# VIDILabs/instantvnr

Hardware: AMD Instinct MI355X
Metric: fps at 1024^2 on 1024^3 volume (higher is better)
Workload: dtype f16

## Files before the change

instantvnr_amd/csrc/infer_kernel.h:

```cpp
#pragma once
#include <algorithm>
#include <cstdlib>

#include "infer_tile.h"
#include "pack_rays.h"

namespace vnr {

struct FusedMlp {
  const uint16_t* packed;
  uint32_t lds_halves, width, n_hidden_matmuls, activation, output_activation;
  bool general;
  bool weights_global;
  float quantize_threshold;
};

struct InferArgs {
  const LevelInfo* levels;
  uint32_t n_levels, interpolation;
  const half_t* table;
  uint32_t table_bytes;
  const uint8_t* brick_image;
  const half_t* packed_mlp;
  const float* coords;
  float* out;
  half_t* features_out;
  half_t* acts_out;
  const uint32_t* n_ptr;
  const uint32_t* dest;
  uint32_t queue_mode;
  uint32_t out_stride;
  uint32_t n;
  uint32_t n_hidden_matmuls;
  uint32_t activation;
  uint32_t output_activation;
  uint32_t lds_halves;
  uint32_t sharers;
  uint32_t weights_global;
  float quantize_threshold;
  PackArgs pack;
};

template <int F, int K_IN, int W, int MODE, bool GENERAL>
__global__ void __launch_bounds__(64 * MlpShape<W>::WAVES) fused_infer_kernel(const InferArgs args)
{
  constexpr int NCHUNK = K_IN / 8;
  constexpr uint32_t WAVES = MlpShape<W>::WAVES;
  extern __shared__ __attribute__((aligned(16))) half_t lds[];

  const uint32_t lane = threadIdx.x & 63u;
  const uint32_t wave = threadIdx.x >> 6;

  if (MODE == 0 && WAVES == 4 && args.pack.n_blocks) {
    uint32_t* s_part = (uint32_t*)lds;
    for (uint32_t item = blockIdx.x; item < args.pack.n_blocks; item += gridDim.x) {
      pack_rays_block<4>(args.pack, item, s_part);
      __syncthreads();
    }
  }
  const uint32_t n = args.n_ptr ? min(*args.n_ptr, args.n) : args.n;
  const uint32_t n_tiles = (n + 63u) >> 6;
  const uint32_t xcd = blockIdx.x & 7u;
  const uint32_t per_xcd = (n_tiles + 7u) >> 3;
  const uint32_t waves_per_xcd = (gridDim.x >> 3) * WAVES;
  const uint32_t tile_end = min(n_tiles, (xcd + 1u) * per_xcd);
  if (xcd * per_xcd + (blockIdx.x >> 3) * WAVES >= tile_end) return;

  constexpr bool CAN_GLOBAL = GENERAL;
  const bool wglobal = CAN_GLOBAL && args.weights_global != 0u;
  if (MODE != 1 && !wglobal) {
    const uint4_t* src = (const uint4_t*)args.packed_mlp;
    uint4_t* dst = (uint4_t*)lds;
    for (uint32_t i = threadIdx.x; i < args.lds_halves / 8; i += blockDim.x) dst[i] = src[i];
    __syncthreads();
  }
  const uint32_t nh = args.n_hidden_matmuls;
  const uint32_t act = args.activation;
  const uint32_t h = lane >> 5;
  const uint32_t r = lane & 31u;
  const table_rsrc_t rsrc = make_table_rsrc(args.table, args.table_bytes);

  for (uint32_t tile = xcd * per_xcd + (blockIdx.x >> 3) * WAVES + wave; tile < tile_end; tile += waves_per_xcd) {
    const uint32_t i = tile * 64u + lane;
    const uint32_t ic = min(i, n - 1u);
    float3_packed p;
    uint32_t out_index = i;
    if (args.queue_mode) {
      const uint4_t rec = ((const uint4_t*)args.coords)[ic];
      p = {__uint_as_float(rec.x), __uint_as_float(rec.y), __uint_as_float(rec.z)};
      out_index = rec.w * args.out_stride;
    } else {
      p = ((const float3_packed*)args.coords)[ic];
      if (args.dest) out_index = args.dest[ic];
    }

    half8_t feat[NCHUNK];
    encode_tile<F, K_IN, GENERAL>(args.levels, args.n_levels, args.interpolation, rsrc, args.brick_image, p.x, p.y, p.z, feat,
                                  GENERAL ? args.quantize_threshold : 0.0f);

    if (MODE != 0 && args.features_out && i < n) {
      half8_t* dst = (half8_t*)(args.features_out + (size_t)i * K_IN);
#pragma unroll
      for (int c = 0; c < NCHUNK; ++c) dst[c] = feat[c];
    }
    if (MODE == 1) continue;

    float y;
    if (CAN_GLOBAL && wglobal)
      y = mlp_tile<W, K_IN, MODE == 2, GENERAL>(args.packed_mlp, feat, nh, act, h, r, args.acts_out, n, tile * 64u);
    else
      y = mlp_tile<W, K_IN, MODE == 2, GENERAL>((const half_t*)lds, feat, nh, act, h, r, args.acts_out, n, tile * 64u);
    if (i < n) args.out[out_index] = finish_output<GENERAL>(y, args.output_activation);
  }
}

template <int F, int K_IN, int W, int MODE, bool GENERAL>
static void launch_one(const InferArgs& a, size_t n_max, hipStream_t s)
{
  constexpr uint32_t WAVES = MlpShape<W>::WAVES;
  const Runtime& rt = Runtime::get();
  const uint32_t n_tiles = div_round_up(n_max, 64);
  uint32_t blocks = div_round_up(n_tiles, WAVES);
  static const uint32_t forced = [] {
    const char* e = std::getenv("VNR_AMD_INFER_BLOCKS_PER_CU");
    const int v = e ? std::atoi(e) : 0;
    return (uint32_t)(v >= 1 && v <= 64 ? v : 0);
  }();
  const size_t shmem = (MODE == 1 || a.weights_global) ? 16 : (size_t)a.lds_halves * sizeof(uint16_t);
  const uint32_t fit = (uint32_t)std::max<size_t>(1, std::min<size_t>(4, (160 * 1024) / std::max<size_t>(shmem, 1)));
  uint32_t max_blocks = (uint32_t)rt.n_cus * (forced ? forced : std::min(fit, a.sharers >= 2 ? 3u : 4u));
  if (!forced && a.n_ptr && a.queue_mode) max_blocks = std::min((uint32_t)rt.n_cus * 32u, std::max((uint32_t)rt.n_cus * 4u, n_tiles / 33u));
  if (blocks > max_blocks) blocks = max_blocks;
  blocks = next_multiple(blocks, 8);
  auto kernel = fused_infer_kernel<F, K_IN, W, MODE, GENERAL>;
  static bool attr_set = false;
  if (!attr_set) {
    VNR_HIP_CHECK(hipFuncSetAttribute((const void*)kernel, hipFuncAttributeMaxDynamicSharedMemorySize, 160 * 1024));
    attr_set = true;
  }
  kernel<<<blocks, 64 * WAVES, shmem, s>>>(a);
  VNR_HIP_CHECK(hipGetLastError());
}

template <int W, int MODE, bool GENERAL>
static void dispatch(uint32_t F, uint32_t K_IN, const InferArgs& a, size_t n_max, hipStream_t s)
{
#define VNR_CASE(f, k) if (F == f && K_IN == k) return launch_one<f, k, W, MODE, GENERAL>(a, n_max, s)
  VNR_CASE(1, 16); VNR_CASE(1, 32);
  VNR_CASE(2, 16); VNR_CASE(2, 32); VNR_CASE(2, 48); VNR_CASE(2, 64);
  VNR_CASE(4, 16); VNR_CASE(4, 32); VNR_CASE(4, 48); VNR_CASE(4, 64); VNR_CASE(4, 80); VNR_CASE(4, 96); VNR_CASE(4, 112); VNR_CASE(4, 128);
  VNR_CASE(8, 16); VNR_CASE(8, 32); VNR_CASE(8, 48); VNR_CASE(8, 64); VNR_CASE(8, 80); VNR_CASE(8, 96); VNR_CASE(8, 112); VNR_CASE(8, 128);
#undef VNR_CASE
  throw std::runtime_error("unsupported encoding shape: n_features_per_level=" + std::to_string(F) +
                           " padded width=" + std::to_string(K_IN));
}

#define VNR_DEFINE_FUSED_WIDTH(W, GENERAL, SUFFIX)                                                                        \
  void launch_fused_w##W##SUFFIX(int mode, uint32_t F, uint32_t K_IN, const InferArgs& a, size_t n_max, hipStream_t s)    \
  {                                                                                                                       \
    if (mode == 0) dispatch<W, 0, GENERAL>(F, K_IN, a, n_max, s);                                                         \
    else dispatch<W, 2, GENERAL>(F, K_IN, a, n_max, s);                                                                   \
  }

}
```

instantvnr_amd/csrc/march_device.h:

```cpp
#pragma once

#include <cfloat>

#include "renderer.h"
#include "sampling_device.h"

namespace vnr {

#define VNR_FLOAT_LARGE 1e20f
#define VNR_NEARLY_ONE 0.9999f

struct RenderParams {
  vec4f* frame;
  vec4f* accumulation;
  int width, height, frame_index;
  uint32_t pixel_lo, pixel_hi;
  uint32_t il_parts, il_part, n_local;
  uint32_t out_parts;
  uint32_t tiles_per_row, tile_row0;
  uint32_t tile_w_log2;
  float bin_depth_rcp;
  uint32_t tfn_in_lds;
  uint32_t debug_flags;
  vec3f cam_pos, cam_dir, cam_hor, cam_ver;
  affine3f wto;
  vec3i vol_dims;
  const float* volume;
  vec3f bbox_lo, bbox_hi;
  float step, step_rcp;
  vec3i mc_dims;
  vec3f mc_rcp;
  const float* mc_max_opacity;
  DeviceTfn tfn;
  int n_iters;
  affine3f otw;
  vec3f grad_step;
  vec3f light_dir;
  uint32_t slot_cap;
  uint32_t shading_mode;
  vec3f* px_org;
  vec3f* px_color;
  float* px_alpha;
  vec4f* px_shading;
  float* px_jitter;
  vec3f shadow_dir;
  float density_scale;
  uint32_t ssh_third_draw;
  uint32_t grad_flip;
  uint32_t pt_reset_interval;
};

#if defined(VNR_DIAG)
__host__ __device__ __forceinline__ uint32_t dbg(const RenderParams& p) { return p.debug_flags; }
#else
__host__ __device__ __forceinline__ constexpr uint32_t dbg(const RenderParams&) { return 0u; }
#endif

enum { M_NONE = 0, M_GRADIENT = 1, M_SSH = 2, M_SHADOW = 3 };

__device__ __forceinline__ uint32_t arena_value_index(uint32_t slot) { return 2u * slot; }
__device__ __forceinline__ uint32_t arena_grad_index(uint32_t slot_cap, uint32_t slot) { return 2u * slot_cap + 4u * slot; }

constexpr int kDepthBins = 64;


__device__ __forceinline__ float min3f(float a, float b, float c) { return fminf(fminf(a, b), c); }
__device__ __forceinline__ float max3f(float a, float b, float c) { return fmaxf(fmaxf(a, b), c); }

__device__ __forceinline__ bool intersect_box(float& t0, float& t1, vec3f org, vec3f dir, vec3f lower, vec3f upper)
{
  const bool sx = fabsf(dir.x) <= FLT_MIN, sy = fabsf(dir.y) <= FLT_MIN, sz = fabsf(dir.z) <= FLT_MIN;
  const vec3f rcp = {1.0f / dir.x, 1.0f / dir.y, 1.0f / dir.z};
  const vec3f lo = {sx ? VNR_FLOAT_LARGE : (lower.x - org.x) * rcp.x, sy ? VNR_FLOAT_LARGE : (lower.y - org.y) * rcp.y,
                    sz ? VNR_FLOAT_LARGE : (lower.z - org.z) * rcp.z};
  const vec3f hi = {sx ? -VNR_FLOAT_LARGE : (upper.x - org.x) * rcp.x, sy ? -VNR_FLOAT_LARGE : (upper.y - org.y) * rcp.y,
                    sz ? -VNR_FLOAT_LARGE : (upper.z - org.z) * rcp.z};
  t0 = fmaxf(t0, max3f(fminf(lo.x, hi.x), fminf(lo.y, hi.y), fminf(lo.z, hi.z)));
  t1 = fminf(t1, min3f(fmaxf(lo.x, hi.x), fmaxf(lo.y, hi.y), fmaxf(lo.z, hi.z)));
  return t1 > t0;
}

__device__ __forceinline__ void compute_ray(const RenderParams& p, uint32_t pixel, vec3f& org, vec3f& dir)
{
  const uint32_t ix = pixel % (uint32_t)p.width, iy = pixel / (uint32_t)p.width;
  const float sx = ((float)ix + 0.5f) / (float)p.width, sy = ((float)iy + 0.5f) / (float)p.height;
  org = xfm_point(p.wto, p.cam_pos);
  const vec3f d = (p.cam_dir + (sx - 0.5f) * p.cam_hor) + (sy - 0.5f) * p.cam_ver;
  dir = xfm_vector(p.wto, normalize(d));
}

__device__ __forceinline__ bool map_pixel(const RenderParams& p, uint32_t i, uint32_t& pixel)
{
  const uint32_t tile = i >> 6, l = i & 63u;
  const uint32_t tr_local = tile / p.tiles_per_row, t = tile - tr_local * p.tiles_per_row;
  const uint32_t twl = p.tile_w_log2, sub_log2 = twl - 3u;
  const uint32_t tc = t >> sub_log2, ts = t & ((1u << sub_log2) - 1u);
  const uint32_t x = (tc << twl) + (l & ((1u << twl) - 1u));
  const uint32_t y = (p.tile_row0 + tr_local * p.il_parts + p.il_part) * 8u + (ts << (6u - twl)) + (l >> twl);
  pixel = y * (uint32_t)p.width + x;
  return x < (uint32_t)p.width && y < (uint32_t)p.height && pixel >= p.pixel_lo && pixel < p.pixel_hi;
}

__device__ __forceinline__ float tea_lcg_first(uint32_t v0, uint32_t v1)
{
  uint32_t s0 = 0;
#pragma unroll
  for (int n = 0; n < 16; ++n) {
    s0 += 0x9e3779b9u;
    v0 += ((v1 << 4) + 0xa341316cu) ^ (v1 + s0) ^ ((v1 >> 5) + 0xc8013ea4u);
    v1 += ((v0 << 4) + 0xad90777du) ^ (v0 + s0) ^ ((v0 >> 5) + 0x7e95761eu);
  }
  const uint32_t state = 1664525u * v0 + 1013904223u;
  return (float)(state & 0x00FFFFFFu) / (float)0x01000000;
}

__device__ __forceinline__ uint32_t tea_lcg_two(uint32_t v0, uint32_t v1, float& a, float& b)
{
  uint32_t s0 = 0;
#pragma unroll
  for (int n = 0; n < 16; ++n) {
    s0 += 0x9e3779b9u;
    v0 += ((v1 << 4) + 0xa341316cu) ^ (v1 + s0) ^ ((v1 >> 5) + 0xc8013ea4u);
    v1 += ((v0 << 4) + 0xad90777du) ^ (v0 + s0) ^ ((v0 >> 5) + 0x7e95761eu);
  }
  uint32_t state = 1664525u * v0 + 1013904223u;
  a = (float)(state & 0x00FFFFFFu) / (float)0x01000000;
  state = 1664525u * state + 1013904223u;
  b = (float)(state & 0x00FFFFFFu) / (float)0x01000000;
  return state;
}

__device__ __forceinline__ float adaptive_sampling_rate(float base_step, float max_opacity)
{
  const float scale = 15.0f * base_step;
  const float r = fabsf(clampf(max_opacity, 0.1f, 1.0f) - 1.0f);
  return fmaxf(base_step + scale * (r * r), base_step);
}
__device__ __forceinline__ float opacity_correction(float step_rcp, float distance, float opacity)
{
  return 1.0f - __builtin_powf(1.0f - opacity, step_rcp * distance);
}
__device__ __forceinline__ void write_pixel(const RenderParams& p, vec4f rgba, uint32_t pixel)
{
  if (p.out_parts > 1u) {
    const uint32_t y = pixel / (uint32_t)p.width, x = pixel - y * (uint32_t)p.width;
    pixel = (((y >> 3) / p.out_parts) * 8u + (y & 7u)) * (uint32_t)p.width + x;
  }
  if (p.frame_index != 1) {
    const vec4f a = p.accumulation[pixel];
    rgba = {a.x + rgba.x, a.y + rgba.y, a.z + rgba.z, a.w + rgba.w};
  }
  p.accumulation[pixel] = rgba;
  const float f = (float)p.frame_index;
  p.frame[pixel] = {rgba.x / f, rgba.y / f, rgba.z / f, rgba.w / f};
}

__device__ __forceinline__ vec3f shade_simple_light(vec3f ray_dir, vec3f normal, vec3f albedo)
{
  if (dot(normal, normal) > 1.0e-6f) {
    const vec3f n = normalize(normal);
    const float c = 0.2f + 0.8f * fabsf(-dot(ray_dir, n));
    return c * albedo;
  }
  return {0, 0, 0};
}

__device__ __forceinline__ vec3f shade_scivis_light(vec3f ray_dir, vec3f normal, vec3f albedo, vec3f light_dir)
{
  const float m_ambient = 0.6f, m_diffuse = 0.9f, m_specular = 0.4f, m_shininess = 40.0f;
  vec3f color = {0, 0, 0};
  if (dot(normal, normal) > 1.0e-6f) {
    const vec3f L = normalize(light_dir);
    const vec3f N = normalize(normal);
    const vec3f V = {-ray_dir.x, -ray_dir.y, -ray_dir.z};
    color = color + m_ambient * albedo;
    const float cosNL = fmaxf(dot(N, L), 0.0f);
    if (cosNL > 0.0f) {
      color = color + (m_diffuse * cosNL) * albedo;
      const vec3f H = normalize(L + V);
      const float cosNH = fmaxf(dot(N, H), 0.0f);
      const float sp = m_specular * powf(cosNH, m_shininess);
      color = color + vec3f{sp, sp, sp};
    }
  }
  const vec3f shading2 = shade_simple_light(ray_dir, normal, albedo);
  return 0.5f * shading2 + 0.5f * color;
}

__device__ __forceinline__ vec3f gradient_shade(const RenderParams& p, vec3f ray_dir_obj, float f, float fgx, float fgy, float fgz,
                                                vec3f step, vec3f albedo)
{
  const vec3f No = {-((fgx - f) / step.x), -((fgy - f) / step.y), -((fgz - f) / step.z)};
  const vec3f Nw = {dot(p.wto.vx, No), dot(p.wto.vy, No), dot(p.wto.vz, No)};
  const vec3f dir_w = xfm_vector(p.otw, ray_dir_obj);
  const vec3f shaded = shade_scivis_light(dir_w, Nw, albedo, p.light_dir);
  const float k = 0.95f;
  return (1.0f - k) * albedo + k * shaded;
}

struct DDAState {
  vec3f t_next;
  vec3i cell;
  float next_cell_begin;
};

__device__ __forceinline__ void dda_init(DDAState& it, vec3f org, vec3f dir, float t_min, vec3i grid)
{
  const vec3f oiv = org + t_min * dir;
  const vec3f fc = {fmaxf(0.0f, fminf((float)grid.x - 1.0f, floorf(oiv.x))), fmaxf(0.0f, fminf((float)grid.y - 1.0f, floorf(oiv.y))),
                    fmaxf(0.0f, fminf((float)grid.z - 1.0f, floorf(oiv.z)))};
  const vec3f fe = {dir.x > 0.0f ? fc.x + 1.0f : fc.x, dir.y > 0.0f ? fc.y + 1.0f : fc.y, dir.z > 0.0f ? fc.z + 1.0f : fc.z};
  const vec3f ts = {fabsf(1.0f / dir.x), fabsf(1.0f / dir.y), fabsf(1.0f / dir.z)};
  it.t_next = {dir.x == 0.0f ? VNR_FLOAT_LARGE : fabsf(fe.x - oiv.x) * ts.x, dir.y == 0.0f ? VNR_FLOAT_LARGE : fabsf(fe.y - oiv.y) * ts.y,
               dir.z == 0.0f ? VNR_FLOAT_LARGE : fabsf(fe.z - oiv.z) * ts.z};
  it.cell = {(int)fc.x, (int)fc.y, (int)fc.z};
  it.next_cell_begin = 0.0f;
}

template <typename F>
__device__ __forceinline__ bool dda_next(DDAState& it, vec3f dir, float t_min, float t_max, vec3i grid, F&& fn)
{
  const vec3i stop = {dir.x > 0.0f ? grid.x : -1, dir.y > 0.0f ? grid.y : -1, dir.z > 0.0f ? grid.z : -1};
  if (it.cell.x == stop.x) return false;
  if (it.cell.y == stop.y) return false;
  if (it.cell.z == stop.z) return false;
  const vec3f ts = {fabsf(1.0f / dir.x), fabsf(1.0f / dir.y), fabsf(1.0f / dir.z)};
  const vec3i delta = {dir.x > 0.0f ? 1 : -1, dir.y > 0.0f ? 1 : -1, dir.z > 0.0f ? 1 : -1};
  const float t_closest = min3f(it.t_next.x, it.t_next.y, it.t_next.z);
  const float cell_t0 = fmaxf(t_min + it.next_cell_begin, t_min);
  const float cell_t1 = fminf(t_min + t_closest, t_max);
  if (cell_t0 >= cell_t1) return false;
  const bool go = fn(it.cell, cell_t0, cell_t1);
  if (go || fmaxf(t_min + it.next_cell_begin, t_min) >= cell_t1) {
    if (it.t_next.x == t_closest) { it.t_next.x += ts.x; it.cell.x += delta.x; if (it.cell.x == stop.x) return false; }
    if (it.t_next.y == t_closest) { it.t_next.y += ts.y; it.cell.y += delta.y; if (it.cell.y == stop.y) return false; }
    if (it.t_next.z == t_closest) { it.t_next.z += ts.z; it.cell.z += delta.z; if (it.cell.z == stop.z) return false; }
    it.next_cell_begin = t_closest;
  }
  return go;
}

__device__ __forceinline__ bool dda_resumable(const DDAState& it, vec3f dir, float t_min, float t_max, vec3i grid)
{
  const vec3i stop = {dir.x > 0.0f ? grid.x : -1, dir.y > 0.0f ? grid.y : -1, dir.z > 0.0f ? grid.z : -1};
  if (it.cell.x == stop.x) return false;
  if (it.cell.y == stop.y) return false;
  if (it.cell.z == stop.z) return false;
  const float t_closest = min3f(it.t_next.x, it.t_next.y, it.t_next.z);
  const float cell_t0 = fmaxf(t_min + it.next_cell_begin, t_min);
  const float cell_t1 = fminf(t_min + t_closest, t_max);
  return cell_t0 < cell_t1;
}

__device__ __forceinline__ float opacity_upper_bound(const RenderParams& p, vec3i cell)
{
#if defined(VNR_WALK_NOLOAD)
  return 0.05f + 1e-9f * (float)cell.x;
#endif
  const uint32_t idx = cell.x + cell.y * (uint32_t)p.mc_dims.x + cell.z * (uint32_t)p.mc_dims.x * (uint32_t)p.mc_dims.y;
  return p.mc_max_opacity[idx];
}

template <typename B>
__device__ __forceinline__ void iter_exec(const RenderParams& p, DDAState& it, vec3f dir, float t_min, float t_max, float step, B&& body)
{
  const vec3i grid = p.mc_dims;
  const vec3i stop = {dir.x > 0.0f ? grid.x : -1, dir.y > 0.0f ? grid.y : -1, dir.z > 0.0f ? grid.z : -1};
  if (it.cell.x == stop.x || it.cell.y == stop.y || it.cell.z == stop.z) return;
  const vec3f ts = {fabsf(1.0f / dir.x), fabsf(1.0f / dir.y), fabsf(1.0f / dir.z)};
  const vec3i delta = {dir.x > 0.0f ? 1 : -1, dir.y > 0.0f ? 1 : -1, dir.z > 0.0f ? 1 : -1};
  float r = opacity_upper_bound(p, it.cell);
  __builtin_amdgcn_s_waitcnt(0x0f70);
  bool more = true;
  while (more) {
    const float t_closest = min3f(it.t_next.x, it.t_next.y, it.t_next.z);
    const float cell_t0 = fmaxf(t_min + it.next_cell_begin, t_min);
    const float cell_t1 = fminf(t_min + t_closest, t_max);
    if (cell_t0 >= cell_t1) break;
    const bool bx = it.t_next.x == t_closest, by = it.t_next.y == t_closest, bz = it.t_next.z == t_closest;
    const vec3i nc = {it.cell.x + (bx ? delta.x : 0), it.cell.y + (by ? delta.y : 0), it.cell.z + (bz ? delta.z : 0)};
    const bool inside = nc.x != stop.x && nc.y != stop.y && nc.z != stop.z;
    const float r_next = opacity_upper_bound(p, inside ? nc : it.cell);
    bool go = true;
    if (!(fabsf(r) <= FLT_EPSILON)) {
      const float ss = adaptive_sampling_rate(step, r);
      float tx = cell_t0, ty = fminf(cell_t1, cell_t0 + ss);
      bool run = ty > tx;
      while (run) {
        it.next_cell_begin = ty - t_min;
        go = body(tx, ty);
        tx = ty;
        ty = fminf(tx + ss, cell_t1);
        run = go && ty > tx;
      }
    }
    const bool adv = go || fmaxf(t_min + it.next_cell_begin, t_min) >= cell_t1;
    it.t_next.x = (adv && bx) ? it.t_next.x + ts.x : it.t_next.x;
    it.t_next.y = (adv && by) ? it.t_next.y + ts.y : it.t_next.y;
    it.t_next.z = (adv && bz) ? it.t_next.z + ts.z : it.t_next.z;
    it.cell.x = adv ? nc.x : it.cell.x;
    it.cell.y = adv ? nc.y : it.cell.y;
    it.cell.z = adv ? nc.z : it.cell.z;
    it.next_cell_begin = adv ? t_closest : it.next_cell_begin;
    more = go && inside;
    r = r_next;
  }
}

__device__ __forceinline__ uint32_t depth_bin(const RenderParams& p, float t, float front)
{
  return (dbg(p) & 4u) ? 0u : min((uint32_t)kDepthBins - 1u, (uint32_t)fmaxf((t - front) * p.bin_depth_rcp, 0.0f));
}

}
```

instantvnr_amd/csrc/network.h:

```cpp
#pragma once

#include <functional>
#include <utility>
#include <vector>

#include "common.h"
#include "json.h"

namespace vnr {

constexpr int kMaxLevels = 32;
constexpr size_t kLdsBytes = 160 * 1024;
constexpr int kLossScale = 128;

struct LevelInfo {
  float scale;
  uint32_t resolution;
  uint32_t res2;
  uint32_t size;
  uint32_t offset;
  uint32_t hashed;
  uint32_t brick;
  uint32_t pad1;
};

template <int F> struct BrickShape;
template <> struct BrickShape<1> { static constexpr uint32_t lx = 2, ly = 2, lz = 2; };
template <> struct BrickShape<2> { static constexpr uint32_t lx = 2, ly = 2, lz = 1; };
template <> struct BrickShape<4> { static constexpr uint32_t lx = 2, ly = 1, lz = 1; };
template <> struct BrickShape<8> { static constexpr uint32_t lx = 1, ly = 1, lz = 1; };

struct GridDevice {
  LevelInfo levels[kMaxLevels];
  uint32_t n_levels;
  uint32_t n_features;
  uint32_t interpolation;
};

struct ModelConfig {
  uint32_t n_levels = 8, n_features = 8, log2_hashmap_size = 19, base_resolution = 16;
  float per_level_scale = 2.0f;
  uint32_t interpolation = 0;
  float quantize_threshold = 0.0f;
  float max_level = 1000.0f;
  uint32_t grid_type = 0;
  uint32_t n_neurons = 64, n_hidden_layers = 4;
  uint32_t activation = 1;
  uint32_t output_activation = 0;
  float learning_rate = 5e-3f, beta1 = 0.9f, beta2 = 0.999f, epsilon = 1e-15f, l2_reg = 1e-6f;
  uint32_t decay_start = 2000, decay_interval = 1000;
  float decay_base = 0.99f;
  bool has_decay = true;
  uint32_t loss = 0;
};

struct alignas(16) OptState {
  float master;
  float m, v;
  uint32_t step;
};
static_assert(sizeof(OptState) == 16, "OptState must be one 16-byte record");

struct TileNet;
struct PackArgs;
struct FusedMlp;

struct GradExchange {
  virtual ~GradExchange() = default;
  virtual void range_ready(size_t lo, size_t hi, hipStream_t s) = 0;
  virtual size_t bucket_params() const { return (size_t)16u << 20; }
};

struct GridBackwardPlan {
  uint32_t n_levels, lds_levels, tile_entries, lds_blocks;
  uint64_t atomic_requests, flush_requests_at_most;
};

class Network {
public:
  Network() = default;
  void configure(const Json& model, uint64_t init_seed);
  bool valid() const { return n_params_ > 0; }

  const ModelConfig& config() const { return cfg_; }
  const Json& model_json() const { return model_; }
  const GridDevice& grid() const { return grid_; }
  uint32_t padded_width() const { return in_width_; }
  uint32_t width() const { return cfg_.n_neurons; }
  uint32_t lds_halves() const { return lds_halves_; }
  bool weights_in_lds() const { return (size_t)lds_halves_ * 2 <= kLdsBytes; }
  bool common_kind() const
  {
    return cfg_.activation <= 1u && cfg_.output_activation == 0u && cfg_.interpolation != 2u && cfg_.grid_type != 2u && cfg_.quantize_threshold == 0.0f &&
           weights_in_lds();
  }
  uint32_t n_active_levels() const;
  uint32_t n_hidden_matmuls() const { return cfg_.n_hidden_layers - 1; }
  size_t n_params() const { return n_params_; }
  size_t n_mlp_params() const { return n_mlp_; }
  size_t n_grid_params() const { return n_params_ - n_mlp_; }
  size_t model_size_bytes() const { return n_params_ * sizeof(uint16_t); }
  uint64_t steps() const { return steps_; }

  void set_params_f16(const uint16_t* host, size_t count, hipStream_t s);
  void get_params_f16(uint16_t* host, size_t count, hipStream_t s) const;
  Json serialize_params(hipStream_t s) const;
  void deserialize_params(const Json& j, hipStream_t s);

  void inference(const float* d_coords, float* d_out, size_t n, const uint32_t* d_n, size_t n_max, hipStream_t s,
                 const uint32_t* d_dest = nullptr) const;
  bool tile_net(TileNet* out, hipStream_t s) const;
  bool inference_queue(const float* d_records, float* d_out, uint32_t out_stride, const uint32_t* d_n, size_t n_max, hipStream_t s,
                       uint32_t sharers = 1, const PackArgs* pack = nullptr) const;
  void encode(const float* d_coords, uint16_t* d_features, size_t n, hipStream_t s) const;

  void forward_backward(const float* d_coords, const float* d_targets, size_t batch, hipStream_t s, GradExchange* exchange = nullptr);
  uint16_t* grads_f16() { return grads_.ptr; }
  size_t grads_count() const { return grads_.count ? n_params_ : 0; }
  size_t grads_alloc() const { return n_params_ + (n_params_ & 1); }
  float* grads_as_f32(hipStream_t s);
  void optimizer_step(float grad_scale, hipStream_t s);
  void optimizer_step_range(size_t lo, size_t hi, float grad_scale, hipStream_t s);
  void optimizer_finish_step(hipStream_t s);
  float learning_rate() const { return lr_; }
  uint16_t* params_device() { return params_f16_.ptr; }
  OptState* opt_state_device() { return opt_state_.ptr; }
  void set_replica_state(uint64_t steps, float lr, hipStream_t s) { steps_ = steps; lr_ = lr; refresh_inference_weights(s); }
  void ensure_training_state(hipStream_t s);
  void reset_master_from_params(hipStream_t s);
  double training_loss(hipStream_t s);
  uint64_t params_generation() const { return params_generation_; }
  void set_opt_sharded(bool e) { opt_sharded_ = e; }
  bool opt_sharded() const { return opt_sharded_; }
  void set_deterministic(bool e) { deterministic_ = e; }
  bool deterministic() const { return deterministic_; }
  static bool deterministic_default();
  std::vector<std::pair<uint32_t, uint32_t>> exchange_level_buckets(size_t bucket) const;
  void for_each_exchange_range(size_t bucket, const std::function<void(size_t, size_t)>& fn) const;
  size_t level_range_lo(uint32_t level) const { return n_mlp_ + (size_t)grid_.levels[level].offset * cfg_.n_features; }
  size_t level_range_hi(uint32_t level_end) const { return n_mlp_ + ((size_t)grid_.levels[level_end - 1].offset + grid_.levels[level_end - 1].size) * cfg_.n_features; }
  const void* training_buffer(int which, size_t* bytes) const;
  void rescatter_grid_gradients(const float* d_coords, size_t n, hipStream_t s);
  void gradient_distance(const uint16_t* d_ref, double out[4], hipStream_t s);
  void scatter_grid_gradients(const float* d_coords, size_t batch, hipStream_t s, GradExchange* exchange, hipStream_t s_lds = nullptr);
  void set_grads_from_f32(const float* host, size_t count, hipStream_t s);

  size_t bytes_allocated() const;
  void release_temporary();
  static void release_temporary_of_all();

  void set_brick_resolution_cap(uint32_t cap) { brick_res_cap_ = cap; }
  void set_brick_mode(int mode);
  void set_brick_budget(size_t bytes);
  GridBackwardPlan grid_backward_plan(size_t batch) const;
  uint32_t brick_levels_mask() const { return brick_levels_mask_; }
  bool brick_image_in_use() const { return brick_valid_; }
  size_t brick_image_bytes() const { return brick_image_.bytes(); }
  float brick_build_ms() const { return brick_build_ms_; }
  uint64_t brick_builds() const { return brick_builds_; }
  uint64_t brick_small_builds() const { return brick_small_builds_; }
  int brick_tier() const { return brick_valid_ ? brick_tier_ : 0; }
  uint32_t brick_after_now() const;

private:
  void build_layout();
  void initialize_params(uint64_t seed, hipStream_t s);
  void refresh_inference_weights(hipStream_t s);
  FusedMlp fused_mlp() const;
  const LevelInfo* inference_levels(hipStream_t s, const uint8_t** image, size_t n_max) const;
  void build_brick_image(hipStream_t s, bool small) const;
  static double brick_small_budget();

  ModelConfig cfg_;
  Json model_;
  GridDevice grid_{};
  uint32_t in_width_ = 0;
  size_t n_params_ = 0, n_mlp_ = 0;
  uint64_t steps_ = 0;
  uint64_t params_generation_ = 0;
  bool opt_sharded_ = false;
  bool deterministic_ = deterministic_default();
  float lr_ = 0.0f;

  DeviceBuffer<uint16_t> params_f16_{MemTag::Network};
  DeviceBuffer<uint16_t> mlp_packed_{MemTag::Network};
  DeviceBuffer<uint16_t> mlp_packed_T_{MemTag::Network};
  DeviceBuffer<LevelInfo> levels_dev_{MemTag::Network};
  DeviceBuffer<OptState> opt_state_{MemTag::Network};
  DeviceBuffer<uint16_t> grads_{MemTag::Network};
  DeviceBuffer<float> grads_f32_{MemTag::Network};
  DeviceBuffer<uint16_t> ws_features_{MemTag::Network};
  DeviceBuffer<uint16_t> ws_acts_{MemTag::Network};
  DeviceBuffer<uint16_t> ws_dfeat_{MemTag::Network};
  DeviceBuffer<float> ws_loss_{MemTag::Network};
  size_t ws_batch_ = 0;
  hipStream_t side_stream_ = nullptr;
  hipEvent_t ev_fork_ = nullptr, ev_join_ = nullptr;
  uint32_t lds_halves_ = 0, lds_halves_T_ = 0;
  mutable DeviceBuffer<uint8_t> brick_image_{MemTag::Network};
  mutable DeviceBuffer<LevelInfo> levels_brick_dev_{MemTag::Network};
  mutable bool brick_valid_ = false, brick_refused_ = false;
  mutable uint32_t brick_stable_calls_ = 0;
  static constexpr uint32_t kBrickPaysAfter = 64;
  mutable uint32_t brick_served_calls_ = 0, brick_after_scale_ = 1;
  mutable uint64_t brick_builds_ = 0;
  static constexpr size_t kBrickSmallMinLaunch = (size_t)1 << 20;
  mutable int brick_tier_ = 0;
  mutable bool brick_small_refused_ = false;
  mutable uint64_t brick_small_builds_ = 0;
  mutable float brick_build_ms_ = 0.0f;
  uint32_t brick_res_cap_ = 0;
  size_t brick_budget_ = 0;
  mutable uint32_t brick_levels_mask_ = 0;
  int brick_mode_ = -1;

public:
  static constexpr int kTrainPhases = 5, kTrainProfileSteps = 64;
  void set_train_profiling(bool e);
  int train_profile(double* ms_per_step );
private:
  void profile_mark(int phase_boundary, hipStream_t s);
  bool train_profiling_ = false;
  std::vector<hipEvent_t> prof_events_;
  uint64_t prof_steps_ = 0;

public:
  ~Network();
  Network(const Network&) = delete;
  Network& operator=(const Network&) = delete;
};

uint32_t grid_make_layout(const ModelConfig& cfg, GridDevice* out);

}
```

instantvnr_amd/csrc/network_host.hip:

```cpp
#include "network.h"

#include <algorithm>
#include <cstdlib>
#include <set>

#include "infer_kernel.h"

namespace vnr {

void launch_pack_mlp(const uint16_t* params, uint16_t* packed, uint16_t* packedT, uint32_t in_width, uint32_t W, uint32_t n_hidden_matmuls, hipStream_t s);
void launch_fused(int mode, const GridDevice& grid, uint32_t in_width, const FusedMlp& mlp, const LevelInfo* d_levels, const uint16_t* table, size_t table_bytes,
                  const float* coords, float* out, uint16_t* features_out, uint16_t* acts_out, size_t n, const uint32_t* d_n, size_t n_max, hipStream_t s,
                  const uint32_t* d_dest = nullptr, uint32_t queue_out_stride = 0, const uint8_t* brick_image = nullptr,
                  uint32_t sharers = 1, const struct PackArgs* pack = nullptr);
void launch_init_params(OptState* state, uint16_t* params, size_t n_mlp, size_t n_total, uint32_t in_width,
                        uint32_t n_hidden_matmuls, uint32_t width, uint64_t seed, hipStream_t s);
void launch_master_from_f16(const uint16_t* params, OptState* state, size_t n, bool reset_optimizer, hipStream_t s);

uint16_t f32_to_f16(float f)
{
  uint32_t x;
  std::memcpy(&x, &f, 4);
  const uint32_t sign = (x >> 16) & 0x8000u;
  const uint32_t ax = x & 0x7fffffffu;
  if (ax >= 0x7f800000u) return (uint16_t)(sign | 0x7c00u | ((ax > 0x7f800000u) ? (0x200u | ((ax >> 13) & 0x3ffu)) : 0u));
  if (ax >= 0x477ff000u) return (uint16_t)(sign | 0x7c00u);
  if (ax < 0x33000001u) return (uint16_t)sign;
  const int32_t e = (int32_t)(ax >> 23) - 127;
  const uint32_t m = (ax & 0x7fffffu) | 0x800000u;
  const uint32_t shift = e < -14 ? (uint32_t)(-1 - e) : 13u;
  const uint32_t he = e < -14 ? 0u : (uint32_t)(e + 15);
  uint32_t q = m >> shift;
  const uint32_t rem = m & ((1u << shift) - 1u), half = 1u << (shift - 1);
  if (rem > half || (rem == half && (q & 1u))) q++;
  return (uint16_t)(sign | (he == 0 ? q : ((he - 1) << 10) + q));
}

float f16_to_f32(uint16_t h)
{
  const uint32_t sign = ((uint32_t)h & 0x8000u) << 16, e = (h >> 10) & 0x1fu, m = h & 0x3ffu;
  uint32_t x;
  if (e == 0) {
    if (m == 0) x = sign;
    else { float v = (float)m * 5.9604644775390625e-8f; std::memcpy(&x, &v, 4); x |= sign; }
  } else if (e == 31) x = sign | 0x7f800000u | (m << 13);
  else x = sign | ((e + 112u) << 23) | (m << 13);
  float f;
  std::memcpy(&f, &x, 4);
  return f;
}

uint32_t grid_make_layout(const ModelConfig& cfg, GridDevice* out)
{
  if (cfg.n_levels > (uint32_t)kMaxLevels) throw std::runtime_error("too many hash-grid levels");
  const float log2_pls = std::log2(cfg.per_level_scale);
  uint32_t offset = 0;
  for (uint32_t l = 0; l < cfg.n_levels; ++l) {
    const float scale = exp2f((float)l * log2_pls) * (float)cfg.base_resolution - 1.0f;
    const uint32_t res = (uint32_t)ceilf(scale) + 1u;
    const uint32_t max_params = 0xffffffffu / 2u;
    const double cube = (double)res * (double)res * (double)res;
    uint32_t n = cube > (double)max_params ? max_params : (uint32_t)cube;
    n = next_multiple(n, 8u);
    if (cfg.grid_type == 2u) {
      const double tile = (double)cfg.base_resolution * cfg.base_resolution * cfg.base_resolution;
      if ((double)n > tile) n = (uint32_t)tile;
    } else if (cfg.grid_type == 0u) {
      const uint32_t cap = 1u << cfg.log2_hashmap_size;
      if (n > cap) n = cap;
    }
    if (n == 0) throw std::runtime_error("grid level without entries");
    uint32_t stride = 1, dims = 0;
    for (; dims < 3 && stride <= n; ++dims) stride *= res;
    LevelInfo& lv = out->levels[l];
    lv.scale = scale;
    lv.resolution = res;
    lv.res2 = res * res;
    lv.size = n;
    lv.offset = offset;
    if (cfg.grid_type == 0u) lv.hashed = n < stride ? 1u : 0u;
    else lv.hashed = (dims == 3 && (uint64_t)res * res * res <= (uint64_t)n) ? 0u : 1u + dims;
    lv.brick = lv.pad1 = 0;
    if (lv.hashed == 1u && (n & (n - 1)) != 0) throw std::runtime_error("internal: hashed level with non power-of-two size");
    if ((uint64_t)offset + n > 0xffffffffull) throw std::runtime_error("grid encoding too large (more than 2^32 entries)");
    offset += n;
  }
  out->n_levels = cfg.n_levels;
  out->n_features = cfg.n_features;
  out->interpolation = cfg.interpolation;
  return offset;
}

static std::set<Network*>& live_networks()
{
  static std::set<Network*> s;
  return s;
}

static uint32_t json_u32(const Json& j, const char* key, uint32_t def) { return j.contains(key) ? (uint32_t)j.at(key).as_int() : def; }
static float json_f32(const Json& j, const char* key, float def) { return j.contains(key) ? j.at(key).as_float() : def; }
static std::string json_str(const Json& j, const char* key, const char* def) { return j.contains(key) ? j.at(key).as_string() : std::string(def); }

void Network::configure(const Json& config, uint64_t init_seed)
{
  const Json loss = config.value("loss", Json::object());
  const Json enc = config.value("encoding", Json::object());
  const Json net = config.value("network", Json::object());
  ModelConfig c = cfg_;
  if (config.contains("optimizer")) {
    const Json& opt = config.at("optimizer");
    const std::string ot = json_str(opt, "otype", "Adam");
    const Json* adam = &opt;
    if (ot == "ExponentialDecay") {
      c.has_decay = true;
      c.decay_start = json_u32(opt, "decay_start", 10000);
      c.decay_interval = json_u32(opt, "decay_interval", 10000);
      c.decay_base = json_f32(opt, "decay_base", 0.33f);
      if (!opt.contains("nested")) throw std::runtime_error("ExponentialDecay optimizer needs a 'nested' optimizer");
      adam = &opt.at("nested");
    } else {
      c.has_decay = false;
    }
    if (json_str(*adam, "otype", "Adam") != "Adam") throw std::runtime_error("unsupported optimizer otype (Adam / ExponentialDecay{Adam} only)");
    c.learning_rate = json_f32(*adam, "learning_rate", 1e-3f);
    c.beta1 = json_f32(*adam, "beta1", 0.9f);
    c.beta2 = json_f32(*adam, "beta2", 0.999f);
    c.epsilon = json_f32(*adam, "epsilon", 1e-8f);
    c.l2_reg = json_f32(*adam, "l2_reg", 1e-8f);
  }
  const std::string lt = json_str(loss, "otype", "L2");
  if (lt == "L1") c.loss = 0;
  else if (lt == "L2") c.loss = 1;
  else throw std::runtime_error("unsupported loss otype: " + lt);

  const std::string et = json_str(enc, "otype", "");
  if (et != "HashGrid" && et != "Grid" && et != "DenseGrid" && et != "TiledGrid")
    throw std::runtime_error("unsupported encoding otype: '" + et + "' (HashGrid / Grid / DenseGrid / TiledGrid)");
  const std::string gt = json_str(enc, "type", et == "DenseGrid" ? "Dense" : et == "TiledGrid" ? "Tiled" : "Hash");
  if (gt == "Hash") c.grid_type = 0;
  else if (gt == "Dense") c.grid_type = 1;
  else if (gt == "Tiled") c.grid_type = 2;
  else throw std::runtime_error("unsupported grid type: " + gt + " (Hash / Dense / Tiled)");
  c.n_levels = json_u32(enc, "n_levels", 16);
  c.n_features = json_u32(enc, "n_features_per_level", 2);
  c.log2_hashmap_size = json_u32(enc, "log2_hashmap_size", 19);
  c.base_resolution = json_u32(enc, "base_resolution", 16);
  c.per_level_scale = json_f32(enc, "per_level_scale", 2.0f);
  const std::string it = json_str(enc, "interpolation", "Linear");
  if (it == "Linear") c.interpolation = 0;
  else if (it == "Smoothstep") c.interpolation = 1;
  else if (it == "Nearest") c.interpolation = 2;
  else throw std::runtime_error("unsupported interpolation: " + it);
  c.quantize_threshold = json_f32(enc, "quantize_threshold", 0.0f);
  c.max_level = json_f32(enc, "max_level", 1000.0f);
  if (c.n_features != 1 && c.n_features != 2 && c.n_features != 4 && c.n_features != 8)
    throw std::runtime_error("n_features_per_level must be 1, 2, 4 or 8");
  if (c.log2_hashmap_size > 28) throw std::runtime_error("log2_hashmap_size too large");

  const std::string nt = json_str(net, "otype", "FullyFusedMLP");
  if (nt != "FullyFusedMLP") throw std::runtime_error("unsupported network otype: " + nt + " (FullyFusedMLP only)");
  c.n_neurons = json_u32(net, "n_neurons", 128);
  c.n_hidden_layers = json_u32(net, "n_hidden_layers", 5);
  if (c.n_neurons != 16 && c.n_neurons != 32 && c.n_neurons != 64 && c.n_neurons != 128)
    throw std::runtime_error("FullyFusedMLP n_neurons must be 16, 32, 64 or 128");
  if (c.n_hidden_layers < 1) throw std::runtime_error("n_hidden_layers must be >= 1");
  auto activation_of = [](const std::string& a, const char* what) -> uint32_t {
    if (a == "None") return kActNone;
    if (a == "ReLU") return kActReLU;
    if (a == "Exponential") return kActExponential;
    if (a == "Sigmoid") return kActSigmoid;
    if (a == "Squareplus") return kActSquareplus;
    if (a == "Softplus") return kActSoftplus;
    throw std::runtime_error(std::string("unsupported ") + what + ": " + a + " (None / ReLU / Exponential / Sigmoid / Squareplus / Softplus)");
  };
  c.activation = activation_of(json_str(net, "activation", "ReLU"), "activation");
  c.output_activation = activation_of(json_str(net, "output_activation", "None"), "output_activation");

  cfg_ = c;
  model_ = Json::object();
  model_["loss"] = loss;
  model_["encoding"] = enc;
  model_["network"] = net;
  build_layout();
  steps_ = 0;
  lr_ = cfg_.learning_rate;
  initialize_params(init_seed, Runtime::get().stream);
  live_networks().insert(this);
}

void Network::build_layout()
{
  const uint32_t total_entries = grid_make_layout(cfg_, &grid_);
  in_width_ = next_multiple(cfg_.n_levels * cfg_.n_features, 16u);
  const uint32_t widest = cfg_.n_features == 1 ? 32u : cfg_.n_features == 2 ? 64u : 128u;
  if (in_width_ > widest)
    throw std::runtime_error("unsupported encoding shape: n_features_per_level=" + std::to_string(cfg_.n_features) + " with n_levels=" +
                             std::to_string(cfg_.n_levels) + " (encoded width " + std::to_string(in_width_) + " > " + std::to_string(widest) + ")");
  const size_t W = cfg_.n_neurons;
  n_mlp_ = W * in_width_ + (size_t)n_hidden_matmuls() * W * W + (size_t)16 * W;
  n_params_ = n_mlp_ + (size_t)total_entries * cfg_.n_features;
  if ((n_params_ - n_mlp_) * sizeof(uint16_t) >= (1ull << 32)) throw std::runtime_error("hash table >= 4 GiB is not supported");
  lds_halves_ = packed_mlp_halves(in_width_, cfg_.n_neurons, n_hidden_matmuls());
  lds_halves_T_ = packedT_halves(in_width_, cfg_.n_neurons, n_hidden_matmuls());
  params_f16_.resize(n_params_);
  mlp_packed_.resize(lds_halves_);
  mlp_packed_T_.resize(lds_halves_T_);
  levels_dev_.resize(kMaxLevels);
  levels_dev_.upload(grid_.levels, kMaxLevels, Runtime::get().stream);
  VNR_HIP_CHECK(hipStreamSynchronize(Runtime::get().stream));
  opt_state_.release(); grads_.release(); grads_f32_.release();
  ws_batch_ = 0;
}

void Network::initialize_params(uint64_t seed, hipStream_t s)
{
  opt_state_.resize(n_params_);
  launch_init_params(opt_state_.ptr, params_f16_.ptr, n_mlp_, n_params_, in_width_, n_hidden_matmuls(), cfg_.n_neurons, seed, s);
  ++params_generation_;
  opt_sharded_ = false;
  refresh_inference_weights(s);
}

uint32_t Network::n_active_levels() const
{
  uint32_t n = 0;
  while (n < cfg_.n_levels && !((float)n >= cfg_.max_level + 1e-3f)) ++n;
  return n;
}

void Network::refresh_inference_weights(hipStream_t s)
{
  launch_pack_mlp(params_f16_.ptr, mlp_packed_.ptr, mlp_packed_T_.ptr, in_width_, cfg_.n_neurons, n_hidden_matmuls(), s);
  if (brick_valid_ && brick_tier_ == 2) {
    if (brick_served_calls_ < kBrickPaysAfter) brick_after_scale_ = std::min<uint32_t>(brick_after_scale_ * 2u, 1u << 16);
    else brick_after_scale_ = 1;
  }
  brick_valid_ = false;
  brick_tier_ = 0;
  brick_stable_calls_ = 0;
  brick_served_calls_ = 0;
}

static uint32_t brick_after_base()
{
  static const uint32_t after = [] { const char* e = std::getenv("VNR_AMD_BRICK_AFTER"); return e ? (uint32_t)std::max(0, std::atoi(e)) : 24u; }();
  return after;
}

uint32_t Network::brick_after_now() const { return brick_after_base() * brick_after_scale_; }

double Network::brick_small_budget()
{
  static const double gb = [] { const char* e = std::getenv("VNR_AMD_BRICK_SMALL_GB"); return e ? std::max(0.0, std::atof(e)) : 0.75; }();
  return gb * 1073741824.0;
}

Network::~Network()
{
  live_networks().erase(this);
  for (hipEvent_t e : prof_events_) (void)hipEventDestroy(e);
  if (side_stream_) { (void)hipStreamSynchronize(side_stream_); (void)hipStreamDestroy(side_stream_); (void)hipEventDestroy(ev_fork_); (void)hipEventDestroy(ev_join_); }
}

void Network::set_brick_mode(int mode)
{
  brick_mode_ = mode < 0 ? -1 : (mode > 0 ? 1 : 0);
  brick_refused_ = false;
  brick_small_refused_ = false;
  if (brick_mode_ == 0 && brick_valid_) {
    if (Runtime::get().ready()) (void)hipDeviceSynchronize();
    brick_image_.release();
    levels_brick_dev_.release();
    brick_valid_ = false;
    brick_tier_ = 0;
  }
  brick_stable_calls_ = 0;
}

void Network::set_brick_budget(size_t bytes)
{
  brick_budget_ = bytes;
  brick_refused_ = false;
  brick_small_refused_ = false;
  if (brick_valid_) {
    if (Runtime::get().ready()) (void)hipDeviceSynchronize();
    brick_image_.release();
    levels_brick_dev_.release();
    brick_valid_ = false;
    brick_tier_ = 0;
  }
  brick_levels_mask_ = 0;
  brick_stable_calls_ = 0;
}

void Network::set_train_profiling(bool e)
{
  train_profiling_ = e;
  prof_steps_ = 0;
  if (e && prof_events_.empty()) {
    prof_events_.resize((size_t)kTrainProfileSteps * (kTrainPhases + 1));
    for (hipEvent_t& ev : prof_events_) VNR_HIP_CHECK(hipEventCreate(&ev));
  }
}

void Network::profile_mark(int boundary, hipStream_t s)
{
  if (!train_profiling_) return;
  VNR_HIP_CHECK(hipEventRecord(prof_events_[(size_t)(prof_steps_ % kTrainProfileSteps) * (kTrainPhases + 1) + boundary], s));
  if (boundary == kTrainPhases) ++prof_steps_;
}

int Network::train_profile(double* ms_per_step)
{
  for (int p = 0; p < kTrainPhases; ++p) ms_per_step[p] = 0.0;
  const int n = (int)std::min<uint64_t>(prof_steps_, kTrainProfileSteps);
  if (!train_profiling_ || n == 0) return 0;
  VNR_HIP_CHECK(hipEventSynchronize(prof_events_[(size_t)((prof_steps_ - 1) % kTrainProfileSteps) * (kTrainPhases + 1) + kTrainPhases]));
  for (int k = 0; k < n; ++k)
    for (int p = 0; p < kTrainPhases; ++p) {
      float ms = 0.0f;
      VNR_HIP_CHECK(hipEventElapsedTime(&ms, prof_events_[(size_t)k * (kTrainPhases + 1) + p], prof_events_[(size_t)k * (kTrainPhases + 1) + p + 1]));
      ms_per_step[p] += ms / n;
    }
  return n;
}

void Network::release_temporary()
{
  if (Runtime::get().ready()) (void)hipDeviceSynchronize();
  brick_image_.release();
  levels_brick_dev_.release();
  brick_valid_ = false;
  brick_tier_ = 0;
  brick_stable_calls_ = 0;
  ws_features_.release(); ws_acts_.release(); ws_dfeat_.release();
  ws_batch_ = 0;
}

void Network::release_temporary_of_all()
{
  for (Network* n : live_networks()) n->release_temporary();
}

template <int F>
__global__ void brick_build_kernel(const LevelInfo lv, const half_t* __restrict__ table, uint8_t* __restrict__ image, uint64_t n_entries)
{
  typedef typename FeatVec<F>::type vec_t;
  constexpr uint32_t LX = BrickShape<F>::lx, LY = BrickShape<F>::ly, LZ = BrickShape<F>::lz;
  constexpr uint32_t E = 1u << (LX + LY + LZ);
  const uint32_t nbx = (lv.resolution >> LX) + 1u, nby = (lv.resolution >> LY) + 1u;
  vec_t* out = (vec_t*)(image + (size_t)(lv.brick - 1u) * 128u);
  const vec_t* src = (const vec_t*)(table + (size_t)lv.offset * F);
  if constexpr (F == 2) {
    const uint32_t gnbx = lv.pad1, gnby = (lv.resolution >> 1) + 1u;
    for (uint64_t e = (uint64_t)blockIdx.x * blockDim.x + threadIdx.x; e < n_entries; e += (uint64_t)gridDim.x * blockDim.x) {
      const uint32_t w = (uint32_t)(e & 31u);
      const uint64_t b = e >> 5;
      const uint32_t bx = (uint32_t)(b % gnbx), by = (uint32_t)((b / gnbx) % gnby), bz = (uint32_t)(b / ((uint64_t)gnbx * gnby));
      const uint32_t x = bx * 7u + (w & 7u), y = (by << 1) | ((w >> 3) & 1u), z = (bz << 1) | (w >> 4);
      vec_t v;
      if (x <= lv.resolution && y <= lv.resolution && z <= lv.resolution) v = src[level_index(lv, x, y, z)];
      else v = vec_t{};
      out[e] = v;
    }
    return;
  }
  for (uint64_t e = (uint64_t)blockIdx.x * blockDim.x + threadIdx.x; e < n_entries; e += (uint64_t)gridDim.x * blockDim.x) {
    const uint32_t w = (uint32_t)(e & (E - 1u));
    const uint64_t b = e >> (LX + LY + LZ);
    const uint32_t bx = (uint32_t)(b % nbx), by = (uint32_t)((b / nbx) % nby), bz = (uint32_t)(b / ((uint64_t)nbx * nby));
    const uint32_t x = (bx << LX) | (w & ((1u << LX) - 1u)), y = (by << LY) | ((w >> LX) & ((1u << LY) - 1u)), z = (bz << LZ) | (w >> (LX + LY));
    vec_t v;
    if (x <= lv.resolution && y <= lv.resolution && z <= lv.resolution) v = src[level_index(lv, x, y, z)];
    else v = vec_t{};
    out[e] = v;
  }
}

template <int F>
__global__ void __launch_bounds__(256) brick_build_rows_kernel(const LevelInfo lv, const half_t* __restrict__ table, uint8_t* __restrict__ image,
                                                               uint32_t nbx, uint32_t nby, uint32_t nbz)
{
  typedef typename FeatVec<F>::type vec_t;
  constexpr uint32_t LX = F == 2 ? 3u : BrickShape<F>::lx, LY = F == 2 ? 1u : BrickShape<F>::ly, LZ = F == 2 ? 1u : BrickShape<F>::lz;
  constexpr uint32_t E = 1u << (LX + LY + LZ), ROWS = 1u << (LY + LZ);
  static_assert(E * F * 2 == 128, "a brick is one 128-byte line");
  extern __shared__ __attribute__((aligned(16))) uint8_t s_raw[];
  vec_t* s_rows = (vec_t*)s_raw;
  const uint32_t res = lv.resolution, nx = (res + 4u) & ~3u;
  const vec_t* src = (const vec_t*)(table + (size_t)lv.offset * F);
  vec_t* out = (vec_t*)(image + (size_t)(lv.brick - 1u) * 128u);
  for (uint32_t row = blockIdx.x; row < nby * nbz; row += gridDim.x) {
    const uint32_t by = row % nby, bz = row / nby;
    for (uint32_t r = 0; r < ROWS; ++r) {
      const uint32_t y = (by << LY) | (r & ((1u << LY) - 1u)), z = (bz << LZ) | (r >> LY);
      const bool inside = y <= res && z <= res;
      if (F == 2 && lv.hashed == 1u && lv.size >= 4u && inside) {
        const uint32_t h = (y * 2654435761u) ^ (z * 805459861u), mask = lv.size - 1u, hl = h & 3u;
        for (uint32_t x4 = threadIdx.x * 4u; x4 < nx; x4 += 1024u) {
          const uint4_t v = *(const uint4_t*)(src + (((x4 ^ h) & mask) & ~3u));
          uint4_t o;
          if (hl == 0u) o = v; else if (hl == 1u) o = uint4_t{v.y, v.x, v.w, v.z}; else if (hl == 2u) o = uint4_t{v.z, v.w, v.x, v.y}; else o = uint4_t{v.w, v.z, v.y, v.x};
          *(uint4_t*)(s_rows + r * nx + x4) = o;
        }
      } else {
        for (uint32_t x = threadIdx.x; x < res + 1u; x += 256u) s_rows[r * nx + x] = inside ? src[level_index(lv, x, y, z)] : vec_t{};
      }
    }
    __syncthreads();
    vec_t* dst = out + (size_t)row * nbx * E;
    if constexpr (F == 2) {
      for (uint32_t t4 = threadIdx.x; t4 < nbx * 8u; t4 += 256u) {
        const uint32_t b = t4 >> 3, r = (t4 >> 1) & 3u, x0 = b * 7u + (t4 & 1u) * 4u;
        const uint32_t* rowp = (const uint32_t*)(s_rows + r * nx);
        uint4_t o;
        o.x = x0 <= res ? rowp[x0] : 0u;
        o.y = x0 + 1u <= res ? rowp[x0 + 1u] : 0u;
        o.z = x0 + 2u <= res ? rowp[x0 + 2u] : 0u;
        o.w = x0 + 3u <= res ? rowp[x0 + 3u] : 0u;
        *(uint4_t*)(dst + (size_t)t4 * 4u) = o;
      }
    } else {
      for (uint32_t t = threadIdx.x; t < nbx * E; t += 256u) {
        const uint32_t b = t / E, w = t % E;
        const uint32_t wx = w & ((1u << LX) - 1u), r = w >> LX;
        const uint32_t x = (b << LX) | wx;
        dst[t] = x <= res ? s_rows[r * nx + x] : vec_t{};
      }
    }
    __syncthreads();
  }
}

template <int F>
static void launch_brick_build(const LevelInfo& lv, const uint16_t* table, uint8_t* image, uint64_t n_entries, hipStream_t s)
{
  constexpr uint32_t LX = F == 2 ? 3u : BrickShape<F>::lx, LY = F == 2 ? 1u : BrickShape<F>::ly, LZ = F == 2 ? 1u : BrickShape<F>::lz;
  const uint64_t res = lv.resolution;
  const uint32_t nbx = F == 2 ? lv.pad1 : (uint32_t)(res >> LX) + 1u, nby = (uint32_t)(res >> LY) + 1u, nbz = (uint32_t)(res >> LZ) + 1u;
  const size_t shmem = (size_t)(1u << (LY + LZ)) * ((res + 4) & ~(uint64_t)3) * F * 2;
  if (shmem <= 64 * 1024 && (uint64_t)nbx * nby * nbz * (128u / (F * 2)) == n_entries) {
    const uint32_t blocks = (uint32_t)std::min<uint64_t>((uint64_t)nby * nbz, 1u << 20);
    brick_build_rows_kernel<F><<<blocks, 256, shmem, s>>>(lv, (const half_t*)table, image, nbx, nby, nbz);
  } else {
    const uint32_t blocks = (uint32_t)std::min<uint64_t>((n_entries + 255) / 256, 1u << 20);
    brick_build_kernel<F><<<blocks, 256, 0, s>>>(lv, (const half_t*)table, image, n_entries);
  }
  VNR_HIP_CHECK(hipGetLastError());
}

void Network::build_brick_image(hipStream_t s, bool small) const
{
  static const double max_gb = [] { const char* e = std::getenv("VNR_AMD_BRICK_MAX_GB"); return e ? std::atof(e) : -1.0; }();
  size_t free_b = 0, total_b = 0;
  VNR_HIP_CHECK(hipMemGetInfo(&free_b, &total_b));
  double policy = brick_budget_ ? (double)brick_budget_ : max_gb >= 0.0 ? max_gb * 1073741824.0 : (double)total_b / 16.0;
  if (small) policy = std::min(policy, brick_small_budget());
  const uint64_t budget_lines = (uint64_t)std::min(policy, (double)(free_b + brick_image_.bytes()) / 4.0) / 128u;
  const uint32_t mask_before = brick_valid_ ? brick_levels_mask_ : 0u;
  brick_levels_mask_ = 0;
  hipEvent_t t0, t1;
  VNR_HIP_CHECK(hipEventCreate(&t0)); VNR_HIP_CHECK(hipEventCreate(&t1));
  const uint32_t F = cfg_.n_features;
  const uint32_t lx = F == 8 ? 1 : 2, ly = F >= 4 ? 1 : 2, lz = F == 1 ? 2 : 1;
  const uint64_t entries_per_line = 64u / F;
  std::vector<LevelInfo> lv(grid_.levels, grid_.levels + kMaxLevels);
  std::vector<uint64_t> lines(kMaxLevels, 0);
  uint64_t used = 0;
  const bool finest_first = F <= 2;
  for (int k = 0; k < (int)grid_.n_levels; ++k) {
    const int l = finest_first ? (int)grid_.n_levels - 1 - k : k;
    if (lv[l].hashed != 1u) continue;
    if (brick_res_cap_ && lv[l].resolution > brick_res_cap_ + 1u) continue;
    const uint64_t res = lv[l].resolution;
    uint64_t n = ((res >> lx) + 1) * ((res >> ly) + 1) * ((res >> lz) + 1);
    if (F == 2) {
      if (res >= 13000) continue;
      n = (res / 7 + 1) * ((res >> 1) + 1) * ((res >> 1) + 1);
      lv[l].pad1 = (uint32_t)(res / 7 + 1);
    }
    if (n * entries_per_line >= (1ull << 32) || used + n + 1 > budget_lines || used + n + 1 >= 0xffffffffull) continue;
    lv[l].brick = (uint32_t)used + 1u;
    lines[l] = n;
    used += n;
    brick_levels_mask_ |= 1u << l;
  }
  if (used == 0) {
    if (!small) brick_refused_ = true;
    else brick_small_refused_ = true;
    brick_valid_ = false;
    (void)hipEventDestroy(t0); (void)hipEventDestroy(t1);
    return;
  }
  if (!small && brick_valid_ && mask_before == brick_levels_mask_ && brick_image_.bytes() == (used + 1) * 128u) {
    brick_tier_ = 2;
    (void)hipEventDestroy(t0); (void)hipEventDestroy(t1);
    return;
  }
  if (brick_image_.bytes() != (used + 1) * 128u) {
    if (brick_image_.bytes()) VNR_HIP_CHECK(hipDeviceSynchronize());
    brick_valid_ = false;
  }
  brick_image_.resize((used + 1) * 128u);
  VNR_HIP_CHECK(hipEventRecord(t0, s));
  for (uint32_t l = 0; l < grid_.n_levels; ++l) {
    if (!lv[l].brick) continue;
    const uint64_t n_entries = lines[l] * entries_per_line;
    const uint16_t* table = params_f16_.ptr + n_mlp_;
    switch (F) {
    case 1: launch_brick_build<1>(lv[l], table, brick_image_.ptr, n_entries, s); break;
    case 2: launch_brick_build<2>(lv[l], table, brick_image_.ptr, n_entries, s); break;
    case 4: launch_brick_build<4>(lv[l], table, brick_image_.ptr, n_entries, s); break;
    default: launch_brick_build<8>(lv[l], table, brick_image_.ptr, n_entries, s); break;
    }
  }
  VNR_HIP_CHECK(hipMemsetAsync(brick_image_.ptr + used * 128u, 0, 128, s));
  levels_brick_dev_.resize(kMaxLevels);
  VNR_HIP_CHECK(hipMemcpyAsync(levels_brick_dev_.ptr, lv.data(), kMaxLevels * sizeof(LevelInfo), hipMemcpyHostToDevice, s));
  VNR_HIP_CHECK(hipEventRecord(t1, s));
  VNR_HIP_CHECK(hipEventSynchronize(t1));
  VNR_HIP_CHECK(hipEventElapsedTime(&brick_build_ms_, t0, t1));
  (void)hipEventDestroy(t0); (void)hipEventDestroy(t1);
  brick_valid_ = true;
  brick_tier_ = small ? 1 : 2;
}

const LevelInfo* Network::inference_levels(hipStream_t s, const uint8_t** image, size_t n_max) const
{
  static const int env_mode = [] { const char* e = std::getenv("VNR_AMD_BRICK"); return e ? std::atoi(e) : -1; }();
  const int mode = brick_mode_ >= 0 ? brick_mode_ : env_mode;
  *image = nullptr;
  if (mode == 0 || brick_refused_) return levels_dev_.ptr;
  if (brick_tier_ != 2 || !brick_valid_) {
    if (brick_stable_calls_ < 0xffffffffu) ++brick_stable_calls_;
    const bool want_full = mode == 1 || brick_stable_calls_ > brick_after_now();
    if (want_full) {
      build_brick_image(s, false);
      if (brick_valid_ && brick_tier_ == 2) { ++brick_builds_; brick_served_calls_ = 0; }
    } else if (!brick_valid_ && !brick_small_refused_ && n_max >= kBrickSmallMinLaunch && brick_small_budget() > 0.0 && cfg_.n_features <= 2u) {
      build_brick_image(s, true);
      if (brick_valid_) ++brick_small_builds_;
    }
    if (!brick_valid_) return levels_dev_.ptr;
  }
  if (brick_served_calls_ < 0xffffffffu) ++brick_served_calls_;
  *image = brick_image_.ptr;
  return levels_brick_dev_.ptr;
}

void Network::set_params_f16(const uint16_t* host, size_t count, hipStream_t s)
{
  if (count != n_params_) throw std::runtime_error("parameter count mismatch: got " + std::to_string(count) + ", model has " + std::to_string(n_params_));
  VNR_HIP_CHECK(hipMemcpyAsync(params_f16_.ptr, host, count * sizeof(uint16_t), hipMemcpyHostToDevice, s));
  if (opt_state_.count == n_params_) launch_master_from_f16(params_f16_.ptr, opt_state_.ptr, n_params_, false, s);
  ++params_generation_;
  refresh_inference_weights(s);
  VNR_HIP_CHECK(hipStreamSynchronize(s));
}

void Network::get_params_f16(uint16_t* host, size_t count, hipStream_t s) const
{
  if (count != n_params_) throw std::runtime_error("parameter count mismatch");
  VNR_HIP_CHECK(hipMemcpyAsync(host, params_f16_.ptr, count * sizeof(uint16_t), hipMemcpyDeviceToHost, s));
  VNR_HIP_CHECK(hipStreamSynchronize(s));
}

Json Network::serialize_params(hipStream_t s) const
{
  std::vector<uint16_t> host(n_params_);
  get_params_f16(host.data(), n_params_, s);
  Json j = Json::object();
  j["n_params"] = (uint64_t)n_params_;
  j["params_type"] = "__half";
  j["params_binary"] = Json::binary(host.data(), host.size() * sizeof(uint16_t));
  return j;
}

void Network::deserialize_params(const Json& j, hipStream_t s)
{
  const size_t n = (size_t)j.at("n_params").as_int();
  if (n != n_params_) throw std::runtime_error("Can't set params because buffer has the wrong size: " + std::to_string(n) + " vs " + std::to_string(n_params_));
  const std::string type = j.at("params_type").as_string();
  const std::string& bin = j.at("params_binary").as_binary();
  std::vector<uint16_t> host(n);
  if (type == "__half") {
    if (bin.size() != n * 2) throw std::runtime_error("params_binary has the wrong size");
    std::memcpy(host.data(), bin.data(), n * 2);
  } else if (type == "float") {
    if (bin.size() != n * 4) throw std::runtime_error("params_binary has the wrong size");
    const float* f = (const float*)bin.data();
    for (size_t i = 0; i < n; ++i) host[i] = f32_to_f16(f[i]);
  } else {
    throw std::runtime_error("Unknown params_type: " + type);
  }
  set_params_f16(host.data(), n, s);
  if (j.contains("optimizer") || j.contains("step")) {  }
}

void Network::inference(const float* d_coords, float* d_out, size_t n, const uint32_t* d_n, size_t n_max, hipStream_t s,
                        const uint32_t* d_dest) const
{
  const uint8_t* image;
  const LevelInfo* levels = inference_levels(s, &image, d_n ? n_max : n);
  GridDevice grid = grid_;
  grid.n_levels = n_active_levels();
  launch_fused(0, grid, in_width_, fused_mlp(), levels, params_f16_.ptr + n_mlp_, n_grid_params() * 2, d_coords, d_out, nullptr, nullptr, n, d_n, n_max, s, d_dest, 0, image);
}

bool Network::inference_queue(const float* d_records, float* d_out, uint32_t out_stride, const uint32_t* d_n, size_t n_max, hipStream_t s,
                              uint32_t sharers, const PackArgs* pack) const
{
  const uint8_t* image;
  const LevelInfo* levels = inference_levels(s, &image, n_max);
  GridDevice grid = grid_;
  grid.n_levels = n_active_levels();
  if (cfg_.n_neurons == 128u) pack = nullptr;
  launch_fused(0, grid, in_width_, fused_mlp(), levels, params_f16_.ptr + n_mlp_, n_grid_params() * 2, d_records, d_out, nullptr, nullptr, 0, d_n, n_max, s, nullptr,
               out_stride, image, sharers, pack);
  return pack != nullptr;
}

FusedMlp Network::fused_mlp() const
{
  const bool wglobal = !weights_in_lds();
  return FusedMlp{mlp_packed_.ptr, lds_halves_, cfg_.n_neurons, n_hidden_matmuls(), cfg_.activation, cfg_.output_activation, !common_kind() || wglobal, wglobal,
                  cfg_.quantize_threshold};
}

bool Network::tile_net(TileNet* out, hipStream_t s) const
{
  if (!weights_in_lds()) return false;
  if (n_grid_params() * 2 >= (1ull << 32)) throw std::runtime_error("hash table >= 4 GiB is not supported");
  const uint8_t* image;
  const LevelInfo* levels = inference_levels(s, &image, kBrickSmallMinLaunch);
  out->levels = levels;
  out->n_levels = n_active_levels();
  out->interpolation = grid_.interpolation;
  out->table = (const half_t*)(params_f16_.ptr + n_mlp_);
  out->table_bytes = (uint32_t)(n_grid_params() * 2);
  out->brick_image = image;
  out->packed_mlp = (const half_t*)mlp_packed_.ptr;
  out->lds_halves = lds_halves_;
  out->n_hidden_matmuls = n_hidden_matmuls();
  out->activation = cfg_.activation;
  out->output_activation = cfg_.output_activation;
  out->n_features = grid_.n_features;
  out->in_width = in_width_;
  out->width = cfg_.n_neurons;
  out->general = common_kind() ? 0u : 1u;
  out->quantize_threshold = cfg_.quantize_threshold;
  return true;
}

void Network::encode(const float* d_coords, uint16_t* d_features, size_t n, hipStream_t s) const
{
  const uint8_t* image;
  const LevelInfo* levels = inference_levels(s, &image, n);
  GridDevice grid = grid_;
  grid.n_levels = n_active_levels();
  launch_fused(1, grid, in_width_, fused_mlp(), levels, params_f16_.ptr + n_mlp_, n_grid_params() * 2, d_coords, nullptr, d_features, nullptr, n, nullptr, n, s, nullptr, 0, image);
}

size_t Network::bytes_allocated() const
{
  return brick_image_.bytes() + params_f16_.bytes() + mlp_packed_.bytes() + mlp_packed_T_.bytes() + opt_state_.bytes() + grads_.bytes() + grads_f32_.bytes() + ws_features_.bytes() + ws_acts_.bytes() + ws_dfeat_.bytes() + ws_loss_.bytes();
}

}
```

instantvnr_amd/csrc/network_infer.hip:

```cpp
#include "infer_kernel.h"

namespace vnr {

__global__ void pack_mlp_kernel(const half_t* __restrict__ params, half_t* __restrict__ packed, half_t* __restrict__ packedT, uint32_t in_width,
                                uint32_t W, uint32_t nh)
{
  const uint32_t RW = mlp_rows_padded(W), KS = W / 16u, step = 16u * RW, hidden = KS * step;
  const uint32_t total = packed_mlp_halves(in_width, W, nh), totalT = packedT ? packedT_halves(in_width, W, nh) : 0u;
  const uint32_t l1 = (in_width / 16u) * step;
  const uint32_t first_sz = W * in_width;
  for (uint32_t e = blockIdx.x * blockDim.x + threadIdx.x; e < total + totalT; e += gridDim.x * blockDim.x) {
    half_t v = (half_t)0.0f;
    if (e < total) {
      if (e < l1) {
        const uint32_t j = e & 7u, q = e >> 3, row = q % RW, hs = q / RW, h = hs & 1u, s = hs >> 1;
        if (row < W) v = params[row * in_width + 16u * s + 8u * h + j];
      } else if (e < l1 + nh * hidden) {
        const uint32_t r = e - l1, layer = r / hidden, qq = r % hidden;
        const uint32_t j = qq & 7u, q = qq >> 3, row = q % RW, hs = q / RW, h = hs & 1u, s = hs >> 1;
        const uint32_t k = 16u * s + 8u * (j >> 2) + 4u * h + (j & 3u);
        if (row < W) v = params[first_sz + layer * W * W + row * W + k];
      } else {
        const uint32_t q = e - l1 - nh * hidden;
        const uint32_t j = q & 7u, h = (q >> 3) & 1u, s = q >> 4;
        const uint32_t k = 16u * s + 8u * (j >> 2) + 4u * h + (j & 3u);
        v = params[first_sz + nh * W * W + k];
      }
      packed[e] = v;
    } else {
      const uint32_t t = e - total;
      const uint32_t rp = ((in_width + 31u) / 32u) * 32u;
      if (t < KS * 16u) {
        const uint32_t j = t & 7u, h = (t >> 3) & 1u, s = t >> 4;
        v = params[first_sz + nh * W * W + 16u * s + 8u * (j >> 2) + 4u * h + (j & 3u)];
      } else if (t < KS * 16u + nh * hidden) {
        const uint32_t r = t - KS * 16u, layer = r / hidden, qq = r % hidden;
        const uint32_t j = qq & 7u, q = qq >> 3, row = q % RW, hs = q / RW, h = hs & 1u, s = hs >> 1;
        const uint32_t kk = 16u * s + 8u * (j >> 2) + 4u * h + (j & 3u);
        if (row < W) v = params[first_sz + layer * W * W + kk * W + row];
      } else {
        const uint32_t qq = t - KS * 16u - nh * hidden;
        const uint32_t j = qq & 7u, q = qq >> 3, row = q % rp, hs = q / rp, h = hs & 1u, s = hs >> 1;
        const uint32_t kk = 16u * s + 8u * (j >> 2) + 4u * h + (j & 3u);
        if (row < in_width) v = params[kk * in_width + row];
      }
      packedT[t] = v;
    }
  }
}

void launch_pack_mlp(const uint16_t* params, uint16_t* packed, uint16_t* packedT, uint32_t in_width, uint32_t W, uint32_t n_hidden_matmuls, hipStream_t s)
{
  const uint32_t total = packed_mlp_halves(in_width, W, n_hidden_matmuls) + (packedT ? packedT_halves(in_width, W, n_hidden_matmuls) : 0u);
  pack_mlp_kernel<<<div_round_up(total, 256), 256, 0, s>>>((const half_t*)params, (half_t*)packed, (half_t*)packedT, in_width, W, n_hidden_matmuls);
}

#define VNR_DECL(name) void name(int mode, uint32_t F, uint32_t K_IN, const InferArgs& a, size_t n_max, hipStream_t s)
VNR_DECL(launch_fused_w16); VNR_DECL(launch_fused_w32); VNR_DECL(launch_fused_w64); VNR_DECL(launch_fused_w128);
VNR_DECL(launch_fused_w16g); VNR_DECL(launch_fused_w32g); VNR_DECL(launch_fused_w64g); VNR_DECL(launch_fused_w128g);
#undef VNR_DECL

void launch_fused(int mode, const GridDevice& grid, uint32_t in_width, const FusedMlp& mlp, const LevelInfo* d_levels, const uint16_t* table, size_t table_bytes,
                  const float* coords, float* out, uint16_t* features_out, uint16_t* acts_out, size_t n, const uint32_t* d_n, size_t n_max, hipStream_t s,
                  const uint32_t* d_dest, uint32_t queue_out_stride, const uint8_t* brick_image, uint32_t sharers, const PackArgs* pack)
{
  if (n_max == 0) { if (pack && pack->n_blocks) throw std::runtime_error("internal: ray packing fused into an empty evaluation launch"); return; }
  if (n_max > 0xffffffc0ull) throw std::runtime_error("inference batch too large (max 2^32-64 samples per call)");
  if (table_bytes >= (1ull << 32)) throw std::runtime_error("hash table >= 4 GiB is not supported");
  InferArgs a;
  a.levels = d_levels;
  a.n_levels = grid.n_levels;
  a.interpolation = grid.interpolation;
  a.table = (const half_t*)table;
  a.table_bytes = (uint32_t)table_bytes;
  a.brick_image = brick_image;
  a.sharers = sharers;
  a.packed_mlp = (const half_t*)mlp.packed;
  a.coords = coords;
  a.out = out;
  a.features_out = (half_t*)features_out;
  a.acts_out = (half_t*)acts_out;
  a.n_ptr = d_n;
  a.dest = d_dest;
  a.queue_mode = queue_out_stride ? 1u : 0u;
  a.out_stride = queue_out_stride;
  a.n = d_n ? (uint32_t)n_max : (uint32_t)n;
  a.n_hidden_matmuls = mlp.n_hidden_matmuls;
  a.activation = mlp.activation;
  a.output_activation = mlp.output_activation;
  a.lds_halves = mlp.lds_halves;
  a.weights_global = mlp.weights_global ? 1u : 0u;
  a.quantize_threshold = mlp.quantize_threshold;
  if (mlp.weights_global && !mlp.general) throw std::runtime_error("internal: weights from global memory are a GENERAL instance's");
  if (pack && mode == 0) {
    if (mlp.width == 128u) throw std::runtime_error("internal: the 128-neuron evaluation kernel (8 waves per block) does not take the ray packing prologue");
    a.pack = *pack;
  } else a.pack.n_blocks = 0;
  if (mode == 1) {
    if (mlp.general) return dispatch<64, 1, true>(grid.n_features, in_width, a, n_max, s);
    return dispatch<64, 1, false>(grid.n_features, in_width, a, n_max, s);
  }
  const uint32_t F = grid.n_features;
  switch (mlp.width) {
  case 16: return mlp.general ? launch_fused_w16g(mode, F, in_width, a, n_max, s) : launch_fused_w16(mode, F, in_width, a, n_max, s);
  case 32: return mlp.general ? launch_fused_w32g(mode, F, in_width, a, n_max, s) : launch_fused_w32(mode, F, in_width, a, n_max, s);
  case 64: return mlp.general ? launch_fused_w64g(mode, F, in_width, a, n_max, s) : launch_fused_w64(mode, F, in_width, a, n_max, s);
  case 128: return mlp.general ? launch_fused_w128g(mode, F, in_width, a, n_max, s) : launch_fused_w128(mode, F, in_width, a, n_max, s);
  default: throw std::runtime_error("internal: no MFMA kernel for n_neurons = " + std::to_string(mlp.width));
  }
}

}
```

instantvnr_amd/csrc/network_train.hip:

```cpp
#include "infer_kernel.h"

namespace vnr {

void launch_fused(int mode, const GridDevice& grid, uint32_t in_width, const FusedMlp& mlp, const LevelInfo* d_levels, const uint16_t* table, size_t table_bytes,
                  const float* coords, float* out, uint16_t* features_out, uint16_t* acts_out, size_t n, const uint32_t* d_n, size_t n_max, hipStream_t s,
                  const uint32_t* d_dest = nullptr, uint32_t queue_out_stride = 0, const uint8_t* brick_image = nullptr,
                  uint32_t sharers = 1, const struct PackArgs* pack = nullptr);

struct Pcg32 {
  uint64_t state, inc;
  __host__ __device__ Pcg32(uint64_t initstate, uint64_t initseq = 0xda3e39cb94b95bdbULL)
  {
    state = 0u;
    inc = (initseq << 1u) | 1u;
    next_uint();
    state += initstate;
    next_uint();
  }
  __host__ __device__ uint32_t next_uint()
  {
    const uint64_t old = state;
    state = old * 0x5851f42d4c957f2dULL + inc;
    const uint32_t xs = (uint32_t)(((old >> 18u) ^ old) >> 27u);
    const uint32_t rot = (uint32_t)(old >> 59u);
    return (xs >> rot) | (xs << ((~rot + 1u) & 31));
  }
  __host__ __device__ float next_float()
  {
    const uint32_t u = (next_uint() >> 9) | 0x3f800000u;
    return __builtin_bit_cast(float, u) - 1.0f;
  }
  __host__ __device__ void advance(uint64_t delta)
  {
    uint64_t cur_mult = 0x5851f42d4c957f2dULL, cur_plus = inc, acc_mult = 1u, acc_plus = 0u;
    while (delta > 0) {
      if (delta & 1) { acc_mult *= cur_mult; acc_plus = acc_plus * cur_mult + cur_plus; }
      cur_plus = (cur_mult + 1) * cur_plus;
      cur_mult *= cur_mult;
      delta >>= 1;
    }
    state = acc_mult * state + acc_plus;
  }
};

__global__ void init_params_kernel(OptState* __restrict__ state, half_t* __restrict__ params, size_t n_mlp, size_t n_total,
                                   uint32_t in_width, uint32_t n_hidden_matmuls, uint32_t width, uint64_t seed)
{
  const size_t t = (size_t)blockIdx.x * blockDim.x + threadIdx.x;
  const size_t e0 = t * 4;
  if (e0 >= n_total) return;
  Pcg32 rng(seed);
  rng.advance(e0);
  const size_t first = (size_t)width * in_width, hidden_end = first + (size_t)n_hidden_matmuls * width * width;
  for (size_t e = e0; e < e0 + 4 && e < n_total; ++e) {
    const float u = rng.next_float();
    float scale;
    if (e < first) scale = sqrtf(6.0f / (float)(in_width + width));
    else if (e < hidden_end) scale = sqrtf(6.0f / (float)(width + width));
    else if (e < n_mlp) scale = sqrtf(6.0f / (float)(width + 16));
    else scale = 1e-4f;
    const float v = u * (2.0f * scale) - scale;
    state[e] = OptState{v, 0.0f, 0.0f, 0u};
    params[e] = (half_t)v;
  }
}

void launch_init_params(OptState* state, uint16_t* params, size_t n_mlp, size_t n_total, uint32_t in_width,
                        uint32_t n_hidden_matmuls, uint32_t width, uint64_t seed, hipStream_t s)
{
  const size_t threads = (n_total + 3) / 4;
  init_params_kernel<<<div_round_up(threads, 256), 256, 0, s>>>(state, (half_t*)params, n_mlp, n_total, in_width,
                                                                n_hidden_matmuls, width, seed);
  VNR_HIP_CHECK(hipGetLastError());
}

__global__ void master_from_f16_kernel(const half_t* __restrict__ in, OptState* __restrict__ state, size_t n, bool reset_optimizer)
{
  for (size_t i = (size_t)blockIdx.x * blockDim.x + threadIdx.x; i < n; i += (size_t)gridDim.x * blockDim.x) {
    if (reset_optimizer) state[i] = OptState{(float)in[i], 0.0f, 0.0f, 0u};
    else state[i].master = (float)in[i];
  }
}
void launch_master_from_f16(const uint16_t* params, OptState* state, size_t n, bool reset_optimizer, hipStream_t s)
{
  master_from_f16_kernel<<<min(div_round_up(n, 256), 4096u), 256, 0, s>>>((const half_t*)params, state, n, reset_optimizer);
  VNR_HIP_CHECK(hipGetLastError());
}

__global__ void loss_grad_kernel(const float* __restrict__ y, const float* __restrict__ target, uint32_t n, uint32_t loss_type, uint32_t out_act,
                                 half_t* __restrict__ dy, float* __restrict__ loss_partials)
{
  __shared__ float red[256];
  float acc = 0.0f;
  const float inv_n = 1.0f / (float)n;
  for (uint32_t i = blockIdx.x * blockDim.x + threadIdx.x; i < n; i += gridDim.x * blockDim.x) {
    const float d = y[i] - target[i];
    float g;
    if (loss_type == 0) { acc += fabsf(d) * inv_n; g = copysignf(1.0f, d); }
    else { acc += d * d * inv_n; g = 2.0f * d; }
    dy[i] = act_backward_f16((half_t)((float)kLossScale * g * inv_n), (half_t)y[i], out_act);
  }
  red[threadIdx.x] = acc;
  __syncthreads();
  for (uint32_t s = 128; s > 0; s >>= 1) {
    if (threadIdx.x < s) red[threadIdx.x] += red[threadIdx.x + s];
    __syncthreads();
  }
  if (threadIdx.x == 0) loss_partials[blockIdx.x] = red[0];
}

struct BackwardArgs {
  const half_t* packedT;
  const half_t* dy;
  const half_t* acts;
  half_t* d_out;
  half_t* dfeat;
  uint32_t n, nh, activation, in_width, lds_halves;
  uint32_t weights_global;
};

__device__ __forceinline__ half8_t load_frag_rowmajor(const half_t* row, int s, uint32_t h)
{
  const half4_t lo = *(const half4_t*)(row + 16 * s + 4 * h);
  const half4_t hi = *(const half4_t*)(row + 16 * s + 8 + 4 * h);
  return half8_t{lo[0], lo[1], lo[2], lo[3], hi[0], hi[1], hi[2], hi[3]};
}
__device__ __forceinline__ void store_frag_rowmajor(half_t* row, int s, uint32_t h, const half8_t& v)
{
  *(half4_t*)(row + 16 * s + 4 * h) = half4_t{v[0], v[1], v[2], v[3]};
  *(half4_t*)(row + 16 * s + 8 + 4 * h) = half4_t{v[4], v[5], v[6], v[7]};
}
__device__ __forceinline__ half8_t pack_plain(const f32x16& acc, int sh)
{
  float8_t v;
#pragma unroll
  for (int j = 0; j < 8; ++j) v[j] = acc[8 * sh + j];
  return __builtin_convertvector(v, half8_t);
}
__device__ __noinline__ half8_t act_backward_general8(half8_t d, half8_t a, uint32_t act)
{
#pragma unroll
  for (int j = 0; j < 8; ++j) d[j] = act_backward_f16(d[j], a[j], act);
  return d;
}
template <bool GENERAL>
__device__ __forceinline__ half8_t act_backward8(const half8_t& d, const half8_t& a, uint32_t act)
{
  if (act == kActNone) return d;
  if (GENERAL && act > kActReLU) return act_backward_general8(d, a, act);
  half8_t r;
#pragma unroll
  for (int j = 0; j < 8; ++j) r[j] = a[j] > (half_t)0.0f ? d[j] : (half_t)0.0f;
  return r;
}

template <int W, int MTF, bool GENERAL>
__global__ void __launch_bounds__(256) mlp_backward_kernel(const BackwardArgs args)
{
  typedef MlpShape<W> Sh;
  constexpr int MT = Sh::MT, RW = Sh::RW, KS = Sh::KS;
  constexpr int NTB = W == 128 ? 1 : 2;
  extern __shared__ __attribute__((aligned(16))) half_t lds[];
  constexpr bool CAN_GLOBAL = GENERAL;
  const bool wglobal = CAN_GLOBAL && args.weights_global != 0u;
  if (!wglobal) {
    const uint4_t* src = (const uint4_t*)args.packedT;
    uint4_t* dst = (uint4_t*)lds;
    for (uint32_t i = threadIdx.x; i < args.lds_halves / 8; i += blockDim.x) dst[i] = src[i];
    __syncthreads();
  }
  const uint32_t lane = threadIdx.x & 63u, wave = threadIdx.x >> 6;
  const uint32_t h = lane >> 5, r = lane & 31u;
  const uint32_t n = args.n, nh = args.nh;
  const uint32_t act = args.activation;
  const uint32_t n_tiles = (n + 63u) >> 6;
  constexpr int RP = MTF * 32;

  auto run = [&](const half_t* __restrict__ img) __attribute__((always_inline)) {
  for (uint32_t tile = blockIdx.x * 4u + wave; tile < n_tiles; tile += gridDim.x * 4u) {
#pragma unroll
    for (int nt0 = 0; nt0 < 2; nt0 += NTB) {
      half8_t bf[KS][NTB];
      uint32_t smp[NTB];
      bool ok[NTB];
#pragma unroll
      for (int q = 0; q < NTB; ++q) {
        smp[q] = tile * 64u + 32u * (uint32_t)(nt0 + q) + r;
        ok[q] = smp[q] < n;
        const uint32_t sc = ok[q] ? smp[q] : n - 1u;
        const float g = (float)args.dy[sc];
        const half_t* arow = args.acts + ((size_t)nh * n + sc) * W;
#pragma unroll
        for (int s = 0; s < KS; ++s) {
          const half8_t wv = *(const half8_t*)(img + (s * 2 + h) * 8);
          half8_t d;
#pragma unroll
          for (int j = 0; j < 8; ++j) d[j] = (half_t)((float)wv[j] * g);
          d = act_backward8<GENERAL>(d, load_frag_rowmajor(arow, s, h), act);
          bf[s][q] = d;
          if (ok[q]) store_frag_rowmajor(args.d_out + ((size_t)nh * n + smp[q]) * W, s, h, d);
        }
      }
      for (int layer = (int)nh - 1; layer >= 0; --layer) {
        const half_t* w = img + Sh::LAST + layer * Sh::HIDDEN;
        f32x16 acc[MT][NTB];
#pragma unroll
        for (int m = 0; m < MT; ++m)
#pragma unroll
          for (int q = 0; q < NTB; ++q)
#pragma unroll
            for (int e = 0; e < 16; ++e) acc[m][q][e] = 0.0f;
#pragma unroll
        for (int s = 0; s < KS; ++s)
#pragma unroll
          for (int m = 0; m < MT; ++m) {
            const half8_t a = *(const half8_t*)(w + ((s * 2 + h) * RW + m * 32 + r) * 8);
#pragma unroll
            for (int q = 0; q < NTB; ++q) acc[m][q] = __builtin_amdgcn_mfma_f32_32x32x16_f16(a, bf[s][q], acc[m][q], 0, 0, 0);
          }
#pragma unroll
        for (int q = 0; q < NTB; ++q) {
          const uint32_t sc = ok[q] ? smp[q] : n - 1u;
          const half_t* arow = args.acts + ((size_t)layer * n + sc) * W;
#pragma unroll
          for (int s = 0; s < KS; ++s) {
            half8_t d = pack_plain(acc[s >> 1][q], s & 1);
            d = act_backward8<GENERAL>(d, load_frag_rowmajor(arow, s, h), act);
            bf[s][q] = d;
            if (ok[q]) store_frag_rowmajor(args.d_out + ((size_t)layer * n + smp[q]) * W, s, h, d);
          }
        }
      }
      {
        const half_t* w = img + Sh::LAST + nh * Sh::HIDDEN;
        f32x16 acc[MTF][NTB];
#pragma unroll
        for (int m = 0; m < MTF; ++m)
#pragma unroll
          for (int q = 0; q < NTB; ++q)
#pragma unroll
            for (int e = 0; e < 16; ++e) acc[m][q][e] = 0.0f;
#pragma unroll
        for (int s = 0; s < KS; ++s)
#pragma unroll
          for (int m = 0; m < MTF; ++m) {
            const half8_t a = *(const half8_t*)(w + ((s * 2 + h) * RP + m * 32 + r) * 8);
#pragma unroll
            for (int q = 0; q < NTB; ++q) acc[m][q] = __builtin_amdgcn_mfma_f32_32x32x16_f16(a, bf[s][q], acc[m][q], 0, 0, 0);
          }
#pragma unroll
        for (int q = 0; q < NTB; ++q) {
          if (!ok[q]) continue;
          half_t* row = args.dfeat + (size_t)smp[q] * args.in_width;
#pragma unroll
          for (int m = 0; m < MTF; ++m)
#pragma unroll
            for (int sh = 0; sh < 2; ++sh) {
              const half8_t d = pack_plain(acc[m][q], sh);
              const uint32_t f0 = 32 * m + 16 * sh;
              if (f0 < args.in_width) {
                *(half4_t*)(row + f0 + 4 * h) = half4_t{d[0], d[1], d[2], d[3]};
                *(half4_t*)(row + f0 + 8 + 4 * h) = half4_t{d[4], d[5], d[6], d[7]};
              }
            }
        }
      }
    }
  }
  };
  if (CAN_GLOBAL && wglobal) run(args.packedT); else run((const half_t*)lds);
}

struct WGradArgs {
  const half_t* features;
  const half_t* acts;
  const half_t* d_all;
  const half_t* dy;
  float* slab;
  uint32_t n, nh, in_width, n_mlp;
};

constexpr int kWgStage = 64;
constexpr int kWgStages = 4;

template <int W, int NT>
__global__ void __launch_bounds__(256) weight_grad_mfma_kernel(const WGradArgs args, uint32_t layer_lo)
{
  typedef MlpShape<W> Sh;
  constexpr int MT = Sh::MT;
  constexpr int DS = W + 8;
  constexpr int DC = W / 8;
  constexpr int DQ = (kWgStage * DC + 255) / 256;
  constexpr int XS = 32 * NT + 8;
  constexpr int XC = 4 * NT;
  constexpr int XQ = (kWgStage * XC + 255) / 256;
  __shared__ __attribute__((aligned(16))) half_t sd[kWgStage * DS];
  __shared__ __attribute__((aligned(16))) half_t sx[kWgStage * XS];
  __shared__ float red[3 * 16 * 64];
  const uint32_t layer = layer_lo + blockIdx.y;
  const uint32_t n = args.n, nh = args.nh;
  const uint32_t blk0 = blockIdx.x * (uint32_t)(kWgStage * kWgStages);
  if (blk0 >= n) return;
  const uint32_t blk_end = min(n, blk0 + (uint32_t)(kWgStage * kWgStages));
  float* slab = args.slab + (size_t)blockIdx.x * args.n_mlp;
  const size_t first_sz = (size_t)W * args.in_width;

  if (layer == nh + 1) {
    constexpr uint32_t CH = W / 8, SL = 256 / CH, ROWS = (kWgStage * kWgStages) / SL;
    const uint32_t c = threadIdx.x % CH, sr = threadIdx.x / CH;
    float acc[8] = {0, 0, 0, 0, 0, 0, 0, 0};
// ... 1118 lines not shown
```

instantvnr_amd/csrc/pack_rays.h:

```cpp
#pragma once
#include "common.h"

namespace vnr {

struct RayList {
  uint32_t* pixel_index;
  float* jitter;
  float* alpha;
  vec3f* color;
  vec3i* cell;
  vec3f* t_next;
  float* next_cell_begin;
  uint32_t* sample_base;
  uint32_t* sample_count;
};

struct SshLists {
  vec3f* org[2];
  vec3f* color[2];
  float* alpha[2];
};

enum { C_RAYS0 = 0, C_RAYS1 = 1, C_SAMPLES0 = 2, C_SAMPLES1 = 3, C_HIT = 4, C_STAT_SAMPLES = 6, C_STAT_REFRAYS = 8, C_COUNT = 16 };

struct PackArgs {
  RayList src, dst;
  const uint32_t* ray_counts;
  uint32_t n_first;
  uint32_t* counters;
  int parity, first, ssh, grad;
  SshLists ssh_lists;
  uint32_t* host_alive;
  uint32_t* host_stats;
  uint32_t n_blocks;
};

#if defined(__HIPCC__)
template <int WAVES>
__device__ __forceinline__ void pack_rays_block(const PackArgs& a, uint32_t item, uint32_t* s_part)
{
  constexpr uint32_t T = 64u * WAVES;
  const uint32_t tid = threadIdx.x, lane = tid & 63u, wave = tid >> 6;
  uint32_t* counters = a.counters;
  const int parity = a.parity;
  const uint32_t n_in = a.first ? a.n_first : counters[C_RAYS0 + parity];
  const uint32_t n_groups = ((n_in + 255u) & ~255u) >> 6;
  if (item == 0 && tid == 0) counters[C_SAMPLES0 + (parity ^ 1)] = 0;
  if (n_groups == 0) {
    if (item == 0 && tid == 0) { counters[C_RAYS0 + (parity ^ 1)] = 0; *a.host_alive = 0; }
    if (item == 0 && tid >= C_HIT && tid < C_COUNT) a.host_stats[tid] = counters[tid];
    return;
  }
  const uint32_t g0 = item * (uint32_t)WAVES;
  if (g0 >= n_groups) return;
  const uint32_t* __restrict__ ray_counts = a.ray_counts;
  uint32_t sum = 0;
  for (uint32_t g = tid; g < g0; g += T) sum += ray_counts[g] & 0xffu;
#pragma unroll
  for (int d = 32; d > 0; d >>= 1) sum += __shfl_xor(sum, d);
  if (lane == 0) s_part[wave] = sum;
  __syncthreads();
  uint32_t before = 0;
#pragma unroll
  for (int w = 0; w < WAVES; ++w) before += s_part[w];
  const uint32_t mine = (lane < (uint32_t)WAVES && g0 + lane < n_groups) ? ray_counts[g0 + lane] & 0xffu : 0u;
  uint32_t incl = mine;
#pragma unroll
  for (int d = 1; d < WAVES; d <<= 1) {
    const uint32_t y = __shfl_up(incl, d);
    if ((int)lane >= d) incl += y;
  }
  const uint32_t count = __shfl(mine, (int)wave), base = before + __shfl(incl, (int)wave) - count;
  const uint32_t block_total = __shfl(incl, WAVES - 1);
  const bool last_block = g0 + (uint32_t)WAVES >= n_groups;
  if (last_block && tid == 0) { counters[C_RAYS0 + (parity ^ 1)] = before + block_total; *a.host_alive = before + block_total; }
  if (lane < count) {
    const RayList& src = a.src;
    const RayList& dst = a.dst;
    const uint32_t from = ((g0 + wave) << 6) + lane, to = base + lane;
    dst.pixel_index[to] = src.pixel_index[from];
    dst.jitter[to] = src.jitter[from];
    dst.alpha[to] = src.alpha[from];
    dst.color[to] = src.color[from];
    dst.cell[to] = src.cell[from];
    dst.t_next[to] = src.t_next[from];
    dst.next_cell_begin[to] = src.next_cell_begin[from];
    dst.sample_base[to] = src.sample_base[from];
    dst.sample_count[to] = src.sample_count[from];
    if (a.ssh) {
      const SshLists& sl = a.ssh_lists;
      sl.org[0][to] = sl.org[1][from]; sl.color[0][to] = sl.color[1][from]; sl.alpha[0][to] = sl.alpha[1][from];
    }
  }
  if (last_block) {
    uint32_t asum = 0;
    for (uint32_t g = tid; g < n_groups; g += T) asum += ray_counts[g] >> 8;
#pragma unroll
    for (int d = 32; d > 0; d >>= 1) asum += __shfl_xor(asum, d);
    __syncthreads();
    if (lane == 0) s_part[wave] = asum;
    __syncthreads();
    if (tid == 0) {
      uint32_t alive_total = 0;
      for (int w = 0; w < WAVES; ++w) alive_total += s_part[w];
      const uint32_t records = counters[C_SAMPLES0 + parity];
      unsigned long long* c64 = (unsigned long long*)counters;
      c64[C_STAT_SAMPLES / 2] += (unsigned long long)(a.grad ? records >> 2 : records);
      c64[C_STAT_REFRAYS / 2] += (unsigned long long)alive_total;
      if (a.first) counters[C_HIT] += alive_total;
    }
    __syncthreads();
    if (tid >= C_HIT && tid < C_COUNT) a.host_stats[tid] = ((volatile uint32_t*)counters)[tid];
  }
}
#endif

}
```

instantvnr_amd/csrc/render.hip:

```cpp
#include "renderer.h"

#include <algorithm>
#include <cfloat>
#include <cstdlib>

#include "dist.h"
#include "infer_tile.h"
#include "pack_rays.h"
#include "sampling_device.h"
#include "march_device.h"
#include "pt_device.h"

namespace vnr {

template <bool FIRST, int MODE>
__global__ void __launch_bounds__(256) march_kernel(const RenderParams p, const RayList cur, const RayList nxt,
                                                    const vec2f* __restrict__ vd_in, vec4f* __restrict__ queue,
                                                    vec2f* __restrict__ vd_out, uint32_t* __restrict__ counters,
                                                    uint32_t* __restrict__ ray_counts, int parity, const SshLists ssh_lists,
                                                    uint32_t* __restrict__ tail_flag)
{
  extern __shared__ float s_t[];
  float* s_t0 = s_t;
  float* s_t1 = s_t + (size_t)p.n_iters * 256;
  uint32_t* s_hist = (uint32_t*)(s_t + (size_t)2 * p.n_iters * 256);
  uint32_t* s_claim = s_hist + 256;
  DeviceTfn tfn = p.tfn;
  constexpr bool GRAD = MODE == M_GRADIENT;
  tfn_lds_colors_t lds_colors = nullptr;
  tfn_lds_alphas_t lds_alphas = nullptr;
  bool tfn_merged = false;
  if (!FIRST && p.tfn_in_lds) {
    vec4f* s_colors = (vec4f*)(s_claim + 16);
    float* s_alphas = (float*)(s_colors + p.tfn.n_colors);
    tfn_merged = tfn_tables_to_lds(p.tfn, s_colors, s_alphas, !(dbg(p) & 32u));
    __syncthreads();
    lds_colors = (tfn_lds_colors_t)s_colors;
    lds_alphas = (tfn_lds_alphas_t)s_alphas;
  }
  const uint32_t tid = threadIdx.x, lane = tid & 63u;
  const uint32_t n_in = FIRST ? p.n_local : counters[C_RAYS0 + parity];
  uint32_t* n_samples_out = counters + C_SAMPLES0 + parity;
  const uint32_t n_round = (n_in + 255u) & ~255u;
  const unsigned long long lt_mask = (1ull << lane) - 1ull;
  uint32_t trip = 0;

  for (uint32_t base = blockIdx.x * 256u; base < n_round; base += gridDim.x * 256u) {
    const uint32_t i = base + tid;
    const bool active = i < n_in;
    uint32_t pixel = 0;
    float jitter = 0.0f, alpha = 0.0f;
    vec3f color = {0, 0, 0};
    DDAState it;
    it.t_next = {0, 0, 0}; it.cell = {0, 0, 0}; it.next_cell_begin = 0.0f;
    vec3f org = {0, 0, 0}, dir = {0, 0, 1}, m_dir = {0, 0, 1};
    float tmin = 0.0f, tmax = VNR_FLOAT_LARGE;
    bool alive = false;
    vec3f h_org = {0, 0, 0}, h_color = {0, 0, 0};
    float h_alpha = 0.0f;

    auto finish = [&]() {
      if (MODE == M_SSH) {
        p.px_org[pixel] = h_org; p.px_color[pixel] = h_color; p.px_alpha[pixel] = h_alpha;
        p.px_shading[pixel] = {color.x, color.y, color.z, alpha};
      } else if (MODE == M_SHADOW) {
        const float transmittance = 1.0f - alpha, k = 0.95f;
        vec4f sc = p.px_shading[pixel];
        const vec3f hc = p.px_color[pixel];
        sc.x = (1.0f - k) * sc.x + k * (hc.x * sc.w * transmittance);
        sc.y = (1.0f - k) * sc.y + k * (hc.y * sc.w * transmittance);
        sc.z = (1.0f - k) * sc.z + k * (hc.z * sc.w * transmittance);
        write_pixel(p, sc, pixel);
      } else {
        write_pixel(p, {color.x, color.y, color.z, alpha}, pixel);
      }
    };

    if (active) {
      if (FIRST) {
        if (map_pixel(p, i, pixel)) {
          if (MODE == M_SHADOW) {
            jitter = p.px_jitter[pixel];
            org = p.px_org[pixel];
            dir = p.shadow_dir;
            color = org;
            m_dir = dir * p.mc_rcp;
            alive = intersect_box(tmin, tmax, org, dir, p.bbox_lo, p.bbox_hi) && p.px_alpha[pixel] > 0.0f;
            if (alive) dda_init(it, org * p.mc_rcp, m_dir, tmin, p.mc_dims);
            else write_pixel(p, p.px_shading[pixel], pixel);
          } else {
            if (MODE == M_SSH) {
              float j2;
              const uint32_t state2 = tea_lcg_two((uint32_t)p.frame_index, pixel, jitter, j2);
              p.px_jitter[pixel] = p.ssh_third_draw ? (float)((1664525u * state2 + 1013904223u) & 0x00FFFFFFu) / (float)0x01000000 : j2;
            } else {
              jitter = tea_lcg_first((uint32_t)p.frame_index, pixel);
            }
            compute_ray(p, pixel, org, dir);
            m_dir = dir * p.mc_rcp;
            alive = intersect_box(tmin, tmax, org, dir, p.bbox_lo, p.bbox_hi);
            if (alive) dda_init(it, org * p.mc_rcp, m_dir, tmin, p.mc_dims);
            else if (MODE == M_SSH) finish();
            else write_pixel(p, {0, 0, 0, 0}, pixel);
          }
        }
      } else {
        pixel = cur.pixel_index[i];
        jitter = cur.jitter[i];
        alpha = cur.alpha[i];
        color = cur.color[i];
        it.cell = cur.cell[i];
        it.t_next = cur.t_next[i];
        it.next_cell_begin = cur.next_cell_begin[i];
        const uint32_t sb = cur.sample_base[i], sc = cur.sample_count[i];
        if (MODE == M_SHADOW) { org = color; dir = p.shadow_dir; }
        else compute_ray(p, pixel, org, dir);
        if (MODE == M_SSH) { h_org = ssh_lists.org[0][i]; h_color = ssh_lists.color[0][i]; h_alpha = ssh_lists.alpha[0][i]; }
        m_dir = dir * p.mc_rcp;
        intersect_box(tmin, tmax, org, dir, p.bbox_lo, p.bbox_hi);
        constexpr uint32_t kChunk = 8;
        const uint32_t sc_eff = (dbg(p) & 1u) ? 0u : sc;
        bool saturated = false;
        vec2f ahead[kChunk];
#pragma unroll
        for (uint32_t j = 0; j < kChunk; ++j) ahead[j] = vd_in[sb + 64u * min(j, sc - 1u)];
        for (uint32_t k0 = 0; k0 < sc_eff && !saturated; k0 += kChunk) {
          vec2f chunk[kChunk];
#pragma unroll
          for (uint32_t j = 0; j < kChunk; ++j) chunk[j] = ahead[j];
#pragma unroll
          for (uint32_t j = 0; j < kChunk; ++j) ahead[j] = vd_in[sb + 64u * min(k0 + kChunk + j, sc - 1u)];
          vec3f crgb[kChunk]; float ca[kChunk];
#pragma unroll
          for (uint32_t j = 0; j < kChunk; ++j) {
            if (dbg(p) & 2u) { crgb[j] = {0.5f, 0.5f, 0.5f}; ca[j] = chunk[j].x * 0.01f; }
            else if (p.tfn_in_lds) tfn_sample_lds(tfn, lds_colors, lds_alphas, chunk[j].x, crgb[j], ca[j], tfn_merged);
            else tfn_sample(tfn, chunk[j].x, crgb[j], ca[j]);
            ca[j] = opacity_correction(p.step_rcp, chunk[j].y, ca[j]);
          }
#pragma unroll
          for (uint32_t j = 0; j < kChunk; ++j) {
            const uint32_t k = k0 + j;
            if (k >= sc_eff) break;
            vec3f rgb = crgb[j]; float a = ca[j];
            const vec2f vd = chunk[j];
            if (GRAD) {
              const vec4f fg = *(const vec4f*)((const float*)vd_in + arena_grad_index(p.slot_cap, sb + 64u * k));
              vec3f stp = p.grad_step;
              if (p.grad_flip) {
                const vec3f c = org + fg.w * dir;
                if (c.x + stp.x > 1.0f - FLT_EPSILON) stp.x *= -1.0f;
                if (c.y + stp.y > 1.0f - FLT_EPSILON) stp.y *= -1.0f;
                if (c.z + stp.z > 1.0f - FLT_EPSILON) stp.z *= -1.0f;
              }
              rgb = gradient_shade(p, dir, vd.x, fg.x, fg.y, fg.z, stp, rgb);
            }
            if (MODE == M_SSH && h_alpha < (1.0f - alpha) * a) {
              const float t = ((const float*)vd_in)[arena_grad_index(p.slot_cap, sb + 64u * k)];
              h_org = org + t * dir;
              h_color = rgb;
              h_alpha = (1.0f - alpha) * a;
            }
            const float tr = 1.0f - alpha;
            alpha += tr * a;
            if (MODE != M_SHADOW) { color.x += tr * rgb.x * a; color.y += tr * rgb.y * a; color.z += tr * rgb.z * a; }
            if (!(alpha < VNR_NEARLY_ONE)) { saturated = true; break; }
          }
        }
        alive = (alpha < VNR_NEARLY_ONE) && dda_resumable(it, m_dir, tmin, tmax, p.mc_dims);
        if (!alive) finish();
      }
    }

    uint32_t k = 0;
    if (alive && !(dbg(p) & 8u)) {
      const int n_iters = p.n_iters;
      iter_exec(p, it, m_dir, tmin, tmax, p.step, [&](float t0, float t1) -> bool {
        s_t0[k * 256u + tid] = t0;
        s_t1[k * 256u + tid] = t1;
        return (int)(++k) < n_iters;
      });
      if (k == 0) finish();
    }
    const bool survive = alive && k > 0;

    const unsigned long long mask = __ballot(survive);
    const unsigned long long alive_mask = __ballot(alive);
    uint32_t incl = k;
#pragma unroll
    for (int d = 1; d < 64; d <<= 1) {
      const uint32_t y = __shfl_up(incl, d);
      if ((int)lane >= d) incl += y;
    }
    const uint32_t wave_samples = __shfl(incl, 63);
    const uint32_t wave_rays = (uint32_t)__popcll(mask);
    if (tail_flag && lane == 0 && wave_rays) *tail_flag = 1u;
    const uint32_t group = i >> 6;
    uint32_t* claim = s_claim + 8u * (trip & 1u);
    if (lane == 0) {
      ray_counts[group] = wave_rays | ((uint32_t)__popcll(alive_mask) << 8);
      claim[tid >> 6] = wave_samples;
    }
    __syncthreads();
    if (tid == 0) {
      const uint32_t total = claim[0] + claim[1] + claim[2] + claim[3];
      uint32_t b = 0;
      if (total) b = GRAD ? atomicAdd(n_samples_out, 4u * total) >> 2 : atomicAdd(n_samples_out, total);
      claim[4] = b;
    }
    __syncthreads();
    uint32_t smp_base = claim[4];
    for (uint32_t w = 0; w < (tid >> 6); ++w) smp_base += claim[w];
    ++trip;
    if (wave_rays == 0 || (dbg(p) & 16u)) continue;

    float front = survive ? s_t0[tid] : VNR_FLOAT_LARGE;
#pragma unroll
    for (int d = 32; d > 0; d >>= 1) front = fminf(front, __shfl_xor(front, d));
    uint32_t* hist = s_hist + (tid & ~63u);
    hist[lane] = 0;
    __builtin_amdgcn_wave_barrier();
    if (survive) {
      for (uint32_t j = 0; j < k; ++j) {
        const float t0 = s_t0[j * 256u + tid], t1 = s_t1[j * 256u + tid];
        const float t = (1.0f - jitter) * t0 + jitter * t1;
        atomicAdd(&hist[depth_bin(p, t, front)], 1u);
      }
    }
    __builtin_amdgcn_wave_barrier();
    const uint32_t h = hist[lane];
    uint32_t hs = h;
#pragma unroll
    for (int d = 1; d < 64; d <<= 1) {
      const uint32_t y = __shfl_up(hs, d);
      if ((int)lane >= d) hs += y;
    }
    hist[lane] = smp_base + hs - h;
    __builtin_amdgcn_wave_barrier();

    if (survive) {
      const uint32_t slot = (group << 6) + (uint32_t)__popcll(mask & lt_mask);
      const uint32_t sb = group * (uint32_t)p.n_iters * 64u + lane;
      nxt.pixel_index[slot] = pixel;
      nxt.jitter[slot] = jitter;
      nxt.alpha[slot] = alpha;
      nxt.color[slot] = color;
      nxt.cell[slot] = it.cell;
      nxt.t_next[slot] = it.t_next;
      nxt.next_cell_begin[slot] = it.next_cell_begin;
      nxt.sample_base[slot] = sb;
      nxt.sample_count[slot] = k;
      if (MODE == M_SSH) { ssh_lists.org[1][slot] = h_org; ssh_lists.color[1][slot] = h_color; ssh_lists.alpha[1][slot] = h_alpha; }
      for (uint32_t j = 0; j < k; ++j) {
        const float t0 = s_t0[j * 256u + tid], t1 = s_t1[j * 256u + tid];
        const float t = (1.0f - jitter) * t0 + jitter * t1;
        const vec3f c = org + t * dir;
        const uint32_t g = atomicAdd(&hist[depth_bin(p, t, front)], 1u);
        if (GRAD) {
          const uint32_t gi = arena_grad_index(p.slot_cap, sb + 64u * j);
          vec4f* q = queue + 4u * (size_t)g;
          vec3f stp = p.grad_step;
          if (p.grad_flip) {
            if (c.x + stp.x > 1.0f - FLT_EPSILON) stp.x *= -1.0f;
            if (c.y + stp.y > 1.0f - FLT_EPSILON) stp.y *= -1.0f;
            if (c.z + stp.z > 1.0f - FLT_EPSILON) stp.z *= -1.0f;
            ((float*)vd_out)[gi + 3u] = t;
          }
          q[0] = {c.x, c.y, c.z, __uint_as_float(arena_value_index(sb + 64u * j))};
          q[1] = {c.x + stp.x, c.y, c.z, __uint_as_float(gi + 0u)};
          q[2] = {c.x, c.y + stp.y, c.z, __uint_as_float(gi + 1u)};
          q[3] = {c.x, c.y, c.z + stp.z, __uint_as_float(gi + 2u)};
        } else {
          if (g < p.slot_cap) queue[g] = {c.x, c.y, c.z, __uint_as_float(arena_value_index(sb + 64u * j))};
        }
        vd_out[sb + 64u * j].y = t1 - t0;
        if (MODE == M_SSH) ((float*)vd_out)[arena_grad_index(p.slot_cap, sb + 64u * j)] = t;
      }
    }
    __builtin_amdgcn_wave_barrier();
  }
}


__global__ void gt_sample_kernel(const uint32_t* __restrict__ n_ptr, const float* __restrict__ vol, vec3i dims,
                                 const vec4f* __restrict__ queue, float* __restrict__ arena)
{
  const uint32_t n = *n_ptr;
  for (uint32_t i = blockIdx.x * blockDim.x + threadIdx.x; i < n; i += gridDim.x * blockDim.x) {
    const vec4f r = queue[i];
    arena[__float_as_uint(r.w)] = sample_volume_nodal(vol, dims, r.x, r.y, r.z);
  }
}

template <int WAVES>
__global__ void __launch_bounds__(64 * WAVES) compact_rays_kernel(const PackArgs a)
{
  __shared__ uint32_t s_part[WAVES];
  pack_rays_block<WAVES>(a, blockIdx.x, s_part);
}

__global__ void monolithic_kernel(const RenderParams p)
{
  const uint32_t i = blockIdx.x * blockDim.x + threadIdx.x;
  if (i >= p.n_local) return;
  uint32_t pixel;
  if (!map_pixel(p, i, pixel)) return;
  vec3f org, dir;
  compute_ray(p, pixel, org, dir);
  float alpha = 0.0f;
  vec3f color = {0, 0, 0};
  vec3f h_org = {0, 0, 0}, h_color = {0, 0, 0};
  float h_alpha = 0.0f;

  auto march = [&](vec3f o, vec3f d, float t0, float t1, float jitter, float step, bool shadow) {
    const vec3f m_dir = d * p.mc_rcp;
    DDAState it;
    dda_init(it, o * p.mc_rcp, m_dir, t0, p.mc_dims);
    auto cell_fn = [&](vec3i cell, float c0, float c1) -> bool {
      const float r = opacity_upper_bound(p, cell);
      if (fabsf(r) <= FLT_EPSILON) return true;
      float ss = adaptive_sampling_rate(step, r);
      {
        const int N = (int)((c1 - c0) / ss + 1.0f);
        ss = (c1 - c0) / (float)N;
      }
      float tx = c0, ty = fminf(c1, c0 + ss);
      while (ty > tx) {
        const float t = (1.0f - jitter) * tx + jitter * ty;
        const vec3f c = o + t * d;
        const float v = sample_volume_nodal(p.volume, p.vol_dims, c.x, c.y, c.z);
        vec3f rgb; float a;
        tfn_sample(p.tfn, v, rgb, a);
        a = opacity_correction(p.step_rcp, ty - tx, a);
        if (shadow) {
          alpha += (1.0f - alpha) * a;
          if (!(alpha < VNR_NEARLY_ONE)) return false;
          tx = ty;
          ty = fminf(tx + ss, c1);
          continue;
        }
        if (p.shading_mode == 1u) {
          vec3f stp = p.grad_step;
          if (c.x + stp.x > 1.0f - FLT_EPSILON) stp.x *= -1.0f;
          if (c.y + stp.y > 1.0f - FLT_EPSILON) stp.y *= -1.0f;
          if (c.z + stp.z > 1.0f - FLT_EPSILON) stp.z *= -1.0f;
          const float fgx = sample_volume_nodal(p.volume, p.vol_dims, c.x + stp.x, c.y, c.z);
          const float fgy = sample_volume_nodal(p.volume, p.vol_dims, c.x, c.y + stp.y, c.z);
          const float fgz = sample_volume_nodal(p.volume, p.vol_dims, c.x, c.y, c.z + stp.z);
          rgb = gradient_shade(p, d, v, fgx, fgy, fgz, stp, rgb);
        }
        if (p.shading_mode == 2u && h_alpha < (1.0f - alpha) * a) {
          h_org = c; h_color = rgb; h_alpha = (1.0f - alpha) * a;
        }
        const float tr = 1.0f - alpha;
        color.x += tr * rgb.x * a; color.y += tr * rgb.y * a; color.z += tr * rgb.z * a;
        alpha += tr * a;
        if (!(alpha < VNR_NEARLY_ONE)) return false;
        tx = ty;
        ty = fminf(tx + ss, c1);
      }
      return true;
    };
    if (t0 < t1) {
      const vec3i stop = {m_dir.x > 0.0f ? p.mc_dims.x : -1, m_dir.y > 0.0f ? p.mc_dims.y : -1, m_dir.z > 0.0f ? p.mc_dims.z : -1};
      const vec3f ts = {fabsf(1.0f / m_dir.x), fabsf(1.0f / m_dir.y), fabsf(1.0f / m_dir.z)};
      const vec3i delta = {m_dir.x > 0.0f ? 1 : -1, m_dir.y > 0.0f ? 1 : -1, m_dir.z > 0.0f ? 1 : -1};
      for (;;) {
        const float t_closest = min3f(it.t_next.x, it.t_next.y, it.t_next.z);
        const float c0 = fmaxf(t0 + it.next_cell_begin, t0), c1 = fminf(t0 + t_closest, t1);
        if (c0 >= c1) break;
        if (!cell_fn(it.cell, c0, c1)) break;
        if (it.t_next.x == t_closest) { it.t_next.x += ts.x; it.cell.x += delta.x; if (it.cell.x == stop.x) break; }
        if (it.t_next.y == t_closest) { it.t_next.y += ts.y; it.cell.y += delta.y; if (it.cell.y == stop.y) break; }
        if (it.t_next.z == t_closest) { it.t_next.z += ts.z; it.cell.z += delta.z; if (it.cell.z == stop.z) break; }
        it.next_cell_begin = t_closest;
      }
    }
  };

  float t0 = 0.0f, t1 = VNR_FLOAT_LARGE;
  if (intersect_box(t0, t1, org, dir, p.bbox_lo, p.bbox_hi)) {
    float jitter, unused;
    tea_lcg_two((uint32_t)p.frame_index, pixel, jitter, unused);
    march(org, dir, t0, t1, jitter, p.step, false);
    if (p.shading_mode == 2u && h_alpha > 0.0f) {
      const float pixel_alpha = alpha;
      float s0 = 0.0f, s1 = VNR_FLOAT_LARGE;
      alpha = 0.0f;
      if (intersect_box(s0, s1, h_org, p.shadow_dir, p.bbox_lo, p.bbox_hi)) {
        uint32_t v0 = (uint32_t)p.frame_index, v1 = pixel, s = 0;
#pragma unroll
        for (int n = 0; n < 16; ++n) {
          s += 0x9e3779b9u;
          v0 += ((v1 << 4) + 0xa341316cu) ^ (v1 + s) ^ ((v1 >> 5) + 0xc8013ea4u);
          v1 += ((v0 << 4) + 0xad90777du) ^ (v0 + s) ^ ((v0 >> 5) + 0x7e95761eu);
        }
        uint32_t st = 1664525u * v0 + 1013904223u;
        st = 1664525u * st + 1013904223u;
        st = 1664525u * st + 1013904223u;
        const float j3 = (float)(st & 0x00FFFFFFu) / (float)0x01000000;
        march(h_org, p.shadow_dir, s0, s1, j3, 2.0f * p.step, true);
      }
      const float transmittance = 1.0f - alpha, k = 0.95f;
      alpha = pixel_alpha;
      color.x = (1.0f - k) * color.x + k * (h_color.x * alpha * transmittance);
      color.y = (1.0f - k) * color.y + k * (h_color.y * alpha * transmittance);
      color.z = (1.0f - k) * color.z + k * (h_color.z * alpha * transmittance);
    }
  }
  write_pixel(p, {color.x, color.y, color.z, alpha}, pixel);
}

template <bool FIRST>
__global__ void __launch_bounds__(256) pt_kernel(const RenderParams p, const PtRays dense, const PtRays scratch, const float* __restrict__ values,
                                                 uint32_t* __restrict__ counters, uint32_t* __restrict__ ray_counts, int parity)
{
  const uint32_t tid = threadIdx.x, lane = tid & 63u;
  const uint32_t n_in = FIRST ? p.n_local : counters[C_RAYS0 + parity];
  const uint32_t n_round = (n_in + 255u) & ~255u;
  const unsigned long long lt_mask = (1ull << lane) - 1ull;
  for (uint32_t base = blockIdx.x * 256u; base < n_round; base += gridDim.x * 256u) {
    const uint32_t i = base + tid;
    PtRay r;
    bool alive = false, finished = false;
    if (i < n_in) {
      if (FIRST) {
        uint32_t pixel;
        if (map_pixel(p, i, pixel)) {
          r.pidx = pixel; r.shadow = false;
          compute_ray(p, pixel, r.org, r.dir);
          r.tnear = 0.0f; r.tfar = VNR_FLOAT_LARGE;
          r.scatter_index = 0; r.sample_coord = {0, 0, 0}; r.majorant = 0.0f;
          r.L = {0, 0, 0}; r.throughput = {1, 1, 1};
          {
            uint32_t v0 = (uint32_t)p.frame_index, v1 = pixel, s0 = 0;
#pragma unroll
            for (int n = 0; n < 16; ++n) {
              s0 += 0x9e3779b9u;
              v0 += ((v1 << 4) + 0xa341316cu) ^ (v1 + s0) ^ ((v1 >> 5) + 0xc8013ea4u);
              v1 += ((v0 << 4) + 0xad90777du) ^ (v0 + s0) ^ ((v0 >> 5) + 0x7e95761eu);
            }
            r.rng = v0;
          }
          r.it.t_next = {0, 0, 0}; r.it.cell = {0, 0, 0}; r.it.next_cell_begin = 0.0f;
          if (intersect_box(r.tnear, r.tfar, r.org, r.dir, p.bbox_lo, p.bbox_hi)) {
            atomicAdd(counters + C_HIT, 1u);
            dda_init(r.it, r.org * p.mc_rcp, r.dir * p.mc_rcp, r.tnear, p.mc_dims);
            alive = pt_take_sample(p, r);
          }
          finished = !alive;
        }
      } else {
        r.load(dense, i);
        r.tnear = 0.0f; r.tfar = VNR_FLOAT_LARGE;
        intersect_box(r.tnear, r.tfar, r.org, r.dir, p.bbox_lo, p.bbox_hi);
        alive = pt_shade(p, p.tfn, r, values[i]) && pt_take_sample(p, r);
        finished = !alive;
      }
    }
    if (finished) write_pixel(p, {r.L.x, r.L.y, r.L.z, 1.0f}, r.pidx);
    const unsigned long long mask = __ballot(alive);
    const uint32_t group = i >> 6;
    if (lane == 0) ray_counts[group] = (uint32_t)__popcll(mask);
    if (alive) r.store(scratch, (group << 6) + (uint32_t)__popcll(mask & lt_mask));
  }
}

__global__ void pt_monolithic_kernel(const RenderParams p)
{
  const uint32_t i = blockIdx.x * blockDim.x + threadIdx.x;
  if (i >= p.n_local) return;
  uint32_t pixel;
  if (!map_pixel(p, i, pixel)) return;
  PtRay r;
  r.pidx = pixel; r.shadow = false;
  compute_ray(p, pixel, r.org, r.dir);
  r.tnear = 0.0f; r.tfar = VNR_FLOAT_LARGE;
  r.scatter_index = 0; r.majorant = 0.0f; r.sample_coord = {0, 0, 0};
  r.L = {0, 0, 0}; r.throughput = {1, 1, 1};
  {
    uint32_t v0 = (uint32_t)p.frame_index, v1 = pixel, s0 = 0;
#pragma unroll
    for (int n = 0; n < 16; ++n) {
      s0 += 0x9e3779b9u;
      v0 += ((v1 << 4) + 0xa341316cu) ^ (v1 + s0) ^ ((v1 >> 5) + 0xc8013ea4u);
      v1 += ((v0 << 4) + 0xad90777du) ^ (v0 + s0) ^ ((v0 >> 5) + 0x7e95761eu);
    }
    r.rng = v0;
  }
  while (intersect_box(r.tnear, r.tfar, r.org, r.dir, p.bbox_lo, p.bbox_hi)) {
    float t = r.tnear;
    vec3f albedo = {0, 0, 0};
    bool found = false;
    dda_init(r.it, r.org * p.mc_rcp, r.dir * p.mc_rcp, r.tnear, p.mc_dims);
    while (pt_hashit(p, r, t)) {
      const vec3f c = r.org + t * r.dir;
      const float v = sample_volume_nodal(p.volume, p.vol_dims, c.x, c.y, c.z);
      vec3f rgb; float a;
      tfn_sample(p.tfn, v, rgb, a);
      if (r.next_float() * r.majorant < a * p.density_scale) { albedo = rgb; found = true; break; }
    }
    const bool exited = !found;
    if (r.shadow) {
      if (exited) r.L = r.L + r.throughput;
      r.tnear = 0.0f; r.tfar = VNR_FLOAT_LARGE;
      const float s0 = r.next_float(), s1 = r.next_float();
      r.dir = xfm_vector(p.wto, pt_uniform_sample_sphere(s0, s1));
      r.shadow = false;
    } else {
      if (exited) {
        if (r.scatter_index > 0u) r.L = r.L + 1.5f * r.throughput;
        break;
      }
      if (r.scatter_index > 4u) {
        const float q = fminf(0.95f, max3f(r.throughput.x, r.throughput.y, r.throughput.z));
        if (r.next_float() > q) break;
        r.throughput = {r.throughput.x / q, r.throughput.y / q, r.throughput.z / q};
      }
      ++r.scatter_index;
      r.org = r.org + t * r.dir;
      r.throughput = r.throughput * (0.6f * albedo);
      r.tnear = 0.0f; r.tfar = VNR_FLOAT_LARGE;
      r.dir = p.shadow_dir;
      r.shadow = true;
    }
  }
  write_pixel(p, {r.L.x, r.L.y, r.L.z, 1.0f}, pixel);
}

__global__ void __launch_bounds__(1024) pt_compact_kernel(const PtRays src, const PtRays dst, const uint32_t* __restrict__ ray_counts,
                                                          uint32_t n_first, uint32_t* __restrict__ counters, int parity, int first,
                                                          vec4f* __restrict__ queue)
{
  __shared__ uint32_t s_part[16];
  const uint32_t tid = threadIdx.x, lane = tid & 63u, wave = tid >> 6;
  const uint32_t n_in = first ? n_first : counters[C_RAYS0 + parity];
  const uint32_t n_groups = ((n_in + 255u) & ~255u) >> 6;
  if (n_groups == 0) {
    if (blockIdx.x == 0 && tid == 0) counters[C_RAYS0 + (parity ^ 1)] = 0;
    return;
  }
  const uint32_t g0 = blockIdx.x * 16u;
  if (g0 >= n_groups) return;
  uint32_t sum = 0;
  for (uint32_t g = tid; g < g0; g += 1024u) sum += ray_counts[g];
#pragma unroll
  for (int d = 32; d > 0; d >>= 1) sum += __shfl_xor(sum, d);
  if (lane == 0) s_part[wave] = sum;
  __syncthreads();
  uint32_t before = 0;
#pragma unroll
  for (int w = 0; w < 16; ++w) before += s_part[w];
  const uint32_t mine = (lane < 16u && g0 + lane < n_groups) ? ray_counts[g0 + lane] : 0u;
  uint32_t incl = mine;
#pragma unroll
  for (int d = 1; d < 16; d <<= 1) {
    const uint32_t y = __shfl_up(incl, d);
    if ((int)lane >= d) incl += y;
  }
  const uint32_t count = __shfl(mine, (int)wave), base = before + __shfl(incl, (int)wave) - count;
  const uint32_t block_total = __shfl(incl, 15);
  if (g0 + 16u >= n_groups && tid == 0) {
    const uint32_t total = before + block_total;
    counters[C_RAYS0 + (parity ^ 1)] = total;
    atomicAdd((unsigned long long*)(counters + C_STAT_SAMPLES), (unsigned long long)total);
  }
  if (lane < count) {
    const uint32_t from = ((g0 + wave) << 6) + lane, to = base + lane;
#pragma unroll
    for (int k = 0; k < kPtPlanes; ++k) dst.base[(size_t)k * dst.stride + to] = src.base[(size_t)k * src.stride + from];
    queue[to] = {src.base[(size_t)8 * src.stride + from], src.base[(size_t)9 * src.stride + from], src.base[(size_t)10 * src.stride + from],
                 __uint_as_float(to)};
  }
}

}
#include "in_shader.h"
#include "decoupled.h"
namespace vnr {

struct PartState {
  RenderParams p;
  RayList rl[2];
  SshLists ssh;
  vec4f* queue;
  vec2f* vd[2];
  uint32_t* c;
  uint32_t* rc;
  uint32_t* hc;
  uint32_t* hs;
  hipStream_t s;
  size_t s_max;
  uint32_t it = 0, used = 0;
  bool done = false;
  bool tail_skipped = false;
  hipEvent_t ev_done = nullptr;
};

struct DPart {
  RenderParams p;
  DRays rays;
  DRing ring[8];
  DHost* host = nullptr;
  hipStream_t sw = nullptr, se = nullptr, sc = nullptr;
  std::vector<hipEvent_t> ev_w, ev_e, ev_c;
  uint32_t it_w = 0, it_c = 0, target = 0;
  size_t s_max = 0;
  bool done = false;
  hipEvent_t& ev(std::vector<hipEvent_t>& v, uint32_t it)
  {
    if (it >= 1024u) throw std::runtime_error("internal: decoupled loop asked for the event of iteration " + std::to_string(it));
    while (v.size() <= it) { hipEvent_t e; VNR_HIP_CHECK(hipEventCreateWithFlags(&e, hipEventDisableTiming)); v.push_back(e); }
    return v[it];
  }
  ~DPart() { for (auto* v : {&ev_w, &ev_e, &ev_c}) for (hipEvent_t e : *v) (void)hipEventDestroy(e); }
};

struct Renderer::StreamingFrame {
  bool pending = false;
  bool decoupled = false;
  int ahead = 2, ring = 3;
  DPart dpart[Renderer::kMaxParts];
  int slot = 0;
  int H = 0, pass_mode = 0;
  bool grad = false, ssh = false;
  NeuralVolume* nv = nullptr;
  size_t shmem = 0, shmem_compose = 0;
  uint32_t max_iterations = 240;
  uint32_t* predicted = nullptr;
  RenderParams p_all;
  uint64_t params_generation = 0;
  PartState part[Renderer::kMaxParts];
  StreamingFrame()
  {
    for (auto& p : part) {
      (void)hipEventCreateWithFlags(&p.ev_done, hipEventDisableTiming);
    }
  }
  ~StreamingFrame() { for (auto& p : part) if (p.ev_done) (void)hipEventDestroy(p.ev_done); }
  void mark(int h) { VNR_HIP_CHECK(hipEventRecord(part[h].ev_done, part[h].s)); }
};

Renderer::Renderer(std::shared_ptr<VolumeBase> volume) : volume_(std::move(volume))
{
  if (!Runtime::get().ready()) Runtime::get().init(-1);
  stream_ = Runtime::get().stream;
  if (const char* e = std::getenv("VNR_RM_N_ITERS")) { n_iters_ = std::max(1, std::min(48, std::atoi(e))); n_iters_fixed_ = true; }
  if (const char* e = std::getenv("VNR_AMD_RENDER_HALVES")) { n_halves_ = std::max(1, std::min(kMaxParts, std::atoi(e))); n_halves_fixed_ = true; }
  if (const char* e = std::getenv("VNR_AMD_SMALL_SHARE_PARTS")) small_share_parts_ = std::max(1, std::min(kMaxParts, std::atoi(e)));
  if (const char* e = std::getenv("VNR_AMD_TILE_W")) {
    const int w = std::atoi(e);
    tile_w_log2_ = w == 16 ? 4u : w == 32 ? 5u : w == 64 ? 6u : 3u;
  }
  if (const char* e = std::getenv("VNR_AMD_DECOUPLED")) decoupled_mode_ = std::max(0, std::min(2, std::atoi(e)));
  if (const char* e = std::getenv("VNR_AMD_DECOUPLED_AHEAD")) decoupled_ahead_ = std::max(1, std::min(7, std::atoi(e)));
  if (const char* e = std::getenv("VNR_AMD_DECOUPLED_PARTS")) decoupled_parts_ = std::max(1, std::min(kMaxParts, std::atoi(e)));
  counters_.resize(2 * kMaxParts * C_COUNT);
  counters_.zero(stream_);
  VNR_HIP_CHECK(hipHostMalloc((void**)&host_counts_, 2 * kMaxParts * (256 + C_COUNT) * sizeof(uint32_t), hipHostMallocDefault));
  VNR_HIP_CHECK(hipEventCreateWithFlags(&ev_fork_, hipEventDisableTiming));
}

Renderer::~Renderer()
{
  if (stream_) (void)hipStreamSynchronize(stream_);
  for (int i = 1; i < kMaxParts; ++i) if (part_streams_[i]) (void)hipStreamSynchronize(part_streams_[i]);
  if (ev_fork_) (void)hipEventDestroy(ev_fork_);
  for (auto& ps : d_streams_) for (hipStream_t st : ps) if (st) { (void)hipStreamSynchronize(st); (void)hipStreamDestroy(st); }
  frame_[0].reset(); frame_[1].reset();
  if (d_host_) (void)hipHostFree(d_host_);
  if (distributed_) (void)hipStreamSynchronize(Dist::get().comm_stream());
  if (ev_rendered_) (void)hipEventDestroy(ev_rendered_);
  for (int i = 0; i < 2; ++i) if (ev_gathered_[i]) (void)hipEventDestroy(ev_gathered_[i]);
  for (int i = 0; i < 2; ++i) if (host_fb_[i]) (void)hipHostFree(host_fb_[i]);
  if (host_counts_) (void)hipHostFree(host_counts_);
  for (auto& sl : events_) for (auto& v : sl) for (auto e : v) (void)hipEventDestroy(e);
}

void Renderer::resize(int w, int h)
{
  finish_pending();
  if (w <= 0 || h <= 0) throw std::runtime_error("invalid framebuffer size");
  VNR_HIP_CHECK(hipDeviceSynchronize());
  width_ = w; height_ = h;
  const size_t n = (size_t)w * h;
  for (int i = 0; i < 2; ++i) { fb_[i].resize(n); fb_[i].zero(stream_); }
  accumulation_.resize(n);
  accumulation_.zero(stream_);
  if (host_fb_pixels_ != n) {
    for (int i = 0; i < 2; ++i) {
      if (host_fb_[i]) (void)hipHostFree(host_fb_[i]);
      VNR_HIP_CHECK(hipHostMalloc((void**)&host_fb_[i], n * sizeof(vec4f), hipHostMallocDefault));
      std::memset(host_fb_[i], 0, n * sizeof(vec4f));
    }
    host_fb_pixels_ = n;
  }
  if (distributed_) ensure_share_buffers();
  reset_ = true;
}

__global__ void assemble_shares_kernel(const vec4f* __restrict__ gathered, vec4f* __restrict__ full, uint32_t width, uint32_t height,
                                       uint32_t world, uint32_t n_local)
{
  const uint32_t n = width * height;
  for (uint32_t i = blockIdx.x * blockDim.x + threadIdx.x; i < n; i += gridDim.x * blockDim.x) {
    const uint32_t y = i / width, x = i - y * width, b = y >> 3;
    full[i] = gathered[(size_t)(b % world) * n_local + ((b / world) * 8u + (y & 7u)) * width + x];
  }
}

void Renderer::set_distributed(bool e)
{
  finish_pending();
  if (e && !Dist::get().active()) throw std::runtime_error("distributed rendering needs vnrAmdDistInitFromEnv / vnrAmdDistInit first");
  distributed_ = e && Dist::get().world() >= 1;
  pipe_prev_ = -1;
  if (distributed_) {
    if (!ev_rendered_) VNR_HIP_CHECK(hipEventCreateWithFlags(&ev_rendered_, hipEventDisableTiming));
    for (int i = 0; i < 2; ++i) if (!ev_gathered_[i]) VNR_HIP_CHECK(hipEventCreateWithFlags(&ev_gathered_[i], hipEventDisableTiming));
    ensure_share_buffers();
  }
  reset_ = true;
}

void Renderer::ensure_share_buffers()
{
  if (width_ <= 0 || height_ <= 0) return;
  const Dist& d = Dist::get();
  const ShareLayout l = share_layout((uint32_t)width_, (uint32_t)height_, (uint32_t)d.world());
  share_world_ = (uint32_t)d.world(); share_rank_ = (uint32_t)d.rank(); share_n_local_ = l.n_local;
  VNR_HIP_CHECK(hipStreamSynchronize(stream_));
  VNR_HIP_CHECK(hipStreamSynchronize(Dist::get().comm_stream()));
  const size_t n = (size_t)width_ * height_;
  for (int i = 0; i < 2; ++i) {
    gathered_[i].resize((size_t)share_world_ * l.n_local);
    gathered_[i].zero(stream_);
    full_[i].resize(n);
    full_[i].zero(stream_);
    gather_issued_[i] = false;
  }
  if (accumulation_.count < l.n_local) { accumulation_.resize(l.n_local); accumulation_.zero(stream_); }
  VNR_HIP_CHECK(hipStreamSynchronize(stream_));
}

void Renderer::issue_gather(int buf)
{
  if (gather_issued_[buf]) return;
  Dist& d = Dist::get();
  hipStream_t comm = d.comm_stream();
  const int fslot = frame_of_buffer_[buf];
  if (fslot >= 0 && frame_[fslot]) {
    for (int h = 0; h < frame_[fslot]->H; ++h) VNR_HIP_CHECK(hipStreamWaitEvent(comm, frame_[fslot]->part[h].ev_done, 0));
  } else {
    VNR_HIP_CHECK(hipEventRecord(ev_rendered_, stream_));
    VNR_HIP_CHECK(hipStreamWaitEvent(comm, ev_rendered_, 0));
  }
  vec4f* g = gathered_[buf].ptr;
  const size_t share_bytes = (size_t)share_n_local_ * sizeof(vec4f);
  d.transport().all_gather(g + (size_t)share_rank_ * share_n_local_, g, share_bytes, comm);
  const uint32_t n = (uint32_t)((size_t)width_ * height_);
  assemble_shares_kernel<<<std::min<uint32_t>(div_round_up(n, 256), (uint32_t)Runtime::get().n_cus * 8u), 256, 0, comm>>>(
      g, full_[buf].ptr, (uint32_t)width_, (uint32_t)height_, share_world_, share_n_local_);
  VNR_HIP_CHECK(hipGetLastError());
  if (!skip_download_) VNR_HIP_CHECK(hipMemcpyAsync(host_fb_[buf], full_[buf].ptr, (size_t)n * sizeof(vec4f), hipMemcpyDeviceToHost, comm));
  VNR_HIP_CHECK(hipEventRecord(ev_gathered_[buf], comm));
  gather_issued_[buf] = true;
}

const float* Renderer::render_pipelined()
{
  const int cur = fb_cur_;
  const bool was_async = async_, was_skip = skip_download_;
  async_ = true;
  if (!distributed_) skip_download_ = true;
  try { render(); } catch (...) { async_ = was_async; skip_download_ = was_skip; throw; }
  async_ = was_async; skip_download_ = was_skip;
  const float* out = nullptr;
  const int prev = pipe_prev_;
  if (prev >= 0) {
    StreamingFrame* older = frame_[slot_ ^ 1].get();
    if (older && older->pending) finish_streaming(*older);
    out = hand_out_frame(prev);
  }
  pipe_prev_ = cur;
  fb_cur_ ^= 1;
  return out;
}

const float* Renderer::flush_pipeline()
{
  if (pipe_prev_ < 0) return nullptr;
  finish_pending();
  const int prev = pipe_prev_;
  pipe_prev_ = -1;
  return hand_out_frame(prev);
}

const float* Renderer::hand_out_frame(int buf)
{
  if (distributed_) {
    issue_gather(buf);
    VNR_HIP_CHECK(hipEventSynchronize(ev_gathered_[buf]));
    return skip_download_ ? (const float*)full_[buf].ptr : (const float*)host_fb_[buf];
  }
  if (skip_download_) return (const float*)fb_[buf].ptr;
  const size_t n = (size_t)width_ * height_;
  VNR_HIP_CHECK(hipMemcpy(host_fb_[buf], fb_[buf].ptr, n * sizeof(vec4f), hipMemcpyDeviceToHost));
  return (const float*)host_fb_[buf];
}

void Renderer::set_transfer_function(const TransferFunctionData& t)
{
  finish_pending();
  volume_->set_transfer_function(t, stream_);
  tfn_.set(t, volume_->desc.range_lo, volume_->desc.range_hi, stream_);
  reset_ = true;
}

void Renderer::ensure_queues(size_t n_pixels, int n_iters, bool gradient)
{
  if (queue_pixels_ >= n_pixels && queue_iters_ >= n_iters && (queue_grad_ || !gradient)) return;
  finish_pending();
  VNR_HIP_CHECK(hipDeviceSynchronize());
  const size_t P = std::max(n_pixels, queue_pixels_);
  const int iters = std::max(n_iters, queue_iters_);
  const bool grad = gradient || queue_grad_;
  q_u32_.resize(2 * 6 * P);
  ray_counts_.resize(2 * (P / 64 + 64 + 8 * kMaxParts));
  q_f32_.resize(2 * 18 * P);
  q_i32_.resize(2 * 6 * P);
  queue_.resize(2 * P * iters * (grad ? 4 : 1));
  arena_.resize(2 * 2 * P * iters * (grad ? 6 : 2));
  queue_pixels_ = P;
  queue_iters_ = iters;
  queue_grad_ = grad;
}

void Renderer::finish_pending()
{
  for (int k = 1; k <= 2; ++k) {
    StreamingFrame* f = frame_[(slot_ + k) & 1].get();
    if (f && f->pending) finish_streaming(*f);
  }
}

void Renderer::render()
{
  const bool in_shader = in_shader_applies();
  const bool pipeline_head = async_ && (skip_download_ || distributed_) && (mode_ == 5 || mode_ == 6 || mode_ == 8 || mode_ == 9) && !in_shader &&
                             frame_[slot_] && frame_[slot_]->pending && !(frame_[slot_ ^ 1] && frame_[slot_ ^ 1]->pending) &&
                             !reset_;
  if (!pipeline_head) finish_pending();
  if (width_ <= 0 || height_ <= 0) return;
  MacroCell& mc = volume_->macrocell();
  if (!mc.allocated()) throw std::runtime_error("volume has no macrocell");
  RenderParams p;
  p.width = width_; p.height = height_;
  const uint32_t n_pixels = (uint32_t)((size_t)width_ * height_);
  p.pixel_lo = std::min(pixel_lo_, n_pixels);
  p.pixel_hi = std::min(pixel_hi_, n_pixels);
  if (p.pixel_hi < p.pixel_lo) p.pixel_hi = p.pixel_lo;
  if (distributed_) { il_block_ = 8u * (uint32_t)width_; il_parts_ = share_world_; il_part_ = share_rank_; }
  if (il_parts_ > 1 && il_block_ != 8u * (uint32_t)width_) throw std::runtime_error("pixel interleave block must be 8 scanlines (8 * width pixels)");
  p.il_parts = il_parts_; p.il_part = il_part_;
  p.out_parts = distributed_ ? share_world_ : 1u;
  p.tile_w_log2 = tile_w_log2_;
  p.tiles_per_row = div_round_up((uint32_t)width_, 1u << p.tile_w_log2) << (p.tile_w_log2 - 3u);
  const uint32_t tr_lo = p.pixel_hi > p.pixel_lo ? (p.pixel_lo / (uint32_t)width_) / 8u : 0u;
  const uint32_t tr_hi = p.pixel_hi > p.pixel_lo ? ((p.pixel_hi - 1u) / (uint32_t)width_) / 8u + 1u : 0u;
  p.tile_row0 = il_parts_ == 1 ? tr_lo : 0u;
  const uint32_t rows_local = il_parts_ == 1 ? (tr_hi - tr_lo) : div_round_up(div_round_up((uint32_t)height_, 8), il_parts_);
  p.n_local = rows_local * p.tiles_per_row * 64u;
  p.debug_flags = 0;
#if defined(VNR_DIAG)
  if (const char* e = std::getenv("VNR_AMD_DEBUG_FLAGS")) p.debug_flags = (uint32_t)std::atoi(e);
#endif
  constexpr float kBinDepth = 8.0f;
  p.bin_depth_rcp = 1.0f / kBinDepth;
  const float t = 2.0f * tanf(camera_.fovy * 0.5f * (float)M_PI / 180.0f);
  const float aspect = (float)width_ / (float)height_;
  p.cam_pos = camera_.from;
  p.cam_dir = normalize(camera_.at - camera_.from);
  p.cam_hor = (t * aspect) * normalize(cross(p.cam_dir, camera_.up));
  p.cam_ver = (1.0f / aspect) * cross(p.cam_hor, p.cam_dir);
  p.wto = affine_inverse(volume_->transform);
  p.vol_dims = volume_->desc.dims;
  p.volume = volume_->is_network() ? static_cast<NeuralVolume*>(volume_.get())->decoded_data()
                                   : static_cast<SimpleVolume*>(volume_.get())->d_data();
  p.bbox_lo = volume_->clipbox.lower; p.bbox_hi = volume_->clipbox.upper;
  {
    auto finite3 = [](vec3f v) { return std::isfinite(v.x) && std::isfinite(v.y) && std::isfinite(v.z); };
    if (!finite3(p.cam_pos) || !finite3(p.cam_dir) || !finite3(p.cam_hor) || !finite3(p.cam_ver))
      throw std::runtime_error("degenerate camera: position, focus, up vector and field of view do not span an image plane "
                               "(from == at, up along the view direction, or a value that is not finite)");
    if (!finite3(p.wto.vx) || !finite3(p.wto.vy) || !finite3(p.wto.vz) || !finite3(p.wto.p))
      throw std::runtime_error("degenerate volume transform: the object-to-world matrix is singular or not finite");
    if (!finite3(p.bbox_lo) || !finite3(p.bbox_hi)) throw std::runtime_error("clipping box is not finite");
    if (!std::isfinite(density_scale_)) throw std::runtime_error("volume density scale is not finite");
  }
  p.step = 1.0f / sampling_rate_; p.step_rcp = sampling_rate_;
  p.mc_dims = mc.dims();
  const vec3f sp = mc.spacings();
  p.mc_rcp = {1.0f / sp.x, 1.0f / sp.y, 1.0f / sp.z};
  p.mc_max_opacity = mc.d_max_opacity();
  p.tfn = tfn_.view();
  p.tfn_in_lds = ((size_t)p.tfn.n_colors * sizeof(vec4f) + (size_t)p.tfn.n_alphas * sizeof(float)) <= 24 * 1024 ? 1u : 0u;
  p.n_iters = (!n_iters_fixed_ && (distributed_ || il_parts_ > 1) && p.n_local <= 262144u) ? 32 : n_iters_;
  p.otw = volume_->transform;
  p.grad_step = {1.0f / (float)p.vol_dims.x, 1.0f / (float)p.vol_dims.y, 1.0f / (float)p.vol_dims.z};
  if (dot(p.cam_dir, light_dir_) > 0.0f) light_dir_ = -1.0f * light_dir_;
  p.light_dir = light_dir_;
  p.shading_mode = (mode_ == 7 || mode_ == 8 || mode_ == 9) ? 1u : (mode_ == 10 || mode_ == 11 || mode_ == 12) ? 2u : 0u;
  p.grad_flip = mode_ == 9 ? 1u : 0u;
  p.pt_reset_interval = mode_ == 15 ? 1u : 0u;
  p.ssh_third_draw = mode_ == 12 ? 1u : 0u;
  p.slot_cap = 0;
  p.shadow_dir = xfm_vector(p.wto, normalize(light_dir_));
  p.density_scale = density_scale_;
  p.px_org = nullptr; p.px_color = nullptr; p.px_alpha = nullptr; p.px_shading = nullptr; p.px_jitter = nullptr;
  if (mode_ == 11 || mode_ == 12) {
    ssh_px_.ensure(12 * (size_t)n_pixels);
    float* b = ssh_px_.ptr;
    p.px_org = (vec3f*)b; p.px_color = (vec3f*)(b + 3 * (size_t)n_pixels); p.px_alpha = b + 6 * (size_t)n_pixels;
    p.px_jitter = b + 7 * (size_t)n_pixels; p.px_shading = (vec4f*)(b + 8 * (size_t)n_pixels);
  }
  if (reset_) frame_index_ = 0;
  ++frame_index_;
  p.frame_index = frame_index_;
  p.frame = fb_[fb_cur_].ptr;
  if (distributed_) {
    if (gather_issued_[fb_cur_]) VNR_HIP_CHECK(hipStreamWaitEvent(stream_, ev_gathered_[fb_cur_], 0));
    gather_issued_[fb_cur_] = false;
    p.frame = gathered_[fb_cur_].ptr + (size_t)share_rank_ * share_n_local_;
  }
  p.accumulation = accumulation_.ptr;
  if (!pipeline_head) stats_ = FrameStats();

  frame_of_buffer_[fb_cur_] = -1;
  if (p.pixel_hi > p.pixel_lo && p.n_local > 0) {
    if (in_shader) {
      render_in_shader(p, mode_ == 9 ? M_GRADIENT : mode_ == 12 ? M_SSH : (mode_ == 14 || mode_ == 15) ? kInShaderPathTracing : M_NONE);
    } else
    switch (mode_) {
    case 6:
    case 9:
    case 5:
    case 8:
      render_streaming(p, p.shading_mode == 1u ? M_GRADIENT : M_NONE, async_ && (skip_download_ || distributed_));
      break;
    case 11:
      render_streaming(p, M_SSH);
      render_streaming(p, M_SHADOW);
      break;
    case 15:
    case 14:
      render_pathtracing(p);
      break;
    case 13:
      if (!p.volume)
        throw std::runtime_error(volume_->is_network() ? "rendering mode 13 traces the decoded volume: call vnrNeuralVolumeDecodeProgressive first (GetNumberOfBlobs calls = one full pass)"
                                                       : "this volume has no resident data to sample");
      pt_monolithic_kernel<<<div_round_up(p.n_local, 128), 128, 0, stream_>>>(p);
      VNR_HIP_CHECK(hipGetLastError());
      break;
    case 12: {
      render_streaming(p, M_SSH);
      RenderParams q = p;
      q.step = 2.0f * p.step;
      render_streaming(q, M_SHADOW);
      break;
    }
    case 4:
    case 7:
    case 10:
      if (volume_->is_network() && !p.volume)
        throw std::runtime_error("rendering mode " + std::to_string(mode_) +
                                 " marches the decoded volume: call vnrNeuralVolumeDecodeProgressive first (GetNumberOfBlobs calls = one full pass)");
      render_monolithic(p);
      break;
    default:
      throw std::runtime_error("rendering mode " + std::to_string(mode_) +
                               " is not implemented in this build (supported: ray marching 4 - 12 and path tracing 13 - 15; 0 - 3 are the OptiX modes)");
    }
  }
  reset_ = false;
  if (!(frame_[slot_] && frame_[slot_]->pending)) completed_stats_ = stats_;
  if (!skip_download_ && !distributed_) {
    const size_t off = p.pixel_lo, cnt = p.pixel_hi - p.pixel_lo;
    if (cnt) VNR_HIP_CHECK(hipMemcpyAsync(host_fb_[fb_cur_] + off, fb_[fb_cur_].ptr + off, cnt * sizeof(vec4f), hipMemcpyDeviceToHost, stream_));
  }
}

bool launch_in_shader_w16(const RenderParams&, const TileNet&, int, const InShaderLaunch&);
bool launch_in_shader_w32(const RenderParams&, const TileNet&, int, const InShaderLaunch&);
bool launch_in_shader_w64(const RenderParams&, const TileNet&, int, const InShaderLaunch&);
bool launch_in_shader_w128(const RenderParams&, const TileNet&, int, const InShaderLaunch&);
bool launch_in_shader_w16g(const RenderParams&, const TileNet&, int, const InShaderLaunch&);
bool launch_in_shader_w32g(const RenderParams&, const TileNet&, int, const InShaderLaunch&);
bool launch_in_shader_w64g(const RenderParams&, const TileNet&, int, const InShaderLaunch&);

bool Renderer::in_shader_applies() const
{
  if (mode_ != 6 && mode_ != 9 && mode_ != 12 && mode_ != 14 && mode_ != 15) return false;
  static const int env = [] { const char* e = std::getenv("VNR_AMD_IN_SHADER"); return e && (e[0] == '0' || e[0] == '1') ? e[0] - '0' : -1; }();
  const int choice = in_shader_mode_ >= 0 ? in_shader_mode_ : env;
  const bool want = choice >= 0 ? choice == 1 : (mode_ == 14 || mode_ == 15);
  if (!want || !volume_->is_network()) return false;
  const Network& net = static_cast<NeuralVolume*>(volume_.get())->network();
  if (!net.valid() || !net.weights_in_lds() || (size_t)net.lds_halves() * 2 + 64 > 160 * 1024) return false;
  if (net.width() == 128u && !net.common_kind()) return false;
  const uint32_t F = net.config().n_features, K = net.padded_width();
#define X(f, k) if (F == f && K == k) return true;
  VNR_IN_SHADER_SHAPES(X)
#undef X
  return false;
}

void Renderer::render_in_shader(const RenderParams& p, int shade)
{
  NeuralVolume* nv = static_cast<NeuralVolume*>(volume_.get());
  TileNet net;
  if (!nv->network().tile_net(&net, stream_)) throw std::runtime_error("internal: in-shader rendering of a model without an MFMA kernel");
  if (is_samples_.count == 0) { is_samples_.resize(kInShaderStatSlots); is_hits_.resize(kInShaderStatSlots); }
  is_samples_.zero(stream_);
  is_hits_.zero(stream_);
  InShaderLaunch l;
  l.blocks = div_round_up(p.n_local, 256);
  l.shmem = (size_t)net.lds_halves * sizeof(uint16_t);
  l.stream = stream_;
  l.stat_samples = is_samples_.ptr;
  l.stat_hits = is_hits_.ptr;
  bool launched = false;
  switch (net.width) {
  case 16: launched = net.general ? launch_in_shader_w16g(p, net, shade, l) : launch_in_shader_w16(p, net, shade, l); break;
  case 32: launched = net.general ? launch_in_shader_w32g(p, net, shade, l) : launch_in_shader_w32(p, net, shade, l); break;
  case 64: launched = net.general ? launch_in_shader_w64g(p, net, shade, l) : launch_in_shader_w64(p, net, shade, l); break;
  case 128: launched = !net.general && launch_in_shader_w128(p, net, shade, l); break;
  default: break;
  }
  if (!launched) throw std::runtime_error("internal: no in-shader instance for this model shape");
  VNR_HIP_CHECK(hipGetLastError());
  unsigned long long hs[kInShaderStatSlots];
  uint32_t hh[kInShaderStatSlots];
  VNR_HIP_CHECK(hipMemcpyAsync(hs, is_samples_.ptr, sizeof(hs), hipMemcpyDeviceToHost, stream_));
  VNR_HIP_CHECK(hipMemcpyAsync(hh, is_hits_.ptr, sizeof(hh), hipMemcpyDeviceToHost, stream_));
  VNR_HIP_CHECK(hipStreamSynchronize(stream_));
  for (int k = 0; k < kInShaderStatSlots; ++k) { stats_.n_samples += hs[k]; stats_.n_rays_hit += hh[k]; }
  stats_.n_reference_slots = stats_.n_samples;
  stats_.n_iterations = 1;
}

void Renderer::render_monolithic(const RenderParams& p)
{
  monolithic_kernel<<<div_round_up(p.n_local, 128), 128, 0, stream_>>>(p);
  VNR_HIP_CHECK(hipGetLastError());
}

void Renderer::render_pathtracing(const RenderParams& p)
{
  const uint32_t P = p.n_local;
  NeuralVolume* nv = volume_->is_network() ? static_cast<NeuralVolume*>(volume_.get()) : nullptr;
  if (nv && !nv->network().valid()) throw std::runtime_error("neural volume has no valid network");
  if (!nv && !p.volume) throw std::runtime_error("this volume has no resident data to sample");
  pt_rays_.ensure((size_t)2 * kPtPlanes * P);
  pt_values_.ensure(P);
  if (queue_.count < P) queue_.resize(P);
  ray_counts_.ensure(P / 64 + 64);
  const PtRays dense = {pt_rays_.ptr, P}, scratch = {pt_rays_.ptr + (size_t)kPtPlanes * P, P};
  uint32_t* c = counters_.ptr;
  hipStream_t s = stream_;
  VNR_HIP_CHECK(hipMemsetAsync(c, 0, C_COUNT * sizeof(uint32_t), s));
  const uint32_t blocks = std::min<uint32_t>(div_round_up(P, 256), 4096u);
  const uint32_t cblocks = div_round_up(P, 1024);
  uint32_t it = 0;
  auto launch = [&]() {
    const int parity = (int)(it & 1u);
    if (it == 0) {
      pt_kernel<true><<<blocks, 256, 0, s>>>(p, dense, scratch, pt_values_.ptr, c, ray_counts_.ptr, 0);
    } else {
      if (nv) nv->network().inference_queue((const float*)queue_.ptr, pt_values_.ptr, 1, c + C_RAYS0 + parity, P, s, 1);
      else gt_sample_kernel<<<std::min<uint32_t>(div_round_up(P, 256), (uint32_t)Runtime::get().n_cus * 8u), 256, 0, s>>>(
               c + C_RAYS0 + parity, p.volume, p.vol_dims, queue_.ptr, pt_values_.ptr);
      pt_kernel<false><<<blocks, 256, 0, s>>>(p, dense, scratch, pt_values_.ptr, c, ray_counts_.ptr, parity);
    }
    pt_compact_kernel<<<cblocks, 1024, 0, s>>>(scratch, dense, ray_counts_.ptr, P, c, parity, it == 0 ? 1 : 0, queue_.ptr);
    VNR_HIP_CHECK(hipGetLastError());
    VNR_HIP_CHECK(hipMemcpyAsync(host_counts_ + (it & 255u), c + C_RAYS0 + (parity ^ 1), sizeof(uint32_t), hipMemcpyDeviceToHost, s));
    ++it;
  };
  const uint32_t max_iterations = 1u << 16;
  while (it < std::max<uint32_t>(predicted_pt_, 1u)) launch();
  for (;;) {
    VNR_HIP_CHECK(hipStreamSynchronize(s));
    if (host_counts_[(it - 1) & 255u] == 0 || it >= max_iterations) break;
    for (int k = 0; k < 8; ++k) launch();
  }
  uint32_t used = it;
  if (it <= 256) { while (used > 1 && host_counts_[(used - 2) & 255u] == 0) --used; }
  predicted_pt_ = used;
  uint32_t hc[C_COUNT];
  VNR_HIP_CHECK(hipMemcpy(hc, c, sizeof(hc), hipMemcpyDeviceToHost));
  stats_.n_rays_hit += hc[C_HIT];
  const uint64_t n = (uint64_t)hc[C_STAT_SAMPLES] | ((uint64_t)hc[C_STAT_SAMPLES + 1] << 32);
  stats_.n_samples += n;
  stats_.n_reference_slots += n;
  stats_.n_iterations += used > 0 ? used - 1 : 0;
}

void Renderer::launch_iteration(StreamingFrame& f, int h)
{
  PartState* half = f.part;
  const int pass_mode = f.pass_mode;
  const size_t shmem = f.shmem, shmem_compose = f.shmem_compose;
  const uint32_t max_iterations = f.max_iterations;
  {
    PartState& hf = half[h];
    const uint32_t it = hf.it;
    const int parity = (int)(it & 1u);
    const uint32_t P = hf.p.n_local;
    uint32_t* c = hf.c;
    const hipStream_t s_it = hf.s;
    const bool skip_tail = it >= 1 && it + 1 == f.predicted[h] && it + 1 < max_iterations;
    uint32_t* tail_flag = nullptr;
    if (skip_tail) { hf.hs[0] = 0; tail_flag = hf.hs; }
    {
      const bool first = it == 0;
      const uint32_t blocks = std::min<uint32_t>(div_round_up(P, 256), first ? 4096u : 2048u);
      const size_t lds = first ? shmem : shmem_compose;
      const vec2f* vd_in = hf.vd[parity ^ 1];
      vec2f* vd_out = hf.vd[parity];
#define VNR_MARCH(FIRST_, MODE_) march_kernel<FIRST_, MODE_><<<blocks, 256, lds, s_it>>>(hf.p, hf.rl[0], hf.rl[1], vd_in, hf.queue, vd_out, c, hf.rc, parity, hf.ssh, tail_flag)
      switch (pass_mode) {
      case M_GRADIENT: if (first) VNR_MARCH(true, M_GRADIENT); else VNR_MARCH(false, M_GRADIENT); break;
      case M_SSH: if (first) VNR_MARCH(true, M_SSH); else VNR_MARCH(false, M_SSH); break;
      case M_SHADOW: if (first) VNR_MARCH(true, M_SHADOW); else VNR_MARCH(false, M_SHADOW); break;
      default: if (first) VNR_MARCH(true, M_NONE); else VNR_MARCH(false, M_NONE); break;
      }
#undef VNR_MARCH
    }
    VNR_HIP_CHECK(hipGetLastError());
    if (skip_tail) {
      if (profiling_) { VNR_HIP_CHECK(hipEventRecord(events_[f.slot][h][2 * it], hf.s)); VNR_HIP_CHECK(hipEventRecord(events_[f.slot][h][2 * it + 1], hf.s)); }
      hf.tail_skipped = true;
      ++hf.it;
      if (hf.it >= max_iterations) hf.done = true;
      return;
    }
  }
  {
    PartState& hf = half[h];
    const uint32_t it = hf.it;
    launch_tail(f, h, it, hf.s);
    ++hf.it;
    if (hf.it >= max_iterations) hf.done = true;
  }
}

void Renderer::launch_tail(StreamingFrame& f, int h, uint32_t it, hipStream_t s_it)
{
  PartState* half = f.part;
  const int H = f.H;
  const bool grad = f.grad, ssh = f.ssh;
  NeuralVolume* nv = f.nv;
  {
    PartState& hf = half[h];
    const int parity = (int)(it & 1u);
    const uint32_t P = hf.p.n_local;
    uint32_t* c = hf.c;
    PackArgs pk;
    pk.src = hf.rl[1]; pk.dst = hf.rl[0]; pk.ray_counts = hf.rc; pk.n_first = P; pk.counters = c; pk.parity = parity; pk.first = it == 0 ? 1 : 0;
    pk.ssh = ssh ? 1 : 0; pk.grad = grad ? 1 : 0; pk.ssh_lists = hf.ssh; pk.host_alive = hf.hc + (it & 255u); pk.host_stats = hf.hs;
    pk.n_blocks = div_round_up(P, 256);
    const bool fused_pack = P <= 262144u;
    bool packed = false;
    if (!s_it) s_it = hf.s;
    if (profiling_) VNR_HIP_CHECK(hipEventRecord(events_[f.slot][h][2 * it], s_it));
#if defined(VNR_DIAG)
    static const bool skip_eval = [] { const char* e = std::getenv("VNR_AMD_DEBUG_SKIP_EVAL"); return e && std::atoi(e) != 0; }();
#else
    constexpr bool skip_eval = false;
#endif
    if (skip_eval) {
    } else if (nv) {
      packed = nv->network().inference_queue((const float*)hf.queue, (float*)hf.vd[parity], 1, c + C_SAMPLES0 + parity, hf.s_max, s_it, (uint32_t)H,
                                             fused_pack ? &pk : nullptr);
    } else {
      const uint32_t blocks = std::min<uint32_t>(div_round_up(hf.s_max, 256), (uint32_t)Runtime::get().n_cus * 8u);
      gt_sample_kernel<<<blocks, 256, 0, s_it>>>(c + C_SAMPLES0 + parity, hf.p.volume, hf.p.vol_dims, hf.queue, (float*)hf.vd[parity]);
    }
    if (profiling_) VNR_HIP_CHECK(hipEventRecord(events_[f.slot][h][2 * it + 1], s_it));
    last_schedule_[2] = packed ? 1 : 0;
    if (!packed) {
      constexpr uint32_t kCompactSmallLimit = 262144u;
      if (P <= kCompactSmallLimit) {
        compact_rays_kernel<4><<<pk.n_blocks, 256, 0, s_it>>>(pk);
      } else {
        pk.n_blocks = div_round_up(P, 1024);
        compact_rays_kernel<16><<<pk.n_blocks, 1024, 0, s_it>>>(pk);
      }
    }
    VNR_HIP_CHECK(hipGetLastError());
  }
}

void Renderer::render_streaming(const RenderParams& p_all, int pass_mode, bool defer)
{
  if (decoupled_applies(p_all, pass_mode)) { render_decoupled(p_all, defer); return; }
  const uint32_t row_items = p_all.tiles_per_row * 64u;
  const uint32_t R = p_all.n_local / row_items;
  const int want = (!n_halves_fixed_ && p_all.n_local <= 524288u) ? small_share_parts_ : n_halves_;
  const int H = (int)std::min<uint32_t>((uint32_t)want, std::max(R, 1u));
  const uint32_t P_total = p_all.n_local;
  const bool grad = pass_mode == M_GRADIENT;
  const bool ssh = pass_mode == M_SSH;
  uint32_t* predicted = predicted_iterations_[pass_mode == M_SHADOW ? 1 : 0];
  ensure_queues(P_total, p_all.n_iters, grad || ssh || pass_mode == M_SHADOW);
  const size_t QP = queue_pixels_;
  if (ssh) q_ssh_.ensure(14 * QP);
  const size_t QI = (size_t)queue_iters_;
  const size_t slot_floats = queue_grad_ ? 6 : 2;
  const size_t rec_per_slot = queue_grad_ ? 4 : 1;
  if ((size_t)P_total * QI * 6 >= (1ull << 32)) throw std::runtime_error("frame share too large for 32-bit result indices");
  NeuralVolume* nv = volume_->is_network() ? static_cast<NeuralVolume*>(volume_.get()) : nullptr;
  if (nv && !nv->network().valid()) throw std::runtime_error("neural volume has no valid network");

  StreamingFrame* older = frame_[slot_] && frame_[slot_]->pending ? frame_[slot_].get() : nullptr;
  const int slot = older ? slot_ ^ 1 : slot_;
  if (!frame_[slot]) frame_[slot].reset(new StreamingFrame());
  StreamingFrame& f = *frame_[slot];
  if (f.pending) throw std::runtime_error("internal: both frame slots are pending");
  f.slot = slot;
  slot_ = slot;
  f.decoupled = false;
  PartState* half = f.part;
  for (int h = 0; h < kMaxParts; ++h) { half[h].it = 0; half[h].used = 0; half[h].done = false; half[h].tail_skipped = false; }
  const size_t n_groups_slot = QP / 64 + 64 + 8 * kMaxParts;
  uint32_t* const u32_base = q_u32_.ptr + (size_t)slot * 6 * QP;
  float* const f32_base = q_f32_.ptr + (size_t)slot * 18 * QP;
  int* const i32_base = q_i32_.ptr + (size_t)slot * 6 * QP;
  uint32_t* const rc_base = ray_counts_.ptr + (size_t)slot * n_groups_slot;
  vec4f* const queue_base = queue_.ptr + (size_t)slot * rec_per_slot * QP * QI;
  float* const arena_base = arena_.ptr + (size_t)slot * 2 * slot_floats * QP * QI;
  uint32_t* const counters_base = counters_.ptr + (size_t)slot * kMaxParts * C_COUNT;
  uint32_t* const host_base = host_counts_ + (size_t)slot * kMaxParts * (256 + C_COUNT);
  size_t off = 0;
  for (int h = 0; h < H; ++h) {
    PartState& hf = half[h];
    hf.p = p_all;
    if (H > 1) {
      hf.p.il_parts = p_all.il_parts * (uint32_t)H;
      hf.p.il_part = p_all.il_part + p_all.il_parts * (uint32_t)h;
      hf.p.n_local = ((R + (uint32_t)(H - 1 - h)) / (uint32_t)H) * row_items;
    }
    for (int b = 0; b < 2; ++b) {
      hf.rl[b].pixel_index = u32_base + (size_t)(0 + b) * QP + off;
      hf.rl[b].sample_base = u32_base + (size_t)(2 + b) * QP + off;
      hf.rl[b].sample_count = u32_base + (size_t)(4 + b) * QP + off;
      float* f = f32_base + (size_t)b * 9 * QP;
      hf.rl[b].jitter = f + off;
      hf.rl[b].alpha = f + QP + off;
      hf.rl[b].color = (vec3f*)(f + 2 * QP) + off;
      hf.rl[b].t_next = (vec3f*)(f + 5 * QP) + off;
      hf.rl[b].next_cell_begin = f + 8 * QP + off;
      hf.rl[b].cell = (vec3i*)(i32_base + (size_t)b * 3 * QP) + off;
      hf.ssh.org[b] = nullptr; hf.ssh.color[b] = nullptr; hf.ssh.alpha[b] = nullptr;
      if (ssh) {
        float* g = q_ssh_.ptr + (size_t)b * 7 * QP;
        hf.ssh.org[b] = (vec3f*)g + off;
        hf.ssh.color[b] = (vec3f*)(g + 3 * QP) + off;
        hf.ssh.alpha[b] = g + 6 * QP + off;
      }
      hf.vd[b] = (vec2f*)(arena_base + (size_t)b * slot_floats * QP * QI + slot_floats * off * QI);
    }
    hf.p.slot_cap = (uint32_t)((size_t)hf.p.n_local * QI);
    hf.queue = queue_base + rec_per_slot * off * QI;
    hf.c = counters_base + (size_t)h * C_COUNT;
    hf.rc = rc_base + off / 64 + (size_t)h * 8;
    hf.hc = host_base + (size_t)h * 256;
    hf.hs = host_base + kMaxParts * 256 + (size_t)h * C_COUNT;
    if (h > 0 && !part_streams_[h]) part_streams_[h] = Runtime::get().part_stream(h);
    hf.s = h == 0 ? stream_ : part_streams_[h];
    hf.s_max = (size_t)hf.p.n_local * hf.p.n_iters * (grad ? 4 : 1);
    off += hf.p.n_local;
  }

  f.params_generation = nv ? nv->network().params_generation() : 0;
  VNR_HIP_CHECK(hipMemsetAsync(counters_base, 0, (size_t)H * C_COUNT * sizeof(uint32_t), stream_));
  if (H > 1) {
    VNR_HIP_CHECK(hipEventRecord(ev_fork_, stream_));
    for (int h = 1; h < H; ++h) VNR_HIP_CHECK(hipStreamWaitEvent(part_streams_[h], ev_fork_, 0));
  }
  const size_t shmem = ((size_t)2 * p_all.n_iters + 1) * 256 * sizeof(float) + 16 * sizeof(uint32_t);
  const size_t shmem_compose = shmem + (p_all.tfn_in_lds ? (size_t)p_all.tfn.n_colors * sizeof(vec4f) + (size_t)p_all.tfn.n_alphas * sizeof(float) : 0);
  if (shmem_compose > 160 * 1024) throw std::runtime_error("VNR_RM_N_ITERS too large for the LDS of one workgroup");
  static bool lds_attr_set = false;
  if (!lds_attr_set) {
#define VNR_ATTR(FIRST_, MODE_) VNR_HIP_CHECK(hipFuncSetAttribute((const void*)march_kernel<FIRST_, MODE_>, hipFuncAttributeMaxDynamicSharedMemorySize, 160 * 1024))
    VNR_ATTR(true, M_NONE); VNR_ATTR(false, M_NONE); VNR_ATTR(true, M_GRADIENT); VNR_ATTR(false, M_GRADIENT);
    VNR_ATTR(true, M_SSH); VNR_ATTR(false, M_SSH); VNR_ATTR(true, M_SHADOW); VNR_ATTR(false, M_SHADOW);
#undef VNR_ATTR
    lds_attr_set = true;
  }
  uint32_t max_iterations = 240;
#if defined(VNR_DIAG)
  if (const char* e = std::getenv("VNR_AMD_DEBUG_MAX_ITERS")) max_iterations = std::max(1, std::min(240, std::atoi(e)));
#endif
  if (profiling_) {
    iter_ms_.assign(max_iterations, 0.0f);
    for (int h = 0; h < H; ++h)
      while (events_[slot][h].size() < 2 * max_iterations) { hipEvent_t e; VNR_HIP_CHECK(hipEventCreate(&e)); events_[slot][h].push_back(e); }
  }

  last_schedule_[0] = p_all.n_iters; last_schedule_[1] = H; last_schedule_[2] = 0; last_schedule_[3] = 0;
  f.H = H; f.pass_mode = pass_mode; f.grad = grad; f.ssh = ssh; f.nv = nv; f.shmem = shmem; f.shmem_compose = shmem_compose;
  f.max_iterations = max_iterations; f.predicted = predicted; f.p_all = p_all;
  if (older) {
    for (int h = 0; h < H; ++h) launch_iteration(f, h);
    finish_streaming(*older);
    stats_ = FrameStats();
  }
  frame_of_buffer_[fb_cur_] = slot;
  for (;;) {
    bool launched = false;
    for (int h = 0; h < H; ++h)
      if (!half[h].done && half[h].it < predicted[h]) { launch_iteration(f, h); launched = true; }
    if (!launched) break;
  }
  for (int h = 0; h < H; ++h) f.mark(h);
  f.pending = true;
  if (!defer) finish_streaming(f);
}

void Renderer::finish_streaming(StreamingFrame& f)
{
  if (!f.pending) return;
  if (f.decoupled) { finish_decoupled(f); return; }
  f.pending = false;
  PartState* half = f.part;
  const int H = f.H, pass_mode = f.pass_mode;
  uint32_t* predicted = f.predicted;
  const RenderParams& p_all = f.p_all;
  for (;;) {
    bool pending = false;
    for (int h = 0; h < H; ++h) {
      PartState& hf = half[h];
      if (hf.done) continue;
      if (hf.it > 0) {
        VNR_HIP_CHECK(hipEventSynchronize(hf.ev_done));
        if (hf.tail_skipped) {
          hf.tail_skipped = false;
          if (hf.hs[0] == 0) { hf.hc[(hf.it - 1) & 255u] = 0; hf.done = true; continue; }
          launch_tail(f, h, hf.it - 1, hf.s);
          f.mark(h);
          pending = true;
          continue;
        }
        if (hf.hc[(hf.it - 1) & 255u] == 0) { hf.done = true; continue; }
      }
      launch_iteration(f, h);
      f.mark(h);
      pending = true;
    }
    if (!pending) break;
  }

  uint32_t pass_iterations = 0;
  uint64_t n_samples = 0, n_refrays = 0;
  for (int h = 0; h < H; ++h) {
    PartState& hf = half[h];
    VNR_HIP_CHECK(hipEventSynchronize(hf.ev_done));
    uint32_t used = hf.it;
    while (used > 1 && hf.hc[(used - 2) & 255u] == 0) --used;
    predicted[h] = used;
    hf.used = used;
    const uint32_t* hc = hf.hs;
    if (pass_mode != M_SHADOW) stats_.n_rays_hit += hc[C_HIT];
    n_samples += (uint64_t)hc[C_STAT_SAMPLES] | ((uint64_t)hc[C_STAT_SAMPLES + 1] << 32);
    n_refrays += (uint64_t)hc[C_STAT_REFRAYS] | ((uint64_t)hc[C_STAT_REFRAYS + 1] << 32);
    pass_iterations = std::max<uint32_t>(pass_iterations, used > 0 ? used - 1 : 0);
    if (profiling_) stats_.infer_kernel_launches += used > 0 ? used - 1 : 0;
  }
  {
    uint32_t launched[kMaxParts] = {};
    for (int h = 0; h < H; ++h) launched[h] = half[h].it;
    collect_eval_profile(f, launched, nullptr);
  }
  stats_.n_iterations += pass_iterations;
  stats_.n_samples += n_samples;
  stats_.n_reference_slots += n_refrays * (uint64_t)p_all.n_iters;
  completed_stats_ = stats_;
}


void Renderer::collect_eval_profile(StreamingFrame& f, const uint32_t* launched, const uint32_t* )
{
  if (!profiling_) return;
  const int H = f.H;
  bool any = false;
  for (int h = 0; h < H; ++h) {
    for (uint32_t k = 0; k < launched[h]; ++k) {
      float ms = 0.0f;
      VNR_HIP_CHECK(hipEventElapsedTime(&ms, events_[f.slot][h][2 * k], events_[f.slot][h][2 * k + 1]));
      stats_.infer_kernel_ms += ms;
      if (k < iter_ms_.size()) iter_ms_[k] += ms;
      any = true;
    }
  }
  if (!any || launched[0] == 0) return;
  std::vector<std::pair<float, float>> iv;
  for (int h = 0; h < H; ++h)
    for (uint32_t k = 0; k < launched[h]; ++k) {
      float t0 = 0.0f, t1 = 0.0f;
      VNR_HIP_CHECK(hipEventElapsedTime(&t0, events_[f.slot][0][0], events_[f.slot][h][2 * k]));
      VNR_HIP_CHECK(hipEventElapsedTime(&t1, events_[f.slot][0][0], events_[f.slot][h][2 * k + 1]));
      iv.emplace_back(t0, t1);
    }
  std::sort(iv.begin(), iv.end());
  float lo = iv[0].first, hi = iv[0].second;
  double total = 0.0;
  for (size_t e = 1; e < iv.size(); ++e) {
    if (iv[e].first > hi) { total += hi - lo; lo = iv[e].first; hi = iv[e].second; }
    else hi = std::max(hi, iv[e].second);
  }
  stats_.infer_union_ms += total + (hi - lo);
}

bool Renderer::decoupled_applies(const RenderParams& p, int pass_mode) const
{
  if (pass_mode != M_NONE || decoupled_mode_ == 0) return false;
  if ((size_t)p.n_local * (size_t)p.n_iters >= (1ull << 28)) return false;
  return decoupled_mode_ == 2 || p.n_local <= 20480u;
}

void Renderer::render_decoupled(const RenderParams& p_all, bool defer)
{
  const uint32_t row_items = p_all.tiles_per_row * 64u;
  const uint32_t R = p_all.n_local / row_items;
  const int H = (int)std::min<uint32_t>((uint32_t)decoupled_parts_, std::max(R, 1u));
  const uint32_t P_total = p_all.n_local;
  const int A = decoupled_ahead_, RING = A + 1;
  last_schedule_[0] = p_all.n_iters; last_schedule_[1] = H; last_schedule_[2] = 0; last_schedule_[3] = 1;
  NeuralVolume* nv = volume_->is_network() ? static_cast<NeuralVolume*>(volume_.get()) : nullptr;
  if (nv && !nv->network().valid()) throw std::runtime_error("neural volume has no valid network");
  if (!nv && !p_all.volume) throw std::runtime_error("this volume has no resident data to sample");

  const size_t Pt = (size_t)P_total + 256u * kMaxParts;
  if (d_rays_ < Pt || d_iters_ < p_all.n_iters || d_ring_ < RING) {
    finish_pending();
    VNR_HIP_CHECK(hipDeviceSynchronize());
    d_rays_ = std::max(d_rays_, Pt); d_iters_ = std::max(d_iters_, p_all.n_iters); d_ring_ = std::max(d_ring_, RING);
    const size_t words = 15 * d_rays_ + (size_t)d_ring_ * d_rays_ + (size_t)d_ring_ * kMaxParts * D_COUNT;
    for (int sl = 0; sl < 2; ++sl) {
      d_words_[sl].resize(words);
      d_words_[sl].zero(stream_);
      d_queue_[sl].resize((size_t)d_ring_ * d_rays_ * d_iters_);
      d_arena_[sl].resize((size_t)d_ring_ * d_rays_ * d_iters_);
    }
    VNR_HIP_CHECK(hipStreamSynchronize(stream_));
  }
  if (!d_host_) {
    VNR_HIP_CHECK(hipHostMalloc(&d_host_, 2 * kMaxParts * sizeof(DHost), hipHostMallocDefault));
    std::memset(d_host_, 0, 2 * kMaxParts * sizeof(DHost));
  }
  int prio_least = 0, prio_greatest = 0;
  VNR_HIP_CHECK(hipDeviceGetStreamPriorityRange(&prio_least, &prio_greatest));
  for (int h = 0; h < H; ++h)
    for (int k = 0; k < 3; ++k)
      if (!d_streams_[h][k]) VNR_HIP_CHECK(hipStreamCreateWithPriority(&d_streams_[h][k], hipStreamNonBlocking, k == 1 ? prio_least : prio_greatest));

  StreamingFrame* older = frame_[slot_] && frame_[slot_]->pending ? frame_[slot_].get() : nullptr;
  const int slot = older ? slot_ ^ 1 : slot_;
  if (!frame_[slot]) frame_[slot].reset(new StreamingFrame());
  StreamingFrame& f = *frame_[slot];
  if (f.pending) throw std::runtime_error("internal: both frame slots are pending");
  f.slot = slot;
  slot_ = slot;
  f.decoupled = true; f.ahead = A; f.ring = RING;
  f.H = H; f.pass_mode = M_NONE; f.grad = false; f.ssh = false; f.nv = nv; f.p_all = p_all;
  f.shmem = ((size_t)2 * p_all.n_iters + 1) * 256 * sizeof(float) + 16 * sizeof(uint32_t) + (size_t)p_all.n_iters * 256 * sizeof(uint16_t);
  f.shmem_compose = p_all.tfn_in_lds ? (size_t)p_all.tfn.n_colors * sizeof(vec4f) + (size_t)p_all.tfn.n_alphas * sizeof(float) : 0;
  if (f.shmem > 160 * 1024) throw std::runtime_error("VNR_RM_N_ITERS too large for the LDS of one workgroup");
  f.max_iterations = 240;
#if defined(VNR_DIAG)
  if (const char* e = std::getenv("VNR_AMD_DEBUG_MAX_ITERS")) f.max_iterations = std::max(1, std::min(240, std::atoi(e)));
#endif
  static bool lds_attr_set = false;
  if (!lds_attr_set) {
    VNR_HIP_CHECK(hipFuncSetAttribute((const void*)walk_kernel<true>, hipFuncAttributeMaxDynamicSharedMemorySize, 160 * 1024));
    VNR_HIP_CHECK(hipFuncSetAttribute((const void*)walk_kernel<false>, hipFuncAttributeMaxDynamicSharedMemorySize, 160 * 1024));
    lds_attr_set = true;
  }
  if (profiling_) {
    iter_ms_.assign(f.max_iterations, 0.0f);
    for (int h = 0; h < H; ++h)
      while (events_[slot][h].size() < 2 * f.max_iterations) { hipEvent_t e; VNR_HIP_CHECK(hipEventCreate(&e)); events_[slot][h].push_back(e); }
  }

  uint32_t* w = d_words_[slot].ptr;
  uint32_t* const rec_base = w + 15 * d_rays_;
  uint32_t* const ctr_base = rec_base + (size_t)d_ring_ * d_rays_;
  size_t off = 0;
  for (int h = 0; h < H; ++h) {
    DPart& d = f.dpart[h];
    d.p = p_all;
    if (H > 1) {
      d.p.il_parts = p_all.il_parts * (uint32_t)H;
      d.p.il_part = p_all.il_part + p_all.il_parts * (uint32_t)h;
      d.p.n_local = ((R + (uint32_t)(H - 1 - h)) / (uint32_t)H) * row_items;
    }
    d.p.slot_cap = (uint32_t)((size_t)d.p.n_local * d.p.n_iters);
    const size_t Pr = ((size_t)d.p.n_local + 255u) & ~(size_t)255u;
    uint32_t* b = w + off;
    const size_t N = d_rays_;
    d.rays.pixel = b; d.rays.jitter = (float*)(b + N); d.rays.ncb = (float*)(b + 2 * N); d.rays.walking = b + 3 * N;
    d.rays.alpha = (float*)(b + 4 * N); d.rays.done = b + 5 * N;
    d.rays.cell = (vec3i*)(w + 6 * N) + off; d.rays.t_next = (vec3f*)(w + 9 * N) + off; d.rays.color = (vec3f*)(w + 12 * N) + off;
    for (int q = 0; q < RING; ++q) {
      d.ring[q].queue = d_queue_[slot].ptr + ((size_t)q * d_rays_ + off) * d_iters_;
      d.ring[q].arena = d_arena_[slot].ptr + ((size_t)q * d_rays_ + off) * d_iters_;
      d.ring[q].rec = rec_base + (size_t)q * d_rays_ + off;
      d.ring[q].ctr = ctr_base + ((size_t)q * kMaxParts + h) * D_COUNT;
    }
    d.host = (DHost*)d_host_ + (size_t)slot * kMaxParts + h;
    d.sw = d_streams_[h][0]; d.se = d_streams_[h][1]; d.sc = d_streams_[h][2];
    d.it_w = d.it_c = 0;
    d.target = std::max<uint32_t>(decoupled_predicted_[h], 1u);
    d.s_max = (size_t)d.p.n_local * d.p.n_iters;
    d.done = false;
    f.part[h].s = d.sc;
    off += Pr;
  }
  VNR_HIP_CHECK(hipEventRecord(ev_fork_, stream_));
  for (int h = 0; h < H; ++h)
    for (int k = 0; k < 3; ++k) VNR_HIP_CHECK(hipStreamWaitEvent(d_streams_[h][k], ev_fork_, 0));

  if (older) {
    for (bool any = true; any;) {
      any = false;
      for (int h = 0; h < H; ++h) { const uint32_t before = f.dpart[h].it_w; decoupled_step(f, h, true); any = any || f.dpart[h].it_w != before; }
    }
    finish_streaming(*older);
    stats_ = FrameStats();
  }
  frame_of_buffer_[fb_cur_] = slot;
  for (bool any = true; any;) {
    any = false;
    for (int h = 0; h < H; ++h) {
      DPart& d = f.dpart[h];
      const uint32_t bw = d.it_w, bc = d.it_c;
      decoupled_step(f, h, false);
      any = any || d.it_w != bw || d.it_c != bc;
    }
  }
  for (int h = 0; h < H; ++h) f.mark(h);
  f.pending = true;
  if (!defer) finish_streaming(f);
}

void Renderer::decoupled_step(StreamingFrame& f, int h, bool head_only)
{
  DPart& d = f.dpart[h];
  const uint32_t A = (uint32_t)f.ahead, RING = (uint32_t)f.ring;
  if (d.it_w < d.target && d.it_w < d.it_c + A) {
    const uint32_t it = d.it_w;
    const DRing& ring = d.ring[it % RING];
    if (it >= A) VNR_HIP_CHECK(hipStreamWaitEvent(d.sw, d.ev(d.ev_c, it - A), 0));
    const uint32_t P = d.p.n_local;
    const uint32_t blocks = std::min<uint32_t>(div_round_up(P, 256), 2048u);
    if (it == 0) walk_kernel<true><<<blocks, 256, f.shmem, d.sw>>>(d.p, d.rays, ring, d.host, it);
    else walk_kernel<false><<<blocks, 256, f.shmem, d.sw>>>(d.p, d.rays, ring, d.host, it);
    VNR_HIP_CHECK(hipGetLastError());
    VNR_HIP_CHECK(hipEventRecord(d.ev(d.ev_w, it), d.sw));
    VNR_HIP_CHECK(hipStreamWaitEvent(d.se, d.ev(d.ev_w, it), 0));
    if (profiling_) VNR_HIP_CHECK(hipEventRecord(events_[f.slot][h][2 * it], d.se));
#if defined(VNR_DIAG)
    static const bool skip_eval = [] { const char* e = std::getenv("VNR_AMD_DEBUG_SKIP_EVAL"); return e && std::atoi(e) != 0; }();
#else
    constexpr bool skip_eval = false;
#endif
    if (skip_eval) {
    } else if (f.nv) {
      f.nv->network().inference_queue((const float*)ring.queue, (float*)ring.arena, 1, ring.ctr + D_SAMPLES, d.s_max, d.se, (uint32_t)f.H, nullptr);
    } else {
      const uint32_t eb = std::min<uint32_t>(div_round_up(d.s_max, 256), (uint32_t)Runtime::get().n_cus * 8u);
      gt_sample_kernel<<<eb, 256, 0, d.se>>>(ring.ctr + D_SAMPLES, d.p.volume, d.p.vol_dims, ring.queue, (float*)ring.arena);
      VNR_HIP_CHECK(hipGetLastError());
    }
    if (profiling_) VNR_HIP_CHECK(hipEventRecord(events_[f.slot][h][2 * it + 1], d.se));
    VNR_HIP_CHECK(hipEventRecord(d.ev(d.ev_e, it), d.se));
    ++d.it_w;
    return;
  }
  if (!head_only && d.it_c < d.it_w) {
    const uint32_t it = d.it_c;
    const DRing& ring = d.ring[it % RING];
    VNR_HIP_CHECK(hipStreamWaitEvent(d.sc, d.ev(d.ev_e, it), 0));
    const uint32_t blocks = std::min<uint32_t>(div_round_up(d.p.n_local, 256), 2048u);
    compose_kernel<<<blocks, 256, f.shmem_compose, d.sc>>>(d.p, d.rays, ring, d.host, it);
    VNR_HIP_CHECK(hipGetLastError());
    VNR_HIP_CHECK(hipEventRecord(d.ev(d.ev_c, it), d.sc));
    ++d.it_c;
  }
}

void Renderer::finish_decoupled(StreamingFrame& f)
{
  if (!f.pending) return;
  f.pending = false;
  const int H = f.H;
  for (;;) {
    bool more = false;
    for (int h = 0; h < H; ++h) {
      DPart& d = f.dpart[h];
      if (d.done) continue;
      for (;;) {
        const uint32_t bw = d.it_w, bc = d.it_c;
        decoupled_step(f, h, false);
        if (d.it_w == bw && d.it_c == bc) break;
      }
    }
    for (int h = 0; h < H; ++h) {
      DPart& d = f.dpart[h];
      if (d.done) continue;
      if (d.it_c == 0 || d.it_w == 0) throw std::runtime_error("internal: a decoupled frame with nothing enqueued");
      VNR_HIP_CHECK(hipEventSynchronize(d.ev(d.ev_c, d.it_c - 1)));
      if (d.host->walking[(d.it_w - 1) & 255u] == 0 || d.it_w >= f.max_iterations) { d.done = true; continue; }
      ++d.target;
      more = true;
    }
    if (!more) break;
  }
  uint32_t pass_iterations = 0, launched[kMaxParts] = {};
  uint64_t n_samples = 0, n_ref = 0;
  for (int h = 0; h < H; ++h) {
    DPart& d = f.dpart[h];
    f.mark(h);
    uint32_t used = 0;
    while (used < d.it_w && used < 256u) { ++used; if (d.host->walking[(used - 1) & 255u] == 0) break; }
    decoupled_predicted_[h] = used;
    uint32_t with_samples = 0;
    for (uint32_t it = 0; it < used; ++it) {
      n_samples += d.host->n_smp[it & 255u];
      n_ref += d.host->n_ref[it & 255u];
      if (d.host->n_ref[it & 255u]) with_samples = it + 1;
    }
    pass_iterations = std::max(pass_iterations, with_samples);
    stats_.n_rays_hit += d.host->hit;
    launched[h] = d.it_w;
    if (profiling_) stats_.infer_kernel_launches += with_samples;
  }
  collect_eval_profile(f, launched, nullptr);
  stats_.n_iterations += pass_iterations;
  stats_.n_samples += n_samples;
  stats_.n_reference_slots += n_ref * (uint64_t)f.p_all.n_iters;
  completed_stats_ = stats_;
}

const float* Renderer::map_frame()
{
  finish_pending();
  if (distributed_) {
    issue_gather(fb_cur_);
    VNR_HIP_CHECK(hipEventSynchronize(ev_gathered_[fb_cur_]));
    const float* out = skip_download_ ? (const float*)full_[fb_cur_].ptr : (const float*)host_fb_[fb_cur_];
    fb_cur_ ^= 1;
    return out;
  }
  VNR_HIP_CHECK(hipStreamSynchronize(stream_));
  const float* out = skip_download_ ? (const float*)fb_[fb_cur_].ptr : (const float*)host_fb_[fb_cur_];
  fb_cur_ ^= 1;
  return out;
}

}
```

instantvnr_amd/csrc/renderer.h:

```cpp
#pragma once
#include <vector>

#include <memory>

#include "volume.h"

namespace vnr {

struct CameraData {
  vec3f from{0, 0, -1}, at{0, 0, 0}, up{0, 1, 0};
  float fovy = 60.0f;
};

struct FrameStats {
  uint64_t n_samples = 0, n_reference_slots = 0;
  uint32_t n_iterations = 0, n_rays_hit = 0;
  double infer_kernel_ms = 0.0;
  uint64_t infer_kernel_launches = 0;
  double infer_union_ms = 0.0;
};

struct RenderParams;

class Renderer {
public:
  explicit Renderer(std::shared_ptr<VolumeBase> volume);
  ~Renderer();

  void resize(int w, int h);
  void set_camera(const CameraData& c) { finish_pending(); camera_ = c; reset_ = true; }
  void set_transfer_function(const TransferFunctionData& t);
  void set_mode(int m) { finish_pending(); mode_ = m; reset_ = true; }
  void set_sampling_rate(float r)
  {
    if (!(r > 0.0f) || !(r < 3.0e38f)) throw std::runtime_error("volume sampling rate must be a positive finite number");
    sampling_rate_ = r; reset_ = true;
  }
  void set_density_scale(float s) { density_scale_ = s; reset_ = true; }
  void reset_accumulation() { reset_ = true; }
  void set_device_output(bool e) { finish_pending(); skip_download_ = e; }
  void set_pixel_range(uint32_t lo, uint32_t hi) { pixel_lo_ = lo; pixel_hi_ = hi; reset_ = true; }
  void set_profiling(bool e) { profiling_ = e; }
  void set_async(bool e) { finish_pending(); async_ = e; }
  void set_in_shader_kernel(int mode) { finish_pending(); in_shader_mode_ = mode; }
  const float* debug_coords() { finish_pending(); return (const float*)queue_.ptr; }
  const uint32_t* debug_counters() { finish_pending(); return counters_.ptr; }
  const std::vector<float>& debug_iteration_ms() { finish_pending(); return iter_ms_; }
  const int* debug_schedule() { finish_pending(); return last_schedule_; }
  void set_pixel_interleave(uint32_t block, uint32_t parts, uint32_t part)
  {
    if (block == 0 || parts == 0 || part >= parts) throw std::runtime_error("invalid pixel interleave");
    il_block_ = block; il_parts_ = parts; il_part_ = part; reset_ = true;
  }

  void render();
  const float* map_frame();
  void set_distributed(bool e);
  bool distributed() const { return distributed_; }
  const float* render_pipelined();
  const float* flush_pipeline();
  const FrameStats& stats() { finish_pending(); return stats_; }
  const FrameStats& completed_stats() const { return completed_stats_; }
  int width() const { return width_; }
  int height() const { return height_; }

private:
  struct StreamingFrame;
  void render_streaming(const RenderParams& p, int pass_mode, bool defer = false);
  void launch_iteration(StreamingFrame& f, int part);
  void launch_tail(StreamingFrame& f, int part, uint32_t it, hipStream_t s);
  void finish_streaming(StreamingFrame& f);
  bool decoupled_applies(const RenderParams& p, int pass_mode) const;
  void render_decoupled(const RenderParams& p, bool defer);
  void decoupled_step(StreamingFrame& f, int part, bool head_only);
  void finish_decoupled(StreamingFrame& f);
  void collect_eval_profile(StreamingFrame& f, const uint32_t* launched, const uint32_t* used);
  void finish_pending();
  void render_monolithic(const RenderParams& p);
  bool in_shader_applies() const;
  void render_in_shader(const RenderParams& p, int shade);
  void render_pathtracing(const RenderParams& p);
  void ensure_queues(size_t n_pixels, int n_iters, bool gradient);
  void ensure_share_buffers();
  void issue_gather(int buf);
  const float* hand_out_frame(int buf);

  std::shared_ptr<VolumeBase> volume_;
  CameraData camera_;
  TfnObject tfn_;
  int mode_ = 5;
  float sampling_rate_ = 1.0f, density_scale_ = 1.0f;
  int width_ = 0, height_ = 0;
  uint32_t pixel_lo_ = 0, pixel_hi_ = 0xffffffffu;
  uint32_t il_block_ = 8, il_parts_ = 1, il_part_ = 0;
  bool reset_ = true, skip_download_ = false, profiling_ = false, async_ = false;
  std::unique_ptr<StreamingFrame> frame_[2];
  int slot_ = 0;
  int frame_of_buffer_[2] = {-1, -1};
  int frame_index_ = 0;
  int n_iters_ = 24;
  DeviceBuffer<unsigned long long> is_samples_{MemTag::Renderer};
  DeviceBuffer<uint32_t> is_hits_{MemTag::Renderer};
  int in_shader_mode_ = -1;
  bool n_iters_fixed_ = false;
  vec3f light_dir_ = {0.7f, 0.9f, 0.4f};
  uint32_t tile_w_log2_ = 3;
  static constexpr int kMaxParts = 4;
  int n_halves_ = 2;
  bool n_halves_fixed_ = false;
  int small_share_parts_ = 3;
  uint32_t predicted_iterations_[2][kMaxParts] = {};
  int decoupled_mode_ = 1, decoupled_ahead_ = 3, decoupled_parts_ = 1;
  uint32_t decoupled_predicted_[kMaxParts] = {};
  hipStream_t d_streams_[kMaxParts][3] = {};
  DeviceBuffer<uint32_t> d_words_[2];
  DeviceBuffer<vec4f> d_queue_[2];
  DeviceBuffer<vec2f> d_arena_[2];
  void* d_host_ = nullptr;
  size_t d_rays_ = 0; int d_iters_ = 0, d_ring_ = 0;
  hipStream_t stream_ = nullptr, part_streams_[kMaxParts] = {};
  hipEvent_t ev_fork_ = nullptr;

  DeviceBuffer<vec4f> fb_[2], accumulation_;
  vec4f* host_fb_[2] = {nullptr, nullptr};
  size_t host_fb_pixels_ = 0;
  int fb_cur_ = 0;

  bool distributed_ = false;
  uint32_t share_world_ = 1, share_rank_ = 0, share_n_local_ = 0;
  DeviceBuffer<vec4f> gathered_[2], full_[2];
  hipEvent_t ev_rendered_ = nullptr, ev_gathered_[2] = {nullptr, nullptr};
  bool gather_issued_[2] = {false, false};
  int pipe_prev_ = -1;

  DeviceBuffer<uint32_t> q_u32_;
  DeviceBuffer<float> q_f32_;
  DeviceBuffer<int> q_i32_;
  DeviceBuffer<float> q_ssh_;
  DeviceBuffer<float> pt_rays_, pt_values_;
  uint32_t predicted_pt_ = 0;
  DeviceBuffer<float> ssh_px_;
  DeviceBuffer<uint32_t> ray_counts_;
  DeviceBuffer<vec4f> queue_;
  DeviceBuffer<float> arena_;
  bool queue_grad_ = false;
  DeviceBuffer<uint32_t> counters_;
  uint32_t* host_counts_ = nullptr;
  size_t queue_pixels_ = 0;
  int queue_iters_ = 0;
  std::vector<hipEvent_t> events_[2][kMaxParts];
  FrameStats stats_, completed_stats_;
  std::vector<float> iter_ms_;
  int last_schedule_[4] = {0, 0, 0, 0};
};

}
```

Baseline: 275.1.

## Split sample queue into per-region sub-queues and add macro-tile pixel mapping

Sample records from the ray marcher are now appended into up to 64 per-region sub-queues, each with its own counter, instead of one global queue. The inference kernel does a wave prefix scan over the region counts to map tiles onto regions. The intent is to keep samples from nearby pixel groups contiguous for better cache locality in the hash-grid lookups, and to spread atomic contention across counters. A configurable macro-tile pixel ordering is also added, but by default it reproduces the old row-major order. The cost is extra scan and readlane work per tile, a few padded tiles per region, and more counter memory.

```diff
diff --git a/instantvnr_amd/csrc/infer_kernel.h b/instantvnr_amd/csrc/infer_kernel.h
--- a/instantvnr_amd/csrc/infer_kernel.h
+++ b/instantvnr_amd/csrc/infer_kernel.h
@@ -27,6 +27,8 @@
   half_t* features_out;
   half_t* acts_out;
   const uint32_t* n_ptr;
+  uint32_t n_regions;
+  uint32_t region_stride;
   const uint32_t* dest;
   uint32_t queue_mode;
   uint32_t out_stride;
@@ -58,8 +60,21 @@
       __syncthreads();
     }
   }
-  const uint32_t n = args.n_ptr ? min(*args.n_ptr, args.n) : args.n;
-  const uint32_t n_tiles = (n + 63u) >> 6;
+  uint32_t n = 0, n_tiles, reg_count = 0, reg_end = 0, reg_base = 0;
+  if (MODE == 0) {
+    if (lane < args.n_regions) reg_count = args.n_ptr ? min(args.n_ptr[lane], args.region_stride) : args.region_stride;
+    reg_base = lane * args.region_stride;
+    reg_end = (reg_count + 63u) >> 6;
+#pragma unroll
+    for (int d = 1; d < 64; d <<= 1) {
+      const uint32_t y = __shfl_up(reg_end, d);
+      if ((int)lane >= d) reg_end += y;
+    }
+    n_tiles = __builtin_amdgcn_readlane(reg_end, 63);
+  } else {
+    n = args.n_ptr ? min(*args.n_ptr, args.n) : args.n;
+    n_tiles = (n + 63u) >> 6;
+  }
   const uint32_t xcd = blockIdx.x & 7u;
   const uint32_t per_xcd = (n_tiles + 7u) >> 3;
   const uint32_t waves_per_xcd = (gridDim.x >> 3) * WAVES;
@@ -82,7 +97,16 @@
 
   for (uint32_t tile = xcd * per_xcd + (blockIdx.x >> 3) * WAVES + wave; tile < tile_end; tile += waves_per_xcd) {
     const uint32_t i = tile * 64u + lane;
-    const uint32_t ic = min(i, n - 1u);
+    uint32_t ic = min(i, n - 1u);
+    bool valid = i < n;
+    if (MODE == 0) {
+      const uint32_t r = (uint32_t)__popcll(__ballot(reg_end <= tile));
+      const uint32_t count = __builtin_amdgcn_readlane(reg_count, r);
+      const uint32_t first_tile = __builtin_amdgcn_readlane(reg_end, r) - ((count + 63u) >> 6);
+      const uint32_t il = (tile - first_tile) * 64u + lane;
+      ic = __builtin_amdgcn_readlane(reg_base, r) + min(il, count - 1u);
+      valid = il < count;
+    }
     float3_packed p;
     uint32_t out_index = i;
     if (args.queue_mode) {
@@ -110,7 +134,7 @@
       y = mlp_tile<W, K_IN, MODE == 2, GENERAL>(args.packed_mlp, feat, nh, act, h, r, args.acts_out, n, tile * 64u);
     else
       y = mlp_tile<W, K_IN, MODE == 2, GENERAL>((const half_t*)lds, feat, nh, act, h, r, args.acts_out, n, tile * 64u);
-    if (i < n) args.out[out_index] = finish_output<GENERAL>(y, args.output_activation);
+    if (valid) args.out[out_index] = finish_output<GENERAL>(y, args.output_activation);
   }
 }
 
@@ -119,7 +143,7 @@
 {
   constexpr uint32_t WAVES = MlpShape<W>::WAVES;
   const Runtime& rt = Runtime::get();
-  const uint32_t n_tiles = div_round_up(n_max, 64);
+  const uint32_t n_tiles = div_round_up(n_max, 64) + (a.n_regions > 1u ? a.n_regions : 0u);
   uint32_t blocks = div_round_up(n_tiles, WAVES);
   static const uint32_t forced = [] {
     const char* e = std::getenv("VNR_AMD_INFER_BLOCKS_PER_CU");
diff --git a/instantvnr_amd/csrc/march_device.h b/instantvnr_amd/csrc/march_device.h
--- a/instantvnr_amd/csrc/march_device.h
+++ b/instantvnr_amd/csrc/march_device.h
@@ -19,6 +19,8 @@
   uint32_t out_parts;
   uint32_t tiles_per_row, tile_row0;
   uint32_t tile_w_log2;
+  uint32_t macro_w, macro_h;
+  uint32_t region_groups, region_cap;
   float bin_depth_rcp;
   uint32_t tfn_in_lds;
   uint32_t debug_flags;
@@ -89,10 +91,22 @@
   dir = xfm_vector(p.wto, normalize(d));
 }
 
+struct PatchCoord { uint32_t row, col; };
+__device__ __forceinline__ PatchCoord map_patch(uint32_t patch, uint32_t rows, uint32_t cols, uint32_t mw, uint32_t mh)
+{
+  const uint32_t mr = patch / (mh * cols), rem = patch - mr * (mh * cols);
+  const uint32_t h = min(mh, rows - mr * mh);
+  const uint32_t mc = rem / (mw * h), q = rem - mc * (mw * h);
+  const uint32_t w = min(mw, cols - mc * mw);
+  const uint32_t ry = q / w;
+  return {mr * mh + ry, mc * mw + (q - ry * w)};
+}
+
 __device__ __forceinline__ bool map_pixel(const RenderParams& p, uint32_t i, uint32_t& pixel)
 {
-  const uint32_t tile = i >> 6, l = i & 63u;
-  const uint32_t tr_local = tile / p.tiles_per_row, t = tile - tr_local * p.tiles_per_row;
+  const uint32_t l = i & 63u;
+  const PatchCoord pc = map_patch(i >> 6, (p.n_local >> 6) / p.tiles_per_row, p.tiles_per_row, p.macro_w, p.macro_h);
+  const uint32_t tr_local = pc.row, t = pc.col;
   const uint32_t twl = p.tile_w_log2, sub_log2 = twl - 3u;
   const uint32_t tc = t >> sub_log2, ts = t & ((1u << sub_log2) - 1u);
   const uint32_t x = (tc << twl) + (l & ((1u << twl) - 1u));
diff --git a/instantvnr_amd/csrc/network.h b/instantvnr_amd/csrc/network.h
--- a/instantvnr_amd/csrc/network.h
+++ b/instantvnr_amd/csrc/network.h
@@ -111,7 +111,7 @@
                  const uint32_t* d_dest = nullptr) const;
   bool tile_net(TileNet* out, hipStream_t s) const;
   bool inference_queue(const float* d_records, float* d_out, uint32_t out_stride, const uint32_t* d_n, size_t n_max, hipStream_t s,
-                       uint32_t sharers = 1, const PackArgs* pack = nullptr) const;
+                       uint32_t sharers = 1, const PackArgs* pack = nullptr, uint32_t n_regions = 1, uint32_t region_stride = 0) const;
   void encode(const float* d_coords, uint16_t* d_features, size_t n, hipStream_t s) const;
 
   void forward_backward(const float* d_coords, const float* d_targets, size_t batch, hipStream_t s, GradExchange* exchange = nullptr);
diff --git a/instantvnr_amd/csrc/network_host.hip b/instantvnr_amd/csrc/network_host.hip
--- a/instantvnr_amd/csrc/network_host.hip
+++ b/instantvnr_amd/csrc/network_host.hip
@@ -12,7 +12,7 @@
 void launch_fused(int mode, const GridDevice& grid, uint32_t in_width, const FusedMlp& mlp, const LevelInfo* d_levels, const uint16_t* table, size_t table_bytes,
                   const float* coords, float* out, uint16_t* features_out, uint16_t* acts_out, size_t n, const uint32_t* d_n, size_t n_max, hipStream_t s,
                   const uint32_t* d_dest = nullptr, uint32_t queue_out_stride = 0, const uint8_t* brick_image = nullptr,
-                  uint32_t sharers = 1, const struct PackArgs* pack = nullptr);
+                  uint32_t sharers = 1, const struct PackArgs* pack = nullptr, uint32_t n_regions = 1, uint32_t region_stride = 0);
 void launch_init_params(OptState* state, uint16_t* params, size_t n_mlp, size_t n_total, uint32_t in_width,
                         uint32_t n_hidden_matmuls, uint32_t width, uint64_t seed, hipStream_t s);
 void launch_master_from_f16(const uint16_t* params, OptState* state, size_t n, bool reset_optimizer, hipStream_t s);
@@ -608,7 +608,7 @@
 }
 
 bool Network::inference_queue(const float* d_records, float* d_out, uint32_t out_stride, const uint32_t* d_n, size_t n_max, hipStream_t s,
-                              uint32_t sharers, const PackArgs* pack) const
+                              uint32_t sharers, const PackArgs* pack, uint32_t n_regions, uint32_t region_stride) const
 {
   const uint8_t* image;
   const LevelInfo* levels = inference_levels(s, &image, n_max);
@@ -616,7 +616,7 @@
   grid.n_levels = n_active_levels();
   if (cfg_.n_neurons == 128u) pack = nullptr;
   launch_fused(0, grid, in_width_, fused_mlp(), levels, params_f16_.ptr + n_mlp_, n_grid_params() * 2, d_records, d_out, nullptr, nullptr, 0, d_n, n_max, s, nullptr,
-               out_stride, image, sharers, pack);
+               out_stride, image, sharers, pack, n_regions, region_stride);
   return pack != nullptr;
 }
 
diff --git a/instantvnr_amd/csrc/network_infer.hip b/instantvnr_amd/csrc/network_infer.hip
--- a/instantvnr_amd/csrc/network_infer.hip
+++ b/instantvnr_amd/csrc/network_infer.hip
@@ -62,7 +62,8 @@
 
 void launch_fused(int mode, const GridDevice& grid, uint32_t in_width, const FusedMlp& mlp, const LevelInfo* d_levels, const uint16_t* table, size_t table_bytes,
                   const float* coords, float* out, uint16_t* features_out, uint16_t* acts_out, size_t n, const uint32_t* d_n, size_t n_max, hipStream_t s,
-                  const uint32_t* d_dest, uint32_t queue_out_stride, const uint8_t* brick_image, uint32_t sharers, const PackArgs* pack)
+                  const uint32_t* d_dest, uint32_t queue_out_stride, const uint8_t* brick_image, uint32_t sharers, const PackArgs* pack,
+                  uint32_t n_regions, uint32_t region_stride)
 {
   if (n_max == 0) { if (pack && pack->n_blocks) throw std::runtime_error("internal: ray packing fused into an empty evaluation launch"); return; }
   if (n_max > 0xffffffc0ull) throw std::runtime_error("inference batch too large (max 2^32-64 samples per call)");
@@ -81,10 +82,15 @@
   a.features_out = (half_t*)features_out;
   a.acts_out = (half_t*)acts_out;
   a.n_ptr = d_n;
+  if (n_regions > 1u && (mode != 0 || !d_n || !queue_out_stride || n_regions > (uint32_t)kMaxRegions || region_stride == 0u ||
+                         (size_t)n_regions * region_stride > 0xffffffc0ull))
+    throw std::runtime_error("internal: a queue in regions is the ray marcher's (inference, counts on the device, at most 64 regions)");
+  a.n_regions = std::max(n_regions, 1u);
   a.dest = d_dest;
   a.queue_mode = queue_out_stride ? 1u : 0u;
   a.out_stride = queue_out_stride;
   a.n = d_n ? (uint32_t)n_max : (uint32_t)n;
+  a.region_stride = a.n_regions > 1u ? region_stride : a.n;
   a.n_hidden_matmuls = mlp.n_hidden_matmuls;
   a.activation = mlp.activation;
   a.output_activation = mlp.output_activation;
diff --git a/instantvnr_amd/csrc/network_train.hip b/instantvnr_amd/csrc/network_train.hip
--- a/instantvnr_amd/csrc/network_train.hip
+++ b/instantvnr_amd/csrc/network_train.hip
@@ -5,7 +5,7 @@
 void launch_fused(int mode, const GridDevice& grid, uint32_t in_width, const FusedMlp& mlp, const LevelInfo* d_levels, const uint16_t* table, size_t table_bytes,
                   const float* coords, float* out, uint16_t* features_out, uint16_t* acts_out, size_t n, const uint32_t* d_n, size_t n_max, hipStream_t s,
                   const uint32_t* d_dest = nullptr, uint32_t queue_out_stride = 0, const uint8_t* brick_image = nullptr,
-                  uint32_t sharers = 1, const struct PackArgs* pack = nullptr);
+                  uint32_t sharers = 1, const struct PackArgs* pack = nullptr, uint32_t n_regions = 1, uint32_t region_stride = 0);
 
 struct Pcg32 {
   uint64_t state, inc;
diff --git a/instantvnr_amd/csrc/pack_rays.h b/instantvnr_amd/csrc/pack_rays.h
--- a/instantvnr_amd/csrc/pack_rays.h
+++ b/instantvnr_amd/csrc/pack_rays.h
@@ -21,7 +21,15 @@
   float* alpha[2];
 };
 
-enum { C_RAYS0 = 0, C_RAYS1 = 1, C_SAMPLES0 = 2, C_SAMPLES1 = 3, C_HIT = 4, C_STAT_SAMPLES = 6, C_STAT_REFRAYS = 8, C_COUNT = 16 };
+constexpr int kMaxRegions = 64;
+enum { C_RAYS0 = 0, C_RAYS1 = 1, C_HIT = 4, C_STAT_SAMPLES = 6, C_STAT_REFRAYS = 8, C_STATS_END = 16, C_SAMPLES0 = 16, C_COUNT = C_SAMPLES0 + 2 * kMaxRegions };
+__host__ __device__ __forceinline__ constexpr int c_samples(int parity) { return C_SAMPLES0 + kMaxRegions * parity; }
+
+struct QueueRegions {
+  const uint32_t* counts;
+  uint32_t n_regions;
+  uint32_t stride;
+};
 
 struct PackArgs {
   RayList src, dst;
@@ -45,10 +53,10 @@
   const int parity = a.parity;
   const uint32_t n_in = a.first ? a.n_first : counters[C_RAYS0 + parity];
   const uint32_t n_groups = ((n_in + 255u) & ~255u) >> 6;
-  if (item == 0 && tid == 0) counters[C_SAMPLES0 + (parity ^ 1)] = 0;
+  if (item == 0 && tid < (uint32_t)kMaxRegions) counters[c_samples(parity ^ 1) + tid] = 0;
   if (n_groups == 0) {
     if (item == 0 && tid == 0) { counters[C_RAYS0 + (parity ^ 1)] = 0; *a.host_alive = 0; }
-    if (item == 0 && tid >= C_HIT && tid < C_COUNT) a.host_stats[tid] = counters[tid];
+    if (item == 0 && tid >= C_HIT && tid < C_STATS_END) a.host_stats[tid] = counters[tid];
     return;
   }
   const uint32_t g0 = item * (uint32_t)WAVES;
@@ -95,22 +103,22 @@
   if (last_block) {
     uint32_t asum = 0;
     for (uint32_t g = tid; g < n_groups; g += T) asum += ray_counts[g] >> 8;
+    uint32_t records = counters[c_samples(parity) + lane];
 #pragma unroll
-    for (int d = 32; d > 0; d >>= 1) asum += __shfl_xor(asum, d);
+    for (int d = 32; d > 0; d >>= 1) { asum += __shfl_xor(asum, d); records += __shfl_xor(records, d); }
     __syncthreads();
     if (lane == 0) s_part[wave] = asum;
     __syncthreads();
     if (tid == 0) {
       uint32_t alive_total = 0;
       for (int w = 0; w < WAVES; ++w) alive_total += s_part[w];
-      const uint32_t records = counters[C_SAMPLES0 + parity];
       unsigned long long* c64 = (unsigned long long*)counters;
       c64[C_STAT_SAMPLES / 2] += (unsigned long long)(a.grad ? records >> 2 : records);
       c64[C_STAT_REFRAYS / 2] += (unsigned long long)alive_total;
       if (a.first) counters[C_HIT] += alive_total;
     }
     __syncthreads();
-    if (tid >= C_HIT && tid < C_COUNT) a.host_stats[tid] = ((volatile uint32_t*)counters)[tid];
+    if (tid >= C_HIT && tid < C_STATS_END) a.host_stats[tid] = ((volatile uint32_t*)counters)[tid];
   }
 }
 #endif
diff --git a/instantvnr_amd/csrc/render.hip b/instantvnr_amd/csrc/render.hip
--- a/instantvnr_amd/csrc/render.hip
+++ b/instantvnr_amd/csrc/render.hip
@@ -2,6 +2,7 @@
 
 #include <algorithm>
 #include <cfloat>
+#include <cstdio>
 #include <cstdlib>
 
 #include "dist.h"
@@ -40,7 +41,7 @@
   }
   const uint32_t tid = threadIdx.x, lane = tid & 63u;
   const uint32_t n_in = FIRST ? p.n_local : counters[C_RAYS0 + parity];
-  uint32_t* n_samples_out = counters + C_SAMPLES0 + parity;
+  uint32_t* n_samples_out = counters + c_samples(parity);
   const uint32_t n_round = (n_in + 255u) & ~255u;
   const unsigned long long lt_mask = (1ull << lane) - 1ull;
   uint32_t trip = 0;
@@ -205,8 +206,9 @@
     if (tid == 0) {
       const uint32_t total = claim[0] + claim[1] + claim[2] + claim[3];
       uint32_t b = 0;
-      if (total) b = GRAD ? atomicAdd(n_samples_out, 4u * total) >> 2 : atomicAdd(n_samples_out, total);
-      claim[4] = b;
+      const uint32_t region = (base >> 6) / p.region_groups;
+      if (total) b = GRAD ? atomicAdd(n_samples_out + region, 4u * total) >> 2 : atomicAdd(n_samples_out + region, total);
+      claim[4] = region * p.region_cap + b;
     }
     __syncthreads();
     uint32_t smp_base = claim[4];
@@ -282,13 +284,16 @@
 }
 
 
-__global__ void gt_sample_kernel(const uint32_t* __restrict__ n_ptr, const float* __restrict__ vol, vec3i dims,
+__global__ void gt_sample_kernel(const QueueRegions regions, const float* __restrict__ vol, vec3i dims,
                                  const vec4f* __restrict__ queue, float* __restrict__ arena)
 {
-  const uint32_t n = *n_ptr;
-  for (uint32_t i = blockIdx.x * blockDim.x + threadIdx.x; i < n; i += gridDim.x * blockDim.x) {
-    const vec4f r = queue[i];
-    arena[__float_as_uint(r.w)] = sample_volume_nodal(vol, dims, r.x, r.y, r.z);
+  for (uint32_t k = 0; k < regions.n_regions; ++k) {
+    const uint32_t n = min(regions.counts[k], regions.stride);
+    const vec4f* __restrict__ q = queue + (size_t)k * regions.stride;
+    for (uint32_t i = blockIdx.x * blockDim.x + threadIdx.x; i < n; i += gridDim.x * blockDim.x) {
+      const vec4f r = q[i];
+      arena[__float_as_uint(r.w)] = sample_volume_nodal(vol, dims, r.x, r.y, r.z);
+    }
   }
 }
 
@@ -591,6 +596,7 @@
   uint32_t* hs;
   hipStream_t s;
   size_t s_max;
+  uint32_t n_regions = 1, region_stride = 0;
   uint32_t it = 0, used = 0;
   bool done = false;
   bool tail_skipped = false;
@@ -651,6 +657,11 @@
   if (const char* e = std::getenv("VNR_AMD_TILE_W")) {
     const int w = std::atoi(e);
     tile_w_log2_ = w == 16 ? 4u : w == 32 ? 5u : w == 64 ? 6u : 3u;
+  }
+  if (const char* e = std::getenv("VNR_AMD_REGION_GROUPS")) region_groups_ = (uint32_t)std::max(0, std::min(1 << 20, std::atoi(e)));
+  if (const char* e = std::getenv("VNR_AMD_MACRO_TILE")) {
+    int w = 0, h = 0;
+    if (std::sscanf(e, "%dx%d", &w, &h) == 2 && w >= 1 && h >= 1 && w <= 1024 && h <= 1024) { macro_w_ = (uint32_t)w; macro_h_ = (uint32_t)h; }
   }
   if (const char* e = std::getenv("VNR_AMD_DECOUPLED")) decoupled_mode_ = std::max(0, std::min(2, std::atoi(e)));
   if (const char* e = std::getenv("VNR_AMD_DECOUPLED_AHEAD")) decoupled_ahead_ = std::max(1, std::min(7, std::atoi(e)));
@@ -866,6 +877,8 @@
   p.out_parts = distributed_ ? share_world_ : 1u;
   p.tile_w_log2 = tile_w_log2_;
   p.tiles_per_row = div_round_up((uint32_t)width_, 1u << p.tile_w_log2) << (p.tile_w_log2 - 3u);
+  p.macro_w = macro_w_ ? macro_w_ : p.tiles_per_row; p.macro_h = macro_h_;
+  p.region_groups = 0; p.region_cap = 0;
   const uint32_t tr_lo = p.pixel_hi > p.pixel_lo ? (p.pixel_lo / (uint32_t)width_) / 8u : 0u;
   const uint32_t tr_hi = p.pixel_hi > p.pixel_lo ? ((p.pixel_hi - 1u) / (uint32_t)width_) / 8u + 1u : 0u;
   p.tile_row0 = il_parts_ == 1 ? tr_lo : 0u;
@@ -1080,7 +1093,7 @@
     } else {
       if (nv) nv->network().inference_queue((const float*)queue_.ptr, pt_values_.ptr, 1, c + C_RAYS0 + parity, P, s, 1);
       else gt_sample_kernel<<<std::min<uint32_t>(div_round_up(P, 256), (uint32_t)Runtime::get().n_cus * 8u), 256, 0, s>>>(
-               c + C_RAYS0 + parity, p.volume, p.vol_dims, queue_.ptr, pt_values_.ptr);
+               QueueRegions{c + C_RAYS0 + parity, 1u, P}, p.volume, p.vol_dims, queue_.ptr, pt_values_.ptr);
       pt_kernel<false><<<blocks, 256, 0, s>>>(p, dense, scratch, pt_values_.ptr, c, ray_counts_.ptr, parity);
     }
     pt_compact_kernel<<<cblocks, 1024, 0, s>>>(scratch, dense, ray_counts_.ptr, P, c, parity, it == 0 ? 1 : 0, queue_.ptr);
@@ -1182,11 +1195,12 @@
 #endif
     if (skip_eval) {
     } else if (nv) {
-      packed = nv->network().inference_queue((const float*)hf.queue, (float*)hf.vd[parity], 1, c + C_SAMPLES0 + parity, hf.s_max, s_it, (uint32_t)H,
-                                             fused_pack ? &pk : nullptr);
+      packed = nv->network().inference_queue((const float*)hf.queue, (float*)hf.vd[parity], 1, c + c_samples(parity), hf.s_max, s_it, (uint32_t)H,
+                                             fused_pack ? &pk : nullptr, hf.n_regions, hf.region_stride);
     } else {
       const uint32_t blocks = std::min<uint32_t>(div_round_up(hf.s_max, 256), (uint32_t)Runtime::get().n_cus * 8u);
-      gt_sample_kernel<<<blocks, 256, 0, s_it>>>(c + C_SAMPLES0 + parity, hf.p.volume, hf.p.vol_dims, hf.queue, (float*)hf.vd[parity]);
+      gt_sample_kernel<<<blocks, 256, 0, s_it>>>(QueueRegions{c + c_samples(parity), hf.n_regions, hf.region_stride}, hf.p.volume, hf.p.vol_dims, hf.queue,
+                                                 (float*)hf.vd[parity]);
     }
     if (profiling_) VNR_HIP_CHECK(hipEventRecord(events_[f.slot][h][2 * it + 1], s_it));
     last_schedule_[2] = packed ? 1 : 0;
@@ -1273,6 +1287,16 @@
       hf.vd[b] = (vec2f*)(arena_base + (size_t)b * slot_floats * QP * QI + slot_floats * off * QI);
     }
     hf.p.slot_cap = (uint32_t)((size_t)hf.p.n_local * QI);
+    {
+      const uint32_t groups = hf.p.n_local / 64u;
+      uint32_t G = region_groups_ ? std::min(region_groups_, groups) : groups;
+      G = std::max(G, div_round_up(groups, (uint32_t)kMaxRegions));
+      G = std::max(next_multiple(G, 4u), 4u);
+      hf.n_regions = std::max(div_round_up(groups, G), 1u);
+      hf.p.region_groups = G;
+      hf.p.region_cap = (uint32_t)std::min<size_t>((size_t)G * 64u * (size_t)hf.p.n_iters, 0xffffffffu);
+      hf.region_stride = (uint32_t)std::min<size_t>((size_t)hf.p.region_cap * (grad ? 4 : 1), 0xffffffffu);
+    }
     hf.queue = queue_base + rec_per_slot * off * QI;
     hf.c = counters_base + (size_t)h * C_COUNT;
     hf.rc = rc_base + off / 64 + (size_t)h * 8;
@@ -1583,7 +1607,7 @@
       f.nv->network().inference_queue((const float*)ring.queue, (float*)ring.arena, 1, ring.ctr + D_SAMPLES, d.s_max, d.se, (uint32_t)f.H, nullptr);
     } else {
       const uint32_t eb = std::min<uint32_t>(div_round_up(d.s_max, 256), (uint32_t)Runtime::get().n_cus * 8u);
-      gt_sample_kernel<<<eb, 256, 0, d.se>>>(ring.ctr + D_SAMPLES, d.p.volume, d.p.vol_dims, ring.queue, (float*)ring.arena);
+      gt_sample_kernel<<<eb, 256, 0, d.se>>>(QueueRegions{ring.ctr + D_SAMPLES, 1u, (uint32_t)d.s_max}, d.p.volume, d.p.vol_dims, ring.queue, (float*)ring.arena);
       VNR_HIP_CHECK(hipGetLastError());
     }
     if (profiling_) VNR_HIP_CHECK(hipEventRecord(events_[f.slot][h][2 * it + 1], d.se));
diff --git a/instantvnr_amd/csrc/renderer.h b/instantvnr_amd/csrc/renderer.h
--- a/instantvnr_amd/csrc/renderer.h
+++ b/instantvnr_amd/csrc/renderer.h
@@ -105,6 +105,7 @@
   bool n_iters_fixed_ = false;
   vec3f light_dir_ = {0.7f, 0.9f, 0.4f};
   uint32_t tile_w_log2_ = 3;
+  uint32_t region_groups_ = 0, macro_w_ = 0, macro_h_ = 1;
   static constexpr int kMaxParts = 4;
   int n_halves_ = 2;
   bool n_halves_fixed_ = false;
```

Result: slower. 271.1 (-1.4%).
